# PytorchConnectomics/pytorch_connectomics

Measured on AMD Instinct MI355X. Metric: voxels/s (train + sliding-window infer), MedNeXt-S 112^3 bf16, higher is better.
Workload: dtype bf16; 1 GPU; Lucchi++ sliding-window inference (configs[1]): MedNeXt-S k3, 165x1024x768 volume, roi 112^3, overlap 0.5, bump blending, sw_batch_size 8, random-init weights; step = one whole-volume EagerSlidingWindowEngine call (TTA off); value = window-voxels/s; sw_batch_size=8, window_pipeline_streams=3

## Files before the change

### include/pytc_hip.h

```cpp
#ifndef PYTC_HIP_H
#define PYTC_HIP_H

#include <stdint.h>

#ifdef __cplusplus
extern "C" {
#endif

#define PYTC_ABI_VERSION 10

#define PYTC_OK 0
#define PYTC_ERR_INVALID 1
#define PYTC_ERR_HIP 2
#define PYTC_ERR_UNSUPPORTED 3

#define PYTC_F32 0
#define PYTC_BF16 1

#define PYTC_VIEW_FLIP_Z 1
#define PYTC_VIEW_FLIP_Y 2
#define PYTC_VIEW_FLIP_X 4
#define PYTC_VIEW_SWAP_YX 8
#define PYTC_VIEW_SWAP_ZY 16
#define PYTC_VIEW_SWAP_ZX 32

#define PYTC_PAD_CONSTANT 0
#define PYTC_PAD_REFLECT 1
#define PYTC_PAD_REPLICATE 2
#define PYTC_PAD_CIRCULAR 3

#define PYTC_BLEND_PRODUCT 0
#define PYTC_BLEND_MIN 1

#define PYTC_ACT_NONE 0
#define PYTC_ACT_SIGMOID 1
#define PYTC_ACT_TANH 2
#define PYTC_ACT_GELU 3

#define PYTC_RES_NONE 0
#define PYTC_RES_ADD 1
#define PYTC_RES_UPSAMPLE 2
#define PYTC_RES_GELU_BWD 3
#define PYTC_RES_NORM_BWD 4

int pytc_abi_version(void);
const char* pytc_last_error(void);
int pytc_device_info(int device, int* cu_count, int* lds_bytes_per_cu, char* arch, int arch_len);
int pytc_set_tuning(const char* key, int value);


int pytc_gather_windows(const float* vol, int C, int Z, int Y, int X, const int32_t* starts, int B,
                        int rz, int ry, int rx, int view, int pad_mode, float cval, void* out,
                        int out_dtype, void* stream);

int pytc_blend_accumulate(const void* pred, int pred_dtype, int B, const int32_t* starts, int rz,
                          int ry, int rx, int C, int view, const float* wz, const float* wy,
                          const float* wx, int combine, float floor_w, const int32_t* border ,
                          float* value, float* weight, int Z, int Y, int X, void* stream);

int pytc_blend_accumulate_mapped(const void* pred, int pred_dtype, int B, const int32_t* starts, int rz, int ry,
                                 int rx, int C, int view, const float* wz, const float* wy, const float* wx,
                                 int combine, float floor_w, const int32_t* border, const int32_t* chan_src,
// ... 105 lines not shown

typedef struct {
  const void* t;
  const float* ab;
  const void* w2_packed;
  const float* b2;
  const void* w3_packed;
  const float* b3;
  const void* res;
  const void* res_low;
  const float* res_bias;
  void* y;
  int N;
  int64_t rows_per_sample;
  int C_in, C_hid, C_out;
  int res_mode;
  int Di, Hi, Wi;
  int w3_format;
  int per_sample;
} pytc_mlp_args;
#define PYTC_W3_BF16 0
#define PYTC_W3_F16 1

int pytc_pw_gemm_supported(int C_in, int C_out);
int pytc_pw_gemm_fwd(const void* x, const void* w, const float* bias, const float* ab, void* y, int N, int64_t rows_per_sample,
                     int C_in, int C_out, int in_f16, int gelu_out, const void* res, const void* res_low, const float* res_bias,
                     int res_mode, int Di, int Hi, int Wi, void* stream);
int pytc_pw_mlp_supported(int C_in, int C_hid, int C_out);
int pytc_pw_pack_weight_paired(const float* w, int C_out, int C_in, int transposed, void* packed_bf16,
                               void* stream);
int pytc_pack_multi(const int64_t* table_dev, int n_items, int64_t total_elems, void* stream);
int pytc_pw_pack_weight_paired_f16(const float* w, int C_out, int C_in, int transposed, void* packed_f16,
                                   void* stream);
int pytc_pw_mlp_fwd(const pytc_mlp_args* a, void* stream);

int pytc_pw_mlp_lds_supported(int C_in, int C_hid, int C_out);
int pytc_pw_mlp_lds_fwd(const pytc_mlp_args* a, void* stream);
int pytc_pw_mlp_dma_applies(const pytc_mlp_args* a, int ignore_res_mode);
int pytc_pw_mlp_proj_supported(int C_in, int C_hid, int C_out, int C_proj);
int pytc_pw_mlp_proj_fwd(const pytc_mlp_args* a, const void* proj_w, const float* proj_b, void* z, int store_y, void* stream);
int pytc_pw_mlp_chunk_supported(int C_in, int C_hid, int C_out);
int pytc_pw_mlp_chunk_fwd(const pytc_mlp_args* a, void* stream);
int pytc_groupnorm_fold_mlp(const float* stats, int slots, float count, const float* gamma, const float* beta, float eps,
                            const float* w2, const float* b2, void* w2n, float* b2n, float* ab_out, int N, int C, int C_hid,
                            void* stream);
int pytc_pw_mlp_train_fwd(const pytc_mlp_args* a, void* hidden_pre, void* stream);
int pytc_pw_mlp_train_fwd_nostore(const pytc_mlp_args* a, void* stream);
int pytc_pw_mlp_bwd(const pytc_mlp_args* a, const void* hidden_pre, void* d_hidden, void* stream);
int pytc_pw_mlp_up_supported(int C_in, int C_hid, int C_out);
int pytc_pw_mlp_up_fwd(const pytc_mlp_args* a, const float* taps, const float* dw_bias, void* stream);
int pytc_pw_mlp_head_supported(int C_in, int C_hid, int C_out);
int pytc_pw_mlp_stemres_fwd(const pytc_mlp_args* a, const float* stem_x, const float* stem_w, const float* stem_b,
                            void* stream);
int pytc_stem_dwconv3d_stat_slots(int D, int H, int W);
int pytc_stem_dwconv3d_supported(int C_in, int C, int K);
int pytc_stem_dwconv3d_mfma_image_bytes(void);
int pytc_stem_dwconv3d_pack_mfma(const float* wx, const float* wb, const float* cst, void* image, void* stream);
int pytc_stem_dwconv3d_fwd(const float* x, const float* wx, const float* wb, const float* cst, const void* mfma_image, void* y,
                           float* stats, int N, int D, int H, int W, int C, void* stream);
int pytc_pw_mlp_head_fwd(const pytc_mlp_args* a, const void* head_w, const float* head_b, float* head_y, int n_head,
                         int store_y, void* stream);


#define PYTC_ACT_RELU 5
#define PYTC_ACT_LEAKY 6
#define PYTC_ACT_ELU 7

typedef struct {
  const void* x;
  const void* w_packed;
  const float* bias;
  const float* ab;
  const void* res;
  void* y;
  int N, D, H, W, C_in, C_out;
  int kd, kh, kw;
  int act_in;
  float act_param;
  int res_mode;
  int dtype;
} pytc_conv3d_args;

int64_t pytc_conv3d_packed_elems(int C_out, int C_in, int kd, int kh, int kw, int dtype);
int pytc_conv3d_pack_weight(const float* w, int C_out, int C_in, int kd, int kh, int kw, void* packed, int dtype,
                            void* stream);
int pytc_conv3d_fwd(const pytc_conv3d_args* a, void* stream);

int pytc_channel_stats_slots(int64_t rows);
int pytc_channel_stats(const void* x, float* stats, int N, int64_t rows, int C, int dtype, void* stream);
int pytc_norm_finalize_groups(const float* stats, int slots, float count, const float* gamma, const float* beta,
                              float eps, int groups, float* ab, int N, int C, void* stream);
int pytc_affine_act(const void* x, void* y, const float* ab, int N, int64_t rows, int C, int act, float prm,
                    int dtype, void* stream);
int pytc_maxpool3d_fwd(const void* x, void* y, int N, int D, int H, int W, int C, int fz, int fy, int fx, int dtype,
                       void* stream);
int pytc_dwconvT3d_generic_fwd(const void* x, void* y, const float* w, int N, int D, int H, int W, int C,
                               const int32_t* kernel, const int32_t* stride, const int32_t* pad, int dtype,
                               void* stream);


int pytc_groupnorm_finalize_mr(const float* stats, int slots, float count, const float* gamma, const float* beta,
                               float eps, float* ab, float* mean_rstd, int N, int C, void* stream);
int pytc_gelu(const void* x, const void* dy, void* out, int64_t n, int dtype, void* stream);
int pytc_add_inplace(void* y, const void* x, int64_t n, int dtype, void* stream);
int pytc_pw_wgrad_slots(int64_t rows_total);
int pytc_pw_wgrad(const void* x, const float* ab, const void* dy, float* dW, float* db, float* workspace, int N,
// ... 217 lines not shown
```

### pytorch_connectomics_amd/_native.py

```python
from __future__ import annotations

import ctypes as C
import os
from pathlib import Path

LIB_PATH = Path(__file__).resolve().parent / "lib" / "libpytc_hip.so"
ABI_VERSION = 10

F32, BF16 = 0, 1
OK = 0

VIEW_FLIP_Z, VIEW_FLIP_Y, VIEW_FLIP_X, VIEW_SWAP_YX, VIEW_SWAP_ZY, VIEW_SWAP_ZX = 1, 2, 4, 8, 16, 32
VIEW_SWAPS = {VIEW_SWAP_YX: (1, 2), VIEW_SWAP_ZY: (0, 1), VIEW_SWAP_ZX: (0, 2)}
PAD_MODES = {"constant": 0, "reflect": 1, "replicate": 2, "circular": 3}
BLEND_PRODUCT, BLEND_MIN = 0, 1
ACT_NONE, ACT_SIGMOID, ACT_TANH, ACT_GELU, ACT_SOFTMAX, ACT_RELU, ACT_LEAKY, ACT_ELU = 0, 1, 2, 3, 4, 5, 6, 7
RES_NONE, RES_ADD, RES_UPSAMPLE, RES_GELU_BWD, RES_NORM_BWD = 0, 1, 2, 3, 4


class PwArgs(C.Structure):
    _fields_ = [
        ("x", C.c_void_p), ("w_packed", C.c_void_p), ("bias", C.c_void_p), ("ab", C.c_void_p),
        ("res", C.c_void_p), ("y", C.c_void_p),
        ("N", C.c_int), ("rows_per_sample", C.c_int64),
        ("C_in", C.c_int), ("C_out", C.c_int),
        ("in_dtype", C.c_int), ("out_dtype", C.c_int), ("w_dtype", C.c_int),
        ("act", C.c_int), ("res_mode", C.c_int), ("gather", C.c_int),
        ("Di", C.c_int), ("Hi", C.c_int), ("Wi", C.c_int),
        ("res_low", C.c_void_p), ("res_bias", C.c_void_p), ("pre_act", C.c_int), ("w_paired", C.c_int),
    ]


class MlpArgs(C.Structure):
    _fields_ = [
        ("t", C.c_void_p), ("ab", C.c_void_p), ("w2_packed", C.c_void_p), ("b2", C.c_void_p),
        ("w3_packed", C.c_void_p), ("b3", C.c_void_p), ("res", C.c_void_p), ("res_low", C.c_void_p),
        ("res_bias", C.c_void_p), ("y", C.c_void_p),
        ("N", C.c_int), ("rows_per_sample", C.c_int64),
        ("C_in", C.c_int), ("C_hid", C.c_int), ("C_out", C.c_int), ("res_mode", C.c_int),
        ("Di", C.c_int), ("Hi", C.c_int), ("Wi", C.c_int), ("w3_format", C.c_int), ("per_sample", C.c_int),
    ]


W3_BF16, W3_F16 = 0, 1
NORM_NONE, NORM_ZSCORE, NORM_MINMAX, NORM_DIVIDE = 0, 1, 2, 3
RAW_DTYPES = {"uint8": 0, "int8": 1, "uint16": 2, "int16": 3, "uint32": 4, "int32": 5, "float32": 6, "float64": 7}


class ReduceItem(C.Structure):
    _fields_ = [("part", C.c_void_p), ("out", C.c_void_p), ("n", C.c_int64), ("slots", C.c_int32), ("out_t", C.c_int32)]


class Conv3dArgs(C.Structure):
    _fields_ = [
        ("x", C.c_void_p), ("w_packed", C.c_void_p), ("bias", C.c_void_p), ("ab", C.c_void_p), ("res", C.c_void_p),
        ("y", C.c_void_p),
        ("N", C.c_int), ("D", C.c_int), ("H", C.c_int), ("W", C.c_int), ("C_in", C.c_int), ("C_out", C.c_int),
        ("kd", C.c_int), ("kh", C.c_int), ("kw", C.c_int),
        ("act_in", C.c_int), ("act_param", C.c_float), ("res_mode", C.c_int), ("dtype", C.c_int),
    ]
# ... 139 lines not shown
                                      C.c_int, C.c_void_p]),
    "pytc_convT3d_phase_plan": (C.c_int, [C.c_int, C.c_int, C.c_int, C.c_void_p]),
    "pytc_convT3d_phase_supported": (C.c_int, [C.c_int, C.c_int, C.c_int]),
    "pytc_convT3d_phase_fwd": (C.c_int, [C.POINTER(Conv3dArgs), C.POINTER(C.c_int32), C.c_void_p]),
    "pytc_conv3d_wgrad_strided_ws_elems": (C.c_int64, [C.c_int, C.POINTER(C.c_int32), C.c_int, C.c_int, C.POINTER(C.c_int32)]),
    "pytc_conv3d_wgrad_strided": (C.c_int, [C.c_void_p, C.c_void_p, C.c_void_p, C.c_void_p, C.c_int, C.POINTER(C.c_int32),
                                            C.POINTER(C.c_int32), C.c_int, C.c_int, C.POINTER(C.c_int32), C.POINTER(C.c_int32),
                                            C.POINTER(C.c_int32), C.c_int, C.c_void_p]),
    "pytc_conv3d_pack_plan": (C.c_int, [C.c_int] * 7 + [C.c_void_p]),
    "pytc_conv3d_pack_multi": (C.c_int, [C.c_void_p, C.c_int, C.c_int64, C.c_void_p]),
    "pytc_conv3d_launch_plan": (C.c_int, [C.c_int] * 13 + [C.c_void_p]),
    "pytc_conv3d_pack_weight_dgrad": (C.c_int, [C.c_void_p, C.c_int, C.c_int, C.c_int, C.c_int, C.c_int, C.c_void_p, C.c_int, C.c_void_p]),
    "pytc_norm_bwd_means": (C.c_int, [C.c_void_p, C.c_void_p, C.c_void_p, C.c_void_p, C.c_void_p, C.c_int, C.c_int, C.c_int,
                                      C.c_float, C.c_void_p]),
    "pytc_norm_bwd_means_cpg": (C.c_int, [C.c_void_p, C.c_void_p, C.c_void_p, C.c_void_p, C.c_void_p, C.c_int, C.c_int, C.c_int,
                                          C.c_int, C.c_float, C.c_void_p]),
    "pytc_norm_finalize_groups_cpg": (C.c_int, [C.c_void_p, C.c_int, C.c_float, C.c_void_p, C.c_void_p, C.c_float, C.c_int, C.c_int,
                                                C.c_void_p, C.c_void_p, C.c_int, C.c_int, C.c_void_p]),
    "pytc_bn_train_finalize": (C.c_int, [C.c_void_p, C.c_int, C.c_float, C.c_void_p, C.c_void_p, C.c_float, C.c_float, C.c_void_p,
                                         C.c_void_p, C.c_void_p, C.c_void_p, C.c_void_p, C.c_int, C.c_int, C.c_void_p]),
    "pytc_bn_train_finalize_cpad": (C.c_int, [C.c_void_p, C.c_int, C.c_float, C.c_void_p, C.c_void_p, C.c_float, C.c_float, C.c_void_p,
                                              C.c_void_p, C.c_void_p, C.c_void_p, C.c_void_p, C.c_int, C.c_int, C.c_int, C.c_void_p]),
    "pytc_bn_update_running": (C.c_int, [C.c_void_p, C.c_void_p, C.c_void_p, C.c_int, C.c_float, C.c_float, C.c_float, C.c_void_p]),
    "pytc_layernorm_rows": (C.c_int, [C.c_void_p, C.c_void_p, C.c_void_p, C.c_void_p, C.c_int64, C.c_int, C.c_float, C.c_int, C.c_void_p]),
    "pytc_layernorm_rows_bwd_slots": (C.c_int, [C.c_int64, C.c_int, C.c_int]),
    "pytc_layernorm_rows_bwd": (C.c_int, [C.c_void_p, C.c_void_p, C.c_void_p, C.c_void_p, C.c_void_p, C.c_int64, C.c_int, C.c_float,
                                          C.c_int, C.c_void_p]),
    "pytc_grn_bwd_apply": (C.c_int, [C.c_void_p, C.c_void_p, C.c_void_p, C.c_void_p, C.c_void_p, C.c_int, C.c_int64, C.c_int, C.c_int,
                                     C.c_void_p]),
    "pytc_bce_dice_ws_elems": (C.c_int64, [C.c_int, C.c_int, C.c_int64]),
    "pytc_bce_dice_fwd": (C.c_int, [C.c_void_p, C.c_void_p, C.c_void_p, C.c_int, C.c_int, C.c_int64, C.POINTER(C.c_int64),
                                    C.POINTER(C.c_int64), C.POINTER(C.c_int64), C.c_float, C.c_float, C.c_float, C.c_float,
                                    C.c_float, C.c_void_p, C.c_void_p, C.c_void_p, C.c_void_p]),
    "pytc_bce_dice_bwd": (C.c_int, [C.c_void_p, C.c_void_p, C.c_void_p, C.c_void_p, C.c_void_p, C.c_void_p, C.c_void_p,
                                    C.c_int, C.c_int, C.c_int64, C.POINTER(C.c_int64), C.POINTER(C.c_int64),
                                    C.POINTER(C.c_int64), C.POINTER(C.c_int64), C.c_float, C.c_float, C.c_float, C.c_float,
                                    C.c_float, C.c_void_p]),
    "pytc_opt_chunk_elems": (C.c_int, []),
    "pytc_grad_norm_multi": (C.c_int, [C.c_void_p, C.c_void_p, C.c_int, C.c_float, C.c_void_p, C.c_void_p, C.c_void_p]),
    "pytc_adamw_multi": (C.c_int, [C.c_void_p, C.c_void_p, C.c_int, C.POINTER(C.c_float), C.c_int, C.c_void_p, C.c_void_p]),
    "pytc_pw_mlp_supported": (C.c_int, [C.c_int, C.c_int, C.c_int]),
    "pytc_pw_pack_weight_paired": (C.c_int, [C.c_void_p, C.c_int, C.c_int, C.c_int, C.c_void_p, C.c_void_p]),
    "pytc_pack_multi": (C.c_int, [C.c_void_p, C.c_int, C.c_int64, C.c_void_p]),
    "pytc_pw_pack_weight_paired_f16": (C.c_int, [C.c_void_p, C.c_int, C.c_int, C.c_int, C.c_void_p, C.c_void_p]),
    "pytc_pw_mlp_fwd": (C.c_int, [C.POINTER(MlpArgs), C.c_void_p]),
    "pytc_pw_mlp_lds_supported": (C.c_int, [C.c_int, C.c_int, C.c_int]),
    "pytc_pw_mlp_lds_fwd": (C.c_int, [C.POINTER(MlpArgs), C.c_void_p]),
    "pytc_pw_mlp_dma_applies": (C.c_int, [C.POINTER(MlpArgs), C.c_int]),
    "pytc_pw_mlp_proj_supported": (C.c_int, [C.c_int, C.c_int, C.c_int, C.c_int]),
    "pytc_pw_mlp_proj_fwd": (C.c_int, [C.POINTER(MlpArgs), C.c_void_p, C.c_void_p, C.c_void_p, C.c_int, C.c_void_p]),
    "pytc_pw_mlp_chunk_supported": (C.c_int, [C.c_int, C.c_int, C.c_int]),
    "pytc_pw_mlp_chunk_fwd": (C.c_int, [C.POINTER(MlpArgs), C.c_void_p]),
    "pytc_pw_mlp_stemres_fwd": (C.c_int, [C.POINTER(MlpArgs), C.c_void_p, C.c_void_p, C.c_void_p, C.c_void_p]),
    "pytc_stem_dwconv3d_stat_slots": (C.c_int, [C.c_int, C.c_int, C.c_int]),
    "pytc_stem_dwconv3d_supported": (C.c_int, [C.c_int, C.c_int, C.c_int]),
    "pytc_convT3d_thin_supported": (C.c_int, [C.c_int, C.c_int]),
    "pytc_convT3d_thin_fwd": (C.c_int, [C.c_void_p, C.c_void_p, C.c_void_p, C.c_void_p, C.c_int, C.POINTER(C.c_int32), C.c_int, C.c_int,
                                        C.c_int, C.c_void_p]),
    "pytc_stem_dwconv3d_mfma_image_bytes": (C.c_int, []),
    "pytc_stem_dwconv3d_pack_mfma": (C.c_int, [C.c_void_p, C.c_void_p, C.c_void_p, C.c_void_p, C.c_void_p]),
    "pytc_stem_dwconv3d_fwd": (C.c_int, [C.c_void_p, C.c_void_p, C.c_void_p, C.c_void_p, C.c_void_p, C.c_void_p, C.c_void_p,
                                         C.c_int, C.c_int, C.c_int, C.c_int, C.c_int, C.c_void_p]),
    "pytc_pw_mlp_train_fwd": (C.c_int, [C.POINTER(MlpArgs), C.c_void_p, C.c_void_p]),
    "pytc_pw_mlp_train_fwd_nostore": (C.c_int, [C.POINTER(MlpArgs), C.c_void_p]),
    "pytc_pw_mlp_bwd": (C.c_int, [C.POINTER(MlpArgs), C.c_void_p, C.c_void_p, C.c_void_p]),
    "pytc_pw_mlp_up_supported": (C.c_int, [C.c_int, C.c_int, C.c_int]),
    "pytc_pw_mlp_up_fwd": (C.c_int, [C.POINTER(MlpArgs), C.c_void_p, C.c_void_p, C.c_void_p]),
    "pytc_pw_mlp_head_supported": (C.c_int, [C.c_int, C.c_int, C.c_int]),
    "pytc_pw_mlp_head_fwd": (C.c_int, [C.POINTER(MlpArgs), C.c_void_p, C.c_void_p, C.c_void_p, C.c_int, C.c_int, C.c_void_p]),
    "pytc_upcat_deconv2_fwd": (C.c_int, [C.c_void_p, C.c_void_p, C.c_void_p, C.c_void_p, C.c_void_p] + [C.c_int] * 11 + [C.c_void_p]),
    "pytc_upcat_deconv2_bwd_data": (C.c_int, [C.c_void_p, C.c_void_p, C.c_void_p, C.c_void_p] + [C.c_int] * 11 + [C.c_void_p]),
    "pytc_upcat_deconv2_wgrad_ws_elems": (C.c_int64, [C.c_int] * 4),
    "pytc_upcat_deconv2_wgrad": (C.c_int, [C.c_void_p] * 5 + [C.c_int] * 11 + [C.c_void_p]),
    "pytc_linear_fwd": (C.c_int, [C.c_void_p] * 4 + [C.c_int] + [C.c_void_p] * 2 + [C.c_int] * 5 + [C.c_void_p]),
    "pytc_linear_bwd_data": (C.c_int, [C.c_void_p] * 4 + [C.c_int] * 4 + [C.c_void_p]),
    "pytc_linear_wgrad": (C.c_int, [C.c_void_p] * 5 + [C.c_int] * 6 + [C.c_void_p]),
    "pytc_layernorm_wide": (C.c_int, [C.c_void_p] * 4 + [C.c_int64, C.c_int, C.c_float, C.c_int, C.c_void_p]),
    "pytc_layernorm_wide_bwd_slots": (C.c_int, [C.c_int64]),
    "pytc_layernorm_wide_bwd": (C.c_int, [C.c_void_p] * 7 + [C.c_int64, C.c_int, C.c_float, C.c_int, C.c_void_p]),
    "pytc_patch_gather16": (C.c_int, [C.c_void_p] * 2 + [C.c_int] * 7 + [C.c_void_p]),
    "pytc_attention_supported": (C.c_int, [C.c_int]),
    "pytc_attention_fwd": (C.c_int, [C.c_void_p] * 3 + [C.c_int] * 4 + [C.c_float, C.c_int, C.c_void_p]),
    "pytc_attention_bwd": (C.c_int, [C.c_void_p] * 6 + [C.c_int] * 4 + [C.c_float, C.c_int, C.c_void_p]),
    "pytc_deconv2_upfirst_fwd": (C.c_int, [C.c_void_p] * 5 + [C.c_int] * 8 + [C.c_void_p]),
    "pytc_deconv2_upfirst_bwd_data": (C.c_int, [C.c_void_p] * 4 + [C.c_int] * 8 + [C.c_void_p]),
    "pytc_deconv2_upfirst_wgrad": (C.c_int, [C.c_void_p] * 5 + [C.c_int] * 8 + [C.c_void_p]),
    "pytc_window_attention_supported": (C.c_int, [C.c_int]),
    "pytc_window_attention_bias_groups": (C.c_int, [C.c_int] * 3),
    "pytc_window_attention_fwd": (C.c_int, [C.c_void_p] * 2 + [C.POINTER(C.c_int32)] + [C.c_void_p] * 2 + [C.c_int] * 4
                                  + [C.c_float, C.c_int, C.c_void_p]),
    "pytc_window_attention_bwd": (C.c_int, [C.c_void_p] * 2 + [C.POINTER(C.c_int32)] + [C.c_void_p] * 7 + [C.c_int] * 4
                                  + [C.c_float, C.c_int, C.c_void_p]),
    "pytc_window_partition": (C.c_int, [C.c_void_p] * 3 + [C.POINTER(C.c_int32)] + [C.c_int] * 4 + [C.c_void_p]),
    "pytc_space_to_depth2": (C.c_int, [C.c_void_p] * 2 + [C.c_int] * 8 + [C.c_void_p]),
    "pytc_layernorm_any": (C.c_int, [C.c_void_p] * 4 + [C.c_int64, C.c_int, C.c_float, C.c_int, C.c_void_p]),
    "pytc_layernorm_any_bwd_slots": (C.c_int, [C.c_int64]),
    "pytc_layernorm_any_bwd": (C.c_int, [C.c_void_p] * 8 + [C.c_int64, C.c_int, C.c_float, C.c_int, C.c_void_p]),
    "pytc_cldice_tiles": (C.c_int, [C.c_int64]),
    "pytc_cldice_erode": (C.c_int, [C.c_void_p] * 2 + [C.c_int] * 5 + [C.c_void_p]),
    "pytc_cldice_skeleton": (C.c_int, [C.c_void_p] * 7 + [C.c_int] * 6 + [C.c_void_p]),
    "pytc_cldice_chain_bwd": (C.c_int, [C.c_void_p] * 7 + [C.c_int] * 6 + [C.c_void_p]),
    "pytc_cldice_sweep_bwd": (C.c_int, [C.c_void_p] * 9 + [C.c_int] * 7 + [C.c_void_p]),
    "pytc_scnp_tiles": (C.c_int, [C.c_int64]),
    "pytc_scnp_forward": (C.c_int, [C.c_void_p] * 7 + [C.c_int] * 9 + [C.c_void_p]),
    "pytc_scnp_backward": (C.c_int, [C.c_void_p] * 7 + [C.c_int] * 9 + [C.c_void_p]),
    "pytc_softmax_loss_tiles": (C.c_int, [C.c_int64]),
# ... 55 lines not shown
```

### pytorch_connectomics_amd/csrc/pw_mlp_kernels.hip

```cpp
#include <cmath>
#include "pw_common.h"

namespace pytc {

struct MlpParams {
  const bf16_t* t;
  const float* ab;
  const bf16x8_t* w2;
  const float* b2;
  const bf16x8_t* w3;
  const float* b3;
  EpiParams e;
  long rps;
  int C_in, C_hid, C_out, HC;
  int w3_f16;
  long w2_stride;
  const bf16x8_t* head_w;
  const float* head_b;
  float* head_y;
  int n_head, store_y;
  bf16_t* proj_y;
  const float* stem_x;
  const float* stem_w;
  const float* stem_b;
  bf16_t* hp;
  int round_h;
  const bf16_t* hp_in;
};

constexpr int mlp_waves_per_simd(int ks, int mo, int nt) {
  if (ks >= 8 && nt == 1) return 1;
  const int regs = ks * nt * 4 + mo * nt * 4 + 2 * nt * 4;
  return regs <= 64 ? 4 : (regs <= 112 ? 3 : (regs <= 200 ? 2 : 1));
}

template <int KS_IN, int MO, int NT, int GELU_MODE, bool HEAD = false, bool STEMRES = false, bool STOREH = false, bool BWD = false>
__global__ void __launch_bounds__(256, mlp_waves_per_simd(KS_IN, MO, NT))
pw_mlp_kernel(MlpParams p) {
  constexpr int CIN = KS_IN * 32, COUT = MO * 16;
  static_assert(MO % 2 == 0, "C_out must be a multiple of 32");
  static_assert(!STEMRES || (MO == 2 && (MO / 2) * NT <= 4), "the stem-recomputing residual covers C_out = 32");
  static_assert(!HEAD || MO == 2, "the fused head covers C_out = 32");
  static_assert(GELU_MODE == 1 || GELU_MODE == 3, "sigmoid-form or packed-fp16 GELU");
  constexpr bool PREFETCH_RES = (MO / 2) * NT <= 4;
  const int wave = threadIdx.x >> 6, lane = threadIdx.x & 63;
  const int n = blockIdx.y;
  constexpr bool WARM = KS_IN * MO >= 32;
  constexpr int WPER = KS_IN * MO >= 512 ? 6 : 2;
  WarmRegs<WPER> warm;
  const bool folded = p.ab == nullptr;
  const bf16x8_t* w2 = p.w2 + (folded ? (long)n * p.w2_stride : 0L);
  const float* b2 = p.b2 + (folded ? (long)n * p.C_hid : 0L);
  if (WARM) {
    warm_l2(w2, (long)p.C_hid * CIN * 2, warm, 0);
    warm_l2(p.w3, (long)COUT * p.C_hid * 2, warm, WPER);
  }
  const long row0 = ((long)blockIdx.x * 4 + wave) * (NT * 16);
  if (row0 >= p.rps) {
    if (WARM) asm volatile("s_waitcnt vmcnt(0)" : : : "memory");
    return;
  }
  const int r = lane & 15, kb = lane >> 4;

  long orow[NT];
#pragma unroll
  for (int nt = 0; nt < NT; ++nt) orow[nt] = row0 + nt * 16 + r;

  bf16x8_t bact[KS_IN][NT];
  const bf16_t* tn = p.t + (long)n * p.rps * CIN;
  if (folded) {
#pragma unroll
    for (int ks = 0; ks < KS_IN; ++ks)
#pragma unroll
      for (int nt = 0; nt < NT; ++nt) {
        const long rr = orow[nt] < p.rps ? orow[nt] : p.rps - 1;
        bact[ks][nt] = ld_stream(reinterpret_cast<const bf16x8_t*>(tn + rr * CIN + ks * 32 + kb * 8), p.e.nt);
      }
  }
  const float* an = p.ab + (long)n * 2 * CIN;
#pragma unroll
  for (int ks = 0; ks < KS_IN; ++ks) {
    if (folded) break;
    const int k0 = ks * 32 + kb * 8;
    float av[8], bv[8];
    VecIO<float, 4>::load(an + k0, reinterpret_cast<float(&)[4]>(av[0]));
    VecIO<float, 4>::load(an + k0 + 4, reinterpret_cast<float(&)[4]>(av[4]));
    VecIO<float, 4>::load(an + CIN + k0, reinterpret_cast<float(&)[4]>(bv[0]));
    VecIO<float, 4>::load(an + CIN + k0 + 4, reinterpret_cast<float(&)[4]>(bv[4]));
#pragma unroll
    for (int nt = 0; nt < NT; ++nt) {
      const long rr = orow[nt] < p.rps ? orow[nt] : p.rps - 1;
      float v[8];
      VecIO<bf16_t, 8>::load(tn + rr * CIN + k0, v);
#pragma unroll
      for (int j = 0; j < 8; ++j) v[j] = fmaf(v[j], av[j], bv[j]);
      bact[ks][nt] = Mma<bf16_t>::from_floats(v);
    }
  }

  if (WARM) warm_l2_done(warm);

  uint4 rpre[PREFETCH_RES ? MO / 2 : 1][PREFETCH_RES ? NT : 1];
  const bool use_pre = PREFETCH_RES && p.e.res_mode != PYTC_RES_NONE;
  if constexpr (STEMRES) {
    const float* sx = p.stem_x + (long)n * p.rps;
    float sw[8], sb[8];
    VecIO<float, 4>::load(p.stem_w + kb * 8, reinterpret_cast<float(&)[4]>(sw[0]));
    VecIO<float, 4>::load(p.stem_w + kb * 8 + 4, reinterpret_cast<float(&)[4]>(sw[4]));
    VecIO<float, 4>::load(p.stem_b + kb * 8, reinterpret_cast<float(&)[4]>(sb[0]));
    VecIO<float, 4>::load(p.stem_b + kb * 8 + 4, reinterpret_cast<float(&)[4]>(sb[4]));
#pragma unroll
    for (int nt = 0; nt < NT; ++nt) {
      const float xv = sx[orow[nt] < p.rps ? orow[nt] : p.rps - 1];
      float rv[8];
#pragma unroll
      for (int j = 0; j < 8; ++j) rv[j] = fmaf(sw[j], xv, sb[j]);
      rpre[0][nt] = __builtin_bit_cast(uint4, Mma<bf16_t>::from_floats(rv));
    }
  } else if (use_pre) {
    const bf16_t* resn = reinterpret_cast<const bf16_t*>(p.e.res) + (long)n * p.rps * COUT;
#pragma unroll
    for (int pr = 0; pr < (PREFETCH_RES ? MO / 2 : 1); ++pr)
#pragma unroll
      for (int nt = 0; nt < (PREFETCH_RES ? NT : 1); ++nt) {
        const long rr = orow[nt] < p.rps ? orow[nt] : p.rps - 1;
        rpre[pr][nt] = ld_stream(reinterpret_cast<const uint4*>(resn + rr * COUT + pr * 32 + kb * 8), p.e.nt);
      }
  }

  f32x4_t acc2[MO][NT];
#pragma unroll
  for (int pr = 0; pr < MO / 2; ++pr) {
    float b[8];
    VecIO<float, 4>::load(p.b3 + pr * 32 + kb * 8, reinterpret_cast<float(&)[4]>(b[0]));
    VecIO<float, 4>::load(p.b3 + pr * 32 + kb * 8 + 4, reinterpret_cast<float(&)[4]>(b[4]));
#pragma unroll
    for (int nt = 0; nt < NT; ++nt) {
      acc2[2 * pr][nt] = f32x4_t{b[0], b[1], b[2], b[3]};
      acc2[2 * pr + 1][nt] = f32x4_t{b[4], b[5], b[6], b[7]};
    }
  }

  for (int hc = 0; hc < p.HC; ++hc) {
    float b2v[8];
    VecIO<float, 4>::load(b2 + hc * 32 + kb * 8, reinterpret_cast<float(&)[4]>(b2v[0]));
    VecIO<float, 4>::load(b2 + hc * 32 + kb * 8 + 4, reinterpret_cast<float(&)[4]>(b2v[4]));
    f32x4_t acc1[2][NT];
#pragma unroll
    for (int nt = 0; nt < NT; ++nt) {
      acc1[0][nt] = f32x4_t{b2v[0], b2v[1], b2v[2], b2v[3]};
      acc1[1][nt] = f32x4_t{b2v[4], b2v[5], b2v[6], b2v[7]};
    }
#pragma unroll
    for (int mt = 0; mt < 2; ++mt) {
#pragma unroll
      for (int ks = 0; ks < KS_IN; ++ks) {
        const bf16x8_t a = w2[((long)(hc * 2 + mt) * KS_IN + ks) * 64 + lane];
#pragma unroll
        for (int nt = 0; nt < NT; ++nt) acc1[mt][nt] = Mma<bf16_t>::mma(a, bact[ks][nt], acc1[mt][nt]);
      }
    }
    bf16x8_t bh[NT];
    h8_t bhh[GELU_MODE == 3 ? NT : 1];
#pragma unroll
    for (int nt = 0; nt < NT; ++nt) {
      float g[8];
// ... 83 lines not shown
  }
  int upos[NT][3];
  const bool ups = p.e.res_mode == PYTC_RES_UPSAMPLE;
  if (ups) {
    const unsigned ur = (unsigned)row0, gw = (unsigned)p.e.Go_w, gh = (unsigned)p.e.Go_h;
    const unsigned t0 = ur / gw;
    const int bx = (int)(ur - t0 * gw);
    const int bz = (int)(t0 / gh);
    const int by = (int)(t0 - (unsigned)bz * gh);
#pragma unroll
    for (int nt = 0; nt < NT; ++nt) {
      int px = bx + nt * 16 + r, py = by, pz = bz;
      while (px >= p.e.Go_w) { px -= p.e.Go_w; ++py; }
      while (py >= p.e.Go_h) { py -= p.e.Go_h; ++pz; }
      upos[nt][0] = pz; upos[nt][1] = py; upos[nt][2] = px;
    }
  }
#pragma unroll
  for (int pr = 0; pr < MO / 2; ++pr) {
#pragma unroll
    for (int nt = 0; nt < NT; ++nt) {
      if (orow[nt] >= p.rps) continue;
      float v[8];
#pragma unroll
      for (int j = 0; j < 4; ++j) {
        v[j] = acc2[2 * pr][nt][j];
        v[4 + j] = acc2[2 * pr + 1][nt][j];
      }
      if (use_pre) {
        float pre[8];
        VecIO<bf16_t, 8>::load(reinterpret_cast<const bf16_t*>(&rpre[PREFETCH_RES ? pr : 0][PREFETCH_RES ? nt : 0]), pre);
        finish_and_store<bf16_t, 8, false, COUT>(v, p.e, n, orow[nt], pr * 32 + kb * 8, pre, ups ? upos[nt] : nullptr);
      } else {
        finish_and_store<bf16_t, 8, false, COUT>(v, p.e, n, orow[nt], pr * 32 + kb * 8, nullptr, ups ? upos[nt] : nullptr);
      }
    }
  }
}


__device__ __forceinline__ void glds16(const void* gsrc, unsigned lds_dst) {
  unsigned keep;
  asm volatile("s_mov_b32 %0, m0\n\ts_mov_b32 m0, %2\n\ts_nop 0\n\tglobal_load_lds_dwordx4 %1, off\n\ts_mov_b32 m0, %0"
               : "=&s"(keep) : "v"(gsrc), "s"(lds_dst) : "memory");
}
__device__ __forceinline__ void glds4(const void* gsrc, unsigned lds_dst) {
  unsigned keep;
  asm volatile("s_mov_b32 %0, m0\n\ts_mov_b32 m0, %2\n\ts_nop 0\n\tglobal_load_lds_dword %1, off\n\ts_mov_b32 m0, %0"
               : "=&s"(keep) : "v"(gsrc), "s"(lds_dst) : "memory");
}

template <int HCT, int KIND>
__global__ void __launch_bounds__(256, 3)
pw_mlp_dma_kernel(MlpParams p, int waves_per_sample) {
  constexpr int NT = 4, CIN = 32, COUT = 32;
  constexpr bool STEM = KIND == 1, HEAD = KIND == 2, PROJ = KIND == 3;
  __shared__ __attribute__((aligned(16))) uint4 land[4][2][NT * 64];
  __shared__ __attribute__((aligned(16))) uint4 w2s[HCT * 2 * 64], w3s[2 * HCT * 64];
  __shared__ __attribute__((aligned(16))) float b2s[HCT * 32], b3s[32];
  __shared__ __attribute__((aligned(16))) float auxa[STEM ? 32 : (HEAD ? 256 : (PROJ ? 512 : 4))], auxb[(STEM || PROJ) ? 32 : (HEAD ? 16 : 4)];
  const int wave = threadIdx.x >> 6, lane = threadIdx.x & 63;
  const int n = blockIdx.y;
  const int r = lane & 15, kb = lane >> 4;
  const long tiles = (p.rps + NT * 16 - 1) / (NT * 16);
  const bool with_res = STEM || p.e.res_mode == PYTC_RES_ADD;
  const bf16_t* tn = p.t + (long)n * p.rps * CIN;
  const bf16_t* resn = (!STEM && with_res) ? reinterpret_cast<const bf16_t*>(p.e.res) + (long)n * p.rps * COUT : nullptr;
  const float* sx = STEM ? p.stem_x + (long)n * p.rps : nullptr;
  bf16_t* yn = reinterpret_cast<bf16_t*>(p.e.y) + (long)n * p.rps * COUT;
  float* hy = HEAD ? p.head_y + (long)n * p.rps * p.n_head : nullptr;
  bf16_t* zn = PROJ ? p.proj_y + (long)n * p.rps * 32 : nullptr;
  {
    const uint4* w2 = reinterpret_cast<const uint4*>(p.w2 + (long)n * p.w2_stride);
    const uint4* w3 = reinterpret_cast<const uint4*>(p.w3);
    for (int i = threadIdx.x; i < HCT * 2 * 64; i += 256) { w2s[i] = w2[i]; w3s[i] = w3[i]; }
    if (threadIdx.x < HCT * 32) b2s[threadIdx.x] = p.b2[(long)n * p.C_hid + threadIdx.x];
    if (threadIdx.x < 32) b3s[threadIdx.x] = p.b3[threadIdx.x];
    if constexpr (STEM) {
      if (threadIdx.x < 32) { auxa[threadIdx.x] = p.stem_w[threadIdx.x]; auxb[threadIdx.x] = p.stem_b[threadIdx.x]; }
    }
    if constexpr (HEAD) {
      reinterpret_cast<float*>(auxa)[threadIdx.x] = reinterpret_cast<const float*>(p.head_w)[threadIdx.x];
      if (threadIdx.x < 16) auxb[threadIdx.x] = (p.head_b && (int)threadIdx.x < p.n_head) ? p.head_b[threadIdx.x] : 0.f;
    }
    if constexpr (PROJ) {
      auxa[threadIdx.x] = reinterpret_cast<const float*>(p.head_w)[threadIdx.x];
      auxa[threadIdx.x + 256] = reinterpret_cast<const float*>(p.head_w)[threadIdx.x + 256];
      if (threadIdx.x < 32) auxb[threadIdx.x] = p.head_b ? p.head_b[threadIdx.x] : 0.f;
    }
  }
  __syncthreads();
  asm volatile("s_waitcnt vmcnt(0)" ::: "memory");

  const unsigned lbase = __builtin_amdgcn_readfirstlane((unsigned)(size_t)(__attribute__((address_space(3))) void*)&land[wave][0][0]);
  auto request = [&](long tile) {
#pragma unroll
    for (int nt = 0; nt < NT; ++nt) {
      long row = tile * (NT * 16) + nt * 16 + r;
      row = row < p.rps ? row : p.rps - 1;
      glds16(tn + row * CIN + kb * 8, lbase + (unsigned)(nt * 64) * 16);
      if constexpr (STEM) glds4(sx + row, lbase + (unsigned)(NT * 64) * 16 + (unsigned)(nt * 64) * 4);
      else if (with_res) glds16(resn + row * COUT + kb * 8, lbase + (unsigned)((NT + nt) * 64) * 16);
    }
  };
  bf16x8_t out[NT];
  f32x4_t hout[HEAD ? NT : 1];
  bf16x8_t zout[PROJ ? NT : 1];
  auto store = [&](long tile) {
#pragma unroll
    for (int nt = 0; nt < NT; ++nt) {
      const long row = tile * (NT * 16) + nt * 16 + r;
      if (row >= p.rps) continue;
      if (!(HEAD || PROJ) || p.store_y) *reinterpret_cast<bf16x8_t*>(yn + row * COUT + kb * 8) = out[nt];
      if constexpr (PROJ) *reinterpret_cast<bf16x8_t*>(zn + row * 32 + kb * 8) = zout[nt];
      if constexpr (HEAD) {
#pragma unroll
        for (int i = 0; i < 4; ++i)
          if (kb * 4 + i < p.n_head) hy[row * p.n_head + kb * 4 + i] = hout[nt][i];
      }
    }
  };
  const long gw = (long)blockIdx.x * 4 + wave;
  long tile = gw;
  if (tile >= tiles) return;
  request(tile);
  long out_tile = -1;
  for (; tile < tiles; tile += waves_per_sample) {
    asm volatile("s_waitcnt vmcnt(0)" ::: "memory");
    __builtin_amdgcn_wave_barrier();
    if (out_tile >= 0) store(out_tile);
    bf16x8_t bact[NT];
    uint4 rpre[STEM ? 1 : NT];
    float xin[STEM ? NT : 1];
#pragma unroll
    for (int nt = 0; nt < NT; ++nt) {
      bact[nt] = __builtin_bit_cast(bf16x8_t, land[wave][0][nt * 64 + lane]);
      if constexpr (STEM) xin[nt] = reinterpret_cast<const float*>(&land[wave][1][0])[nt * 64 + lane];
      else if (with_res) rpre[nt] = land[wave][1][nt * 64 + lane];
    }
    asm volatile("s_waitcnt lgkmcnt(0)" ::: "memory");
    __builtin_amdgcn_wave_barrier();
    if (tile + waves_per_sample < tiles) request(tile + waves_per_sample);
    f32x4_t acc2[2][NT];
    {
      const f32x4_t lo = *reinterpret_cast<const f32x4_t*>(&b3s[kb * 8]), hi = *reinterpret_cast<const f32x4_t*>(&b3s[kb * 8 + 4]);
#pragma unroll
      for (int nt = 0; nt < NT; ++nt) { acc2[0][nt] = lo; acc2[1][nt] = hi; }
    }
#pragma unroll
    for (int hc = 0; hc < HCT; ++hc) {
      f32x4_t acc1[2][NT];
      {
        const f32x4_t lo = *reinterpret_cast<const f32x4_t*>(&b2s[hc * 32 + kb * 8]), hi = *reinterpret_cast<const f32x4_t*>(&b2s[hc * 32 + kb * 8 + 4]);
#pragma unroll
        for (int nt = 0; nt < NT; ++nt) { acc1[0][nt] = lo; acc1[1][nt] = hi; }
// ... 22 lines not shown
    float sw[STEM ? 8 : 1], sb[STEM ? 8 : 1];
    if constexpr (STEM) {
#pragma unroll
      for (int j = 0; j < 8; ++j) { sw[j] = auxa[kb * 8 + j]; sb[j] = auxb[kb * 8 + j]; }
    }
#pragma unroll
    for (int nt = 0; nt < NT; ++nt) {
      float v[8];
#pragma unroll
      for (int j = 0; j < 4; ++j) { v[j] = acc2[0][nt][j]; v[4 + j] = acc2[1][nt][j]; }
      if constexpr (STEM) {
        float rv[8], pre[8];
#pragma unroll
        for (int j = 0; j < 8; ++j) rv[j] = fmaf(sw[j], xin[nt], sb[j]);
        const bf16x8_t rb = Mma<bf16_t>::from_floats(rv);
        VecIO<bf16_t, 8>::load(reinterpret_cast<const bf16_t*>(&rb), pre);
#pragma unroll
        for (int j = 0; j < 8; ++j) v[j] += pre[j];
      } else if (with_res) {
        float pre[8];
        VecIO<bf16_t, 8>::load(reinterpret_cast<const bf16_t*>(&rpre[nt]), pre);
#pragma unroll
        for (int j = 0; j < 8; ++j) v[j] += pre[j];
      }
      out[nt] = Mma<bf16_t>::from_floats(v);
      if constexpr (HEAD) {
        const bf16x8_t ah = __builtin_bit_cast(bf16x8_t, reinterpret_cast<const uint4*>(auxa)[lane]);
        const f32x4_t hb = *reinterpret_cast<const f32x4_t*>(&auxb[kb * 4]);
        const f32x4_t h = Mma<bf16_t>::mma(ah, out[nt], f32x4_t{0.f, 0.f, 0.f, 0.f});
#pragma unroll
        for (int i = 0; i < 4; ++i) hout[nt][i] = h[i] + hb[i];
      }
      if constexpr (PROJ) {
        f32x4_t z0 = *reinterpret_cast<const f32x4_t*>(&auxb[kb * 8]), z1 = *reinterpret_cast<const f32x4_t*>(&auxb[kb * 8 + 4]);
        z0 = Mma<bf16_t>::mma(__builtin_bit_cast(bf16x8_t, reinterpret_cast<const uint4*>(auxa)[lane]), out[nt], z0);
        z1 = Mma<bf16_t>::mma(__builtin_bit_cast(bf16x8_t, reinterpret_cast<const uint4*>(auxa)[64 + lane]), out[nt], z1);
        float zv[8];
#pragma unroll
        for (int j = 0; j < 4; ++j) { zv[j] = z0[j]; zv[4 + j] = z1[j]; }
        zout[nt] = Mma<bf16_t>::from_floats(zv);
      }
    }
    out_tile = tile;
  }
  store(out_tile);
}

static bool mlp_dma_applies(const pytc_mlp_args* a, const MlpParams& p) {
  return a->per_sample && p.w3_f16 && a->C_in == 32 && a->C_out == 32 && (p.HC == 2 || p.HC == 3 || p.HC == 4) &&
         (a->res_mode == PYTC_RES_NONE || a->res_mode == PYTC_RES_ADD) && tuning_get(K_mlp_dma) != 0 &&
         (long)a->N * a->rows_per_sample >= (long)tuning_get(K_mlp_dma_rows);
}
template <int KIND>
static void mlp_dma_launch(const pytc_mlp_args* a, const MlpParams& p, hipStream_t s) {
  const long tiles = (a->rows_per_sample + 63) / 64;
  long wgs = (3072 + a->N - 1) / a->N;
  const long most = (tiles / 2 + 3) / 4;
  if (wgs > most) wgs = most < 1 ? 1 : most;
  if (const int forced = tuning_get(K_mlp_dma_wgs); forced > 0) wgs = forced;
  dim3 grid((unsigned)wgs, (unsigned)a->N), block(256);
  const int wps = (int)(wgs * 4);
  if (p.HC == 2) hipLaunchKernelGGL((pw_mlp_dma_kernel<2, KIND>), grid, block, 0, s, p, wps);
  else if (p.HC == 3) hipLaunchKernelGGL((pw_mlp_dma_kernel<3, KIND>), grid, block, 0, s, p, wps);
  else hipLaunchKernelGGL((pw_mlp_dma_kernel<4, KIND>), grid, block, 0, s, p, wps);
}

template <typename OUT>
__global__ void __launch_bounds__(256)
pw_pack_paired_kernel(const float* __restrict__ w, int C_out, int C_in, int transposed,
                      OUT* __restrict__ packed, int KG, long total) {
  long i = (long)blockIdx.x * blockDim.x + threadIdx.x;
  if (i >= total) return;
  int j = (int)(i % 8);
  long t = i / 8;
  int lane = (int)(t % 64);
  t /= 64;
  int kg = (int)(t % KG);
  int T = (int)(t / KG);
  int o = paired_row(T, lane & 15);
  int k = kg * 32 + (lane >> 4) * 8 + j;
  float v = 0.f;
  if (o < C_out && k < C_in) v = transposed ? w[(long)k * C_out + o] : w[(long)o * C_in + k];
  if constexpr (sizeof(OUT) == 2 && !__is_same(OUT, bf16_t)) packed[i] = (OUT)v;
  else packed[i] = from_f32<bf16_t>(v);
}

__global__ void __launch_bounds__(256)
pack_multi_kernel(const long* __restrict__ table, int n_items, long total) {
  const long i = (long)blockIdx.x * blockDim.x + threadIdx.x;
  __shared__ int s_lo;
  if (threadIdx.x == 0) {
    const long i0 = (long)blockIdx.x * blockDim.x;
    int lo = 0, hi = n_items - 1;
    while (lo < hi) {
      const int mid = (lo + hi + 1) >> 1;
      if (table[mid * 8 + 6] <= i0) lo = mid; else hi = mid - 1;
    }
    s_lo = lo;
  }
  __syncthreads();
  if (i >= total) return;
  int lo = s_lo;
  while (lo + 1 < n_items && table[(lo + 1) * 8 + 6] <= i) ++lo;
  const long* it = table + lo * 8;
  const float* w = reinterpret_cast<const float*>(it[0]);
  const int kind = (int)it[2], C_out = (int)it[3], C_in = (int)it[4], aux = (int)it[5];
  const long e = i - it[6];
  if (kind >= 6) {
    const int o = (int)(e / C_in), k = (int)(e % C_in);
    reinterpret_cast<bf16_t*>(it[1])[e] = from_f32<bf16_t>(kind == 7 ? w[(long)k * C_out + o] : w[e]);
    return;
  }
  if (kind >= 4) {
    const int K3 = aux, C = C_out;
    const int k = (int)(e / C), c = (int)(e % C);
    reinterpret_cast<float*>(it[1])[e] = w[(long)c * K3 + (kind == 5 ? K3 - 1 - k : k)];
    return;
// ... 225 lines not shown
  PYTC_LAUNCH_CHECK("pw_pack_weight_paired_f16");
  return PYTC_OK;
}

extern "C" int pytc_pack_multi(const int64_t* table_dev, int n_items, int64_t total_elems, void* stream) {
  PYTC_REQUIRE(table_dev && n_items >= 1 && total_elems >= 1, "pack_multi: bad arguments");
  hipLaunchKernelGGL(pack_multi_kernel, dim3(ceil_div(total_elems, 256)), dim3(256), 0, (hipStream_t)stream,
                     reinterpret_cast<const long*>(table_dev), n_items, (long)total_elems);
  PYTC_LAUNCH_CHECK("pack_multi");
  return PYTC_OK;
}

extern "C" int pytc_pw_mlp_head_fwd(const pytc_mlp_args* a, const void* head_w, const float* head_b, float* head_y,
                                    int n_head, int store_y, void* stream) {
  PYTC_REQUIRE(a && a->t && (a->ab || a->per_sample) && a->w2_packed && a->w3_packed && a->b2 && a->b3 && head_w && head_y, "pw_mlp_head: null pointer");
  PYTC_REQUIRE(!(a->ab && a->per_sample), "pw_mlp_head: per-sample (norm-folded) expand operands come without an affine");
  PYTC_REQUIRE(!store_y || a->y, "pw_mlp_head: store_y without an output buffer");
  PYTC_REQUIRE(a->N >= 1 && a->rows_per_sample >= 1 && n_head >= 1 && n_head <= 16, "pw_mlp_head: bad shape");
  if (!pytc_pw_mlp_head_supported(a->C_in, a->C_hid, a->C_out)) {
    set_error("pw_mlp_head: no fused kernel for C_in=%d C_hid=%d C_out=%d", a->C_in, a->C_hid, a->C_out);
    return PYTC_ERR_UNSUPPORTED;
  }
  PYTC_REQUIRE(a->res_mode == PYTC_RES_NONE || (a->res_mode == PYTC_RES_ADD && a->res), "pw_mlp_head: residual add or none");
  MlpParams p;
  p.t = (const bf16_t*)a->t; p.ab = a->ab; p.w2 = (const bf16x8_t*)a->w2_packed; p.b2 = a->b2;
  p.w3 = (const bf16x8_t*)a->w3_packed; p.b3 = a->b3;
  p.rps = a->rows_per_sample; p.C_in = a->C_in; p.C_hid = a->C_hid; p.C_out = a->C_out; p.HC = a->C_hid / 32;
  p.w2_stride = (long)(a->C_hid / 16) * (a->C_in / 32) * 64;
  p.e.res = a->res; p.e.res_low = nullptr; p.e.res_bias = nullptr; p.e.y = a->y;
  p.e.rps_out = a->rows_per_sample; p.e.C_out = a->C_out; p.e.res_mode = a->res_mode;
  p.e.nt = 0;
  p.e.Go_d = p.e.Go_h = p.e.Go_w = p.e.Gl_d = p.e.Gl_h = p.e.Gl_w = 0;
  p.head_w = (const bf16x8_t*)head_w; p.head_b = head_b; p.head_y = head_y; p.n_head = n_head; p.store_y = store_y;
  p.w3_f16 = a->w3_format == PYTC_W3_F16 ? 1 : 0;
  dim3 grid((unsigned)((p.rps + 4L * 4 * 16 - 1) / (4L * 4 * 16)), (unsigned)a->N), block(256);
  hipStream_t s = (hipStream_t)stream;
  if (mlp_dma_applies(a, p)) {
    mlp_dma_launch<2>(a, p, s);
    PYTC_LAUNCH_CHECK("pw_mlp_head_dma");
    return PYTC_OK;
  }
  if (p.w3_f16) {
    if (a->C_in == 32) hipLaunchKernelGGL((pw_mlp_kernel<1, 2, 4, 3, true>), grid, block, 0, s, p);
    else hipLaunchKernelGGL((pw_mlp_kernel<2, 2, 4, 3, true>), grid, block, 0, s, p);
  } else if (a->C_in == 32) {
    hipLaunchKernelGGL((pw_mlp_kernel<1, 2, 4, 1, true>), grid, block, 0, s, p);
  } else {
    hipLaunchKernelGGL((pw_mlp_kernel<2, 2, 4, 1, true>), grid, block, 0, s, p);
  }
  PYTC_LAUNCH_CHECK("pw_mlp_head");
  return PYTC_OK;
}

extern "C" int pytc_pw_mlp_stemres_fwd(const pytc_mlp_args* a, const float* stem_x, const float* stem_w, const float* stem_b,
                                       void* stream) {
  PYTC_REQUIRE(a && a->t && (a->ab || a->per_sample) && a->w2_packed && a->w3_packed && a->b2 && a->b3 && a->y && stem_x && stem_w && stem_b,
               "pw_mlp_stemres: null pointer");
  PYTC_REQUIRE(!(a->ab && a->per_sample), "pw_mlp_stemres: per-sample (norm-folded) expand operands come without an affine");
  PYTC_REQUIRE(a->N >= 1 && a->rows_per_sample >= 1, "pw_mlp_stemres: bad shape");
  if (!(a->C_in == 32 && a->C_out == 32 && a->C_hid % 32 == 0 && a->C_hid >= 32)) {
    set_error("pw_mlp_stemres: no fused kernel for C_in=%d C_hid=%d C_out=%d", a->C_in, a->C_hid, a->C_out);
    return PYTC_ERR_UNSUPPORTED;
  }
  MlpParams p{};
  p.t = (const bf16_t*)a->t; p.ab = a->ab; p.w2 = (const bf16x8_t*)a->w2_packed; p.b2 = a->b2;
  p.w3 = (const bf16x8_t*)a->w3_packed; p.b3 = a->b3;
  p.rps = a->rows_per_sample; p.C_in = a->C_in; p.C_hid = a->C_hid; p.C_out = a->C_out; p.HC = a->C_hid / 32;
  p.w2_stride = (long)(a->C_hid / 16) * (a->C_in / 32) * 64;
  p.e.res = a->y;
  p.e.y = a->y;
  p.e.rps_out = a->rows_per_sample; p.e.C_out = a->C_out; p.e.res_mode = PYTC_RES_ADD;
  p.e.nt = 0;
  p.stem_x = stem_x; p.stem_w = stem_w; p.stem_b = stem_b;
  p.w3_f16 = a->w3_format == PYTC_W3_F16 ? 1 : 0;
  dim3 grid((unsigned)((p.rps + 4L * 4 * 16 - 1) / (4L * 4 * 16)), (unsigned)a->N), block(256);
  hipStream_t s = (hipStream_t)stream;
  pytc_mlp_args shape = *a;
  shape.res_mode = PYTC_RES_NONE;
  if (mlp_dma_applies(&shape, p)) {
    mlp_dma_launch<1>(a, p, s);
    PYTC_LAUNCH_CHECK("pw_mlp_stemres_dma");
    return PYTC_OK;
  }
  if (p.w3_f16) hipLaunchKernelGGL((pw_mlp_kernel<1, 2, 4, 3, false, true>), grid, block, 0, s, p);
  else hipLaunchKernelGGL((pw_mlp_kernel<1, 2, 4, 1, false, true>), grid, block, 0, s, p);
  PYTC_LAUNCH_CHECK("pw_mlp_stemres");
  return PYTC_OK;
}

extern "C" int pytc_pw_mlp_dma_applies(const pytc_mlp_args* a, int ignore_res_mode) {
  if (!a) return 0;
  MlpParams p{};
  p.HC = a->C_hid / 32;
  p.w3_f16 = a->w3_format == PYTC_W3_F16 ? 1 : 0;
  pytc_mlp_args shape = *a;
  if (ignore_res_mode) shape.res_mode = PYTC_RES_NONE;
  return mlp_dma_applies(&shape, p) ? 1 : 0;
}

extern "C" int pytc_pw_mlp_proj_supported(int C_in, int C_hid, int C_out, int C_proj) {
  return (C_in == 32 && C_out == 32 && C_proj == 32 && (C_hid == 64 || C_hid == 96 || C_hid == 128)) ? 1 : 0;
}
extern "C" int pytc_pw_mlp_proj_fwd(const pytc_mlp_args* a, const void* proj_w, const float* proj_b, void* z, int store_y, void* stream) {
  PYTC_REQUIRE(a && a->t && a->w2_packed && a->w3_packed && a->b2 && a->b3 && proj_w && z, "pw_mlp_proj: null pointer");
  PYTC_REQUIRE(a->per_sample && !a->ab, "pw_mlp_proj: takes the per-sample (norm-folded) expand operands");
  PYTC_REQUIRE(a->w3_format == PYTC_W3_F16, "pw_mlp_proj: the mixer's projection image must be fp16 (pytc_pw_pack_weight_paired_f16)");
  PYTC_REQUIRE(!store_y || a->y, "pw_mlp_proj: store_y without an output buffer");
  PYTC_REQUIRE(a->N >= 1 && a->rows_per_sample >= 1, "pw_mlp_proj: bad shape");
  if (!pytc_pw_mlp_proj_supported(a->C_in, a->C_hid, a->C_out, 32)) {
    set_error("pw_mlp_proj: no fused kernel for C_in=%d C_hid=%d C_out=%d", a->C_in, a->C_hid, a->C_out);
    return PYTC_ERR_UNSUPPORTED;
  }
  PYTC_REQUIRE(a->res_mode == PYTC_RES_NONE || (a->res_mode == PYTC_RES_ADD && a->res), "pw_mlp_proj: residual add or none");
  MlpParams p{};
  p.t = (const bf16_t*)a->t; p.ab = nullptr; p.w2 = (const bf16x8_t*)a->w2_packed; p.b2 = a->b2;
  p.w3 = (const bf16x8_t*)a->w3_packed; p.b3 = a->b3;
  p.rps = a->rows_per_sample; p.C_in = a->C_in; p.C_hid = a->C_hid; p.C_out = a->C_out; p.HC = a->C_hid / 32;
  p.w2_stride = (long)(a->C_hid / 16) * (a->C_in / 32) * 64;
  p.e.res = a->res; p.e.y = a->y; p.e.rps_out = a->rows_per_sample; p.e.C_out = a->C_out; p.e.res_mode = a->res_mode;
  p.head_w = (const bf16x8_t*)proj_w; p.head_b = proj_b; p.proj_y = (bf16_t*)z; p.store_y = store_y;
  p.w3_f16 = 1;
  mlp_dma_launch<3>(a, p, (hipStream_t)stream);
  PYTC_LAUNCH_CHECK("pw_mlp_proj");
  return PYTC_OK;
}

static int mlp_fwd_impl(const pytc_mlp_args* a, void* hp, void* stream, const void* hp_in = nullptr, bool round_h = false);

extern "C" int pytc_pw_mlp_bwd(const pytc_mlp_args* a, const void* hidden_pre, void* d_hidden, void* stream) {
  PYTC_REQUIRE(hidden_pre && d_hidden, "pw_mlp_bwd: null hidden buffers");
  PYTC_REQUIRE(a && a->res_mode == PYTC_RES_NONE, "pw_mlp_bwd: no residual in the backward mixer");
  return mlp_fwd_impl(a, d_hidden, stream, hidden_pre);
}

extern "C" int pytc_pw_mlp_train_fwd(const pytc_mlp_args* a, void* hidden_pre, void* stream) {
  PYTC_REQUIRE(hidden_pre, "pw_mlp_train: null hidden buffer");
  return mlp_fwd_impl(a, hidden_pre, stream);
}

extern "C" int pytc_pw_mlp_train_fwd_nostore(const pytc_mlp_args* a, void* stream) {
// ... 51 lines not shown
```

### pytorch_connectomics_amd/csrc/pytc_common.h

```cpp
#pragma once
#include <hip/hip_runtime.h>
#include <stdint.h>
#include <stdio.h>
#include <string.h>

#include "../../include/pytc_hip.h"

namespace pytc {

typedef __bf16 bf16_t;
typedef __bf16 bf16x2_t __attribute__((ext_vector_type(2)));
typedef __bf16 bf16x4_t __attribute__((ext_vector_type(4)));
typedef __bf16 bf16x8_t __attribute__((ext_vector_type(8)));
typedef float f32x2_t __attribute__((ext_vector_type(2)));
typedef float f32x4_t __attribute__((ext_vector_type(4)));
typedef float f32x8_t __attribute__((ext_vector_type(8)));
typedef float f32x16_t __attribute__((ext_vector_type(16)));
typedef short s16x8_t __attribute__((ext_vector_type(8)));

constexpr int WAVE = 64;

void set_error(const char* fmt, ...);
int hip_fail(hipError_t e, const char* what);
bool ensure_dynamic_lds(const void* kernel, size_t bytes, const char* what);
bool take_launch_failure();

#define PYTC_REQUIRE(cond, ...)                     \
  do {                                              \
    if (!(cond)) {                                  \
      pytc::set_error(__VA_ARGS__);                 \
      return PYTC_ERR_INVALID;                      \
    }                                               \
  } while (0)

#define PYTC_LAUNCH_CHECK(name)                                  \
  do {                                                           \
    if (pytc::take_launch_failure()) return PYTC_ERR_HIP;        \
    hipError_t e_ = hipGetLastError();                           \
    if (e_ != hipSuccess) return pytc::hip_fail(e_, name);       \
  } while (0)

#define PYTC_KNOBS(X)                                                                                                             \
  X(channel_act_flat, 1, "channel activation of contiguous NDHWC tensors as a flat 16-byte stream; 0 = the per-voxel kernel")      \
  X(conv_wgrad_mfma, 1, "dense-conv weight gradient on the matrix cores (bf16); 0 = the VALU kernel")                              \
  X(dw_wgrad_march, 1, "depthwise K = 3 / stride 1 weight gradient as a z-march; 0 = the vector / generic kernels")                \
  X(dw_wgrad_vec, 1, "depthwise K = 3 weight gradient with 16-byte channel vectors; 0 = the generic kernel")                       \
  X(dwconvT_tile, 1, "transposed depthwise conv at C = 64 / 128 (bf16) as one tile of input cells per workgroup; 0 = cell kernel") \
  X(dwconv_march_h16, 1, "VALU z-march depthwise conv: packed-f16 in-plane partial sums; 0 = fp32 taps")                           \
  X(dwconv_mfma, 1, "bf16 stride-1 K = 3 depthwise forward (and the fused block) on the matrix cores; 0 = the VALU z-march")       \
  X(dwconv_mfma_variant, 0, "matrix-core depthwise conv: bit 0 = hi + lo weight halves, bit 1 = two planes in flight, not three")  \
  X(dwconv_s2_march, 1, "stride-2 K = 3 depthwise conv at C = 32 / 64 (bf16) as a z-march over an LDS ring; 0 = gather kernel")    \
  X(elementwise_vec, 1, "16-byte vector forms of the norm-apply / elementwise training kernels; 0 = the scalar kernels")           \
  X(mixer_bwd_rc_slot_div, 1, "recomputing mixer backward: divide the slot count (fewer, longer slots)")                           \
  X(mlp_chunk_variant, 0, "chunked-hidden mixer (pw_mlp_chunk_kernels.hip): tile shape of the launch")                             \
  X(mlp_dma, 1, "level-0 mixer with DMA-prefetched row tiles (pw_mlp_dma_kernel); 0 = one tile per wave")                          \
  X(mlp_dma_rows, 1 << 20, "fewest rows of a launch that takes the DMA mixer")                                                     \
  X(mlp_dma_wgs, 0, "DMA mixer: workgroups per sample; 0 = chosen from the row count")                                             \
  X(mlp_lds_variant, 0, "LDS-resident mixer (pw_mlp_lds_kernels.hip): tile shape of the launch")                                   \
  X(norm_bwd_from_wgrad_flat, 1, "GroupNorm-backward epilogue of the expand weight gradient as one flat kernel; 0 = chunked")      \
  X(pw_gemm_rows, 0, "LDS-tiled 1x1 GEMM: 64 / 128 forces the rows per workgroup; 0 = by problem size")                            \
  X(pw_thin, 1, "plain 1x1 convs with one input / few output channels on the thin kernels; 0 = the generic kernel")                \
  X(wgrad_dgrad_fused, 1, "projecting conv's weight gradient and the GELU-backward data gradient in one kernel; 0 = two launches")  \
  X(wgrad_small_split, 1, "matrix-core 1x1 weight gradient: more, shorter row slots when the launch would leave CUs idle")         \
  X(wgrad_valu, 0, "1: 1x1 weight gradient on the VALU kernel instead of the matrix cores")                                        \
  X(wgrad_whole_rounds, 1, "matrix-core 1x1 weight gradient: round the slot count down to whole rounds of resident workgroups")

enum Knob {
#define PYTC_KNOB_ENUM(name, dflt, doc) K_##name,
  PYTC_KNOBS(PYTC_KNOB_ENUM)
#undef PYTC_KNOB_ENUM
  K_COUNT
};
int tuning_get(Knob k);

template <typename T, int VEC>
struct VecIO;

template <int VEC>
struct VecIO<float, VEC> {
  typedef float vec_t __attribute__((ext_vector_type(VEC)));
  static __device__ __forceinline__ void load(const float* p, float (&v)[VEC]) {
    vec_t t = *reinterpret_cast<const vec_t*>(p);
#pragma unroll
    for (int i = 0; i < VEC; ++i) v[i] = t[i];
  }
  static __device__ __forceinline__ void store(float* p, const float (&v)[VEC]) {
    vec_t t;
#pragma unroll
    for (int i = 0; i < VEC; ++i) t[i] = v[i];
    *reinterpret_cast<vec_t*>(p) = t;
  }
};
template <>
struct VecIO<float, 1> {
  static __device__ __forceinline__ void load(const float* p, float (&v)[1]) { v[0] = *p; }
  static __device__ __forceinline__ void store(float* p, const float (&v)[1]) { *p = v[0]; }
};

template <int VEC>
struct VecIO<bf16_t, VEC> {
  typedef __bf16 vec_t __attribute__((ext_vector_type(VEC)));
  typedef float fvec_t __attribute__((ext_vector_type(VEC)));
  static __device__ __forceinline__ void load(const bf16_t* p, float (&v)[VEC]) {
    vec_t t = *reinterpret_cast<const vec_t*>(p);
    fvec_t f = __builtin_convertvector(t, fvec_t);
#pragma unroll
    for (int i = 0; i < VEC; ++i) v[i] = f[i];
  }
  static __device__ __forceinline__ void store(bf16_t* p, const float (&v)[VEC]) {
    fvec_t f;
#pragma unroll
    for (int i = 0; i < VEC; ++i) f[i] = v[i];
    *reinterpret_cast<vec_t*>(p) = __builtin_convertvector(f, vec_t);
  }
// ... 126 lines not shown
```

### pytorch_connectomics_amd/csrc/stem_dwconv_kernels.hip

```cpp
#include "pytc_common.h"

namespace pytc {

constexpr int SD_C = 32;

struct StemDw { int D, H, W, GX; long groups; };

constexpr int SD_IT = 4;
template <int SD_VX>
__global__ void __launch_bounds__(256)
stem_dwconv_k3_kernel(const float* __restrict__ x, const float* __restrict__ wx, const float* __restrict__ wb,
                      const float* __restrict__ cst, bf16_t* __restrict__ y, float* __restrict__ stats, StemDw g, int slots) {
  __shared__ __attribute__((aligned(16))) float lw[2 * 27 * SD_C + SD_C];
  __shared__ float red[16][256 + 4];
  for (int i = threadIdx.x; i < 27 * SD_C; i += 256) { lw[i] = wx[i]; lw[27 * SD_C + i] = wb[i]; }
  if (threadIdx.x < SD_C) lw[54 * SD_C + threadIdx.x] = cst[threadIdx.x];
  __syncthreads();
  const float* lwx = lw;
  const float* lwb = lw + 27 * SD_C;
  const float* lc = lw + 54 * SD_C;

  const int n = blockIdx.y;
  const int cg = threadIdx.x & 3, c0 = cg * 8;
  const long rps = (long)g.D * g.H * g.W;
  const float* xn = x + (long)n * rps;
  bf16_t* yn = y + (long)n * rps * SD_C;
  float s1[8], s2[8];
#pragma unroll
  for (int j = 0; j < 8; ++j) { s1[j] = 0.f; s2[j] = 0.f; }

  for (int it = 0; it < SD_IT; ++it) {
    asm volatile("" ::: "memory");
    const long G = ((long)blockIdx.x * SD_IT + it) * 64 + (threadIdx.x >> 2);
    const bool live = G < g.groups;
    const long Gc = live ? G : g.groups - 1;
    const int gx = (int)(Gc % g.GX);
    const long tq = Gc / g.GX;
    const int vy = (int)(tq % g.H), vz = (int)(tq / g.H);
    const int x0 = gx * SD_VX;
    float acc[SD_VX][8];
    {
      const float4 k0 = *reinterpret_cast<const float4*>(lc + c0), k1 = *reinterpret_cast<const float4*>(lc + c0 + 4);
#pragma unroll
      for (int v = 0; v < SD_VX; ++v) {
        acc[v][0] = k0.x; acc[v][1] = k0.y; acc[v][2] = k0.z; acc[v][3] = k0.w;
        acc[v][4] = k1.x; acc[v][5] = k1.y; acc[v][6] = k1.z; acc[v][7] = k1.w;
      }
    }
    const bool left_in = x0 > 0, right_in = x0 + SD_VX < g.W;
#pragma unroll
    for (int r = 0; r < 9; ++r) {
      const int dz = r / 3 - 1, dy = r % 3 - 1;
      const int z = vz + dz, yy = vy + dy;
      const bool row_in = z >= 0 && z < g.D && yy >= 0 && yy < g.H;
      const int zc = z < 0 ? 0 : (z >= g.D ? g.D - 1 : z), yc = yy < 0 ? 0 : (yy >= g.H ? g.H - 1 : yy);
      const float* row = xn + ((long)zc * g.H + yc) * g.W + x0;
      const float lft = row[left_in ? -1 : 0], rgt = row[right_in ? SD_VX : SD_VX - 1];
      float in[SD_VX + 2];
      in[0] = (row_in && left_in) ? lft : 0.f;
#pragma unroll
      for (int q = 0; q < SD_VX / 4; ++q) {
        const float4 mid = *reinterpret_cast<const float4*>(row + q * 4);
        in[1 + q * 4] = row_in ? mid.x : 0.f; in[2 + q * 4] = row_in ? mid.y : 0.f;
        in[3 + q * 4] = row_in ? mid.z : 0.f; in[4 + q * 4] = row_in ? mid.w : 0.f;
      }
      in[SD_VX + 1] = (row_in && right_in) ? rgt : 0.f;
#pragma unroll
      for (int dx = 0; dx < 3; ++dx) {
        const int t = r * 3 + dx;
        const float4 w0 = *reinterpret_cast<const float4*>(lwx + t * SD_C + c0);
        const float4 w1 = *reinterpret_cast<const float4*>(lwx + t * SD_C + c0 + 4);
#pragma unroll
        for (int v = 0; v < SD_VX; ++v) {
          const float xv = in[v + dx];
          acc[v][0] = fmaf(w0.x, xv, acc[v][0]); acc[v][1] = fmaf(w0.y, xv, acc[v][1]);
          acc[v][2] = fmaf(w0.z, xv, acc[v][2]); acc[v][3] = fmaf(w0.w, xv, acc[v][3]);
          acc[v][4] = fmaf(w1.x, xv, acc[v][4]); acc[v][5] = fmaf(w1.y, xv, acc[v][5]);
          acc[v][6] = fmaf(w1.z, xv, acc[v][6]); acc[v][7] = fmaf(w1.w, xv, acc[v][7]);
        }
        const bool edge_l = dx == 0 && !left_in, edge_r = dx == 2 && !right_in;
        if (!row_in || edge_l || edge_r) {
          const float4 b0 = *reinterpret_cast<const float4*>(lwb + t * SD_C + c0);
          const float4 b1 = *reinterpret_cast<const float4*>(lwb + t * SD_C + c0 + 4);
#pragma unroll
          for (int v = 0; v < SD_VX; ++v) {
            const bool out = !row_in || (edge_l && v == 0) || (edge_r && v == SD_VX - 1);
            if (out) {
              acc[v][0] -= b0.x; acc[v][1] -= b0.y; acc[v][2] -= b0.z; acc[v][3] -= b0.w;
              acc[v][4] -= b1.x; acc[v][5] -= b1.y; acc[v][6] -= b1.z; acc[v][7] -= b1.w;
            }
          }
        }
      }
    }
    if (live) {
      const long vbase = ((long)vz * g.H + vy) * g.W + x0;
#pragma unroll
      for (int v = 0; v < SD_VX; ++v) {
        f32x8_t f;
#pragma unroll
        for (int j = 0; j < 8; ++j) f[j] = acc[v][j];
        const bf16x8_t o = __builtin_convertvector(f, bf16x8_t);
        *reinterpret_cast<bf16x8_t*>(yn + (vbase + v) * SD_C + c0) = o;
        const f32x8_t q = __builtin_convertvector(o, f32x8_t);
#pragma unroll
        for (int j = 0; j < 8; ++j) { s1[j] += q[j]; s2[j] = fmaf(q[j], q[j], s2[j]); }
      }
    }
  }

#pragma unroll
  for (int j = 0; j < 8; ++j) { red[j][threadIdx.x] = s1[j]; red[8 + j][threadIdx.x] = s2[j]; }
  __syncthreads();
  if (threadIdx.x < 2 * SD_C) {
    const int which = threadIdx.x / SD_C, c = threadIdx.x % SD_C;
    const float* col = red[which * 8 + (c & 7)];
    float a = 0.f;
    for (int l = 0; l < 64; ++l) a += col[l * 4 + (c >> 3)];
    stats[(((long)n * slots + blockIdx.x) * 2 + which) * SD_C + c] = a;
  }
}

constexpr int SM_XT = 16, SM_YT = 8, SM_ZT = 8;
constexpr int SM_RS = 20;
constexpr int SM_EY = SM_YT + 2, SM_EZ = SM_ZT + 2, SM_ROWS = SM_EY * SM_EZ, SM_HALO = SM_ROWS * SM_RS;
constexpr int SM_IMG_FRAG = 4 * 64;
constexpr int SM_IMG_BYTES = SM_IMG_FRAG * 16 + 2 * SD_C * 4;

struct StemMf { int D, H, W, bx, by, bz, zr; };

__global__ void __launch_bounds__(256)
stem_pack_mfma_kernel(const float* __restrict__ wx, const float* __restrict__ wb, const float* __restrict__ cst,
                      h8_t* __restrict__ frag, float* __restrict__ kc) {
  const int tid = threadIdx.x;
  const int mat = tid >> 7, q = (tid >> 6) & 1, lane = tid & 63;
  const int grp = lane >> 4, m = lane & 15;
  const int ch = 8 * (m >> 2) + (m & 3) + 4 * q;
  const float* w = mat ? wb : wx;
  h8_t v;
#pragma unroll
  for (int j = 0; j < 8; ++j) {
    const int k = 8 * grp + j;
    v[j] = (_Float16)(k < 27 ? w[k * SD_C + ch] : 0.f);
  }
  frag[tid] = v;
  if (tid < SD_C) {
    float sb = 0.f;
    for (int k = 0; k < 27; ++k) sb += wb[k * SD_C + tid];
    kc[tid] = cst[tid];
    kc[SD_C + tid] = cst[tid] - sb;
  }
}

template <bool STORE_PERMUTE>
__global__ void __launch_bounds__(256, 4)
stem_dwconv_k3_mfma_kernel(const float* __restrict__ x, const h8_t* __restrict__ frag, const float* __restrict__ kc,
                           bf16_t* __restrict__ y, float* __restrict__ stats, StemMf g, int slots) {
  __shared__ __attribute__((aligned(16))) _Float16 hbuf[2 * SM_HALO];
  _Float16* const hx = hbuf;
  _Float16* const hin = hbuf + SM_HALO;
  __shared__ float red[4][2][SD_C];
  const int tid = threadIdx.x;
  const int lane = tid & 63, wave = tid >> 6;
  const int grp = lane >> 4, nn = lane & 15;
  const int c0 = 8 * grp;
  const h8_t ax0 = frag[lane], ax1 = frag[64 + lane], ab0 = frag[128 + lane], ab1 = frag[192 + lane];
  const f32x4_t ki0 = *reinterpret_cast<const f32x4_t*>(kc + c0), ki1 = *reinterpret_cast<const f32x4_t*>(kc + c0 + 4);
  const f32x4_t kb0 = *reinterpret_cast<const f32x4_t*>(kc + SD_C + c0), kb1 = *reinterpret_cast<const f32x4_t*>(kc + SD_C + c0 + 4);

  const int n = blockIdx.y;
  int b = blockIdx.x;
  const int bxi = b % g.bx; b /= g.bx;
  const int byi = b % g.by;
  const int bzi = b / g.by;
  const int x0 = bxi * SM_XT, y0 = byi * SM_YT;
  const int zbeg = bzi * g.zr, zend = min(zbeg + g.zr, g.D);
  const bool left_in = x0 > 0, right_in = x0 + SM_XT < g.W;
  const bool xy_border = !left_in || !right_in || y0 == 0 || y0 + SM_YT >= g.H;
  const long rps = (long)g.D * g.H * g.W;
  const float* xn = x + (long)n * rps;
  bf16_t* yn = y + (long)n * rps * SD_C;

  typedef const __attribute__((address_space(3))) _Float16* lds_h_ptr;
  lds_h_ptr tp[8];
#pragma unroll
  for (int j = 0; j < 8; ++j) {
    const int k = 8 * grp + j;
    tp[j] = (lds_h_ptr)hbuf + (wave * SM_RS + 1 + nn + (k < 27 ? ((k / 9) * SM_EY + (k / 3) % 3) * SM_RS + k % 3 : 0));
  }
  const int st_src = ((lane & 3) << 4) | (lane >> 2);
  const int st_vox = lane >> 2, st_piece = lane & 3;
  float s1[8], s2[8];
#pragma unroll
  for (int j = 0; j < 8; ++j) { s1[j] = 0.f; s2[j] = 0.f; }

  constexpr int N_INT = SM_ROWS * 4, N_EDGE = SM_ROWS * 2;
  float4 pre_v[2];
  float pre_e;
  auto stage_issue = [&](int z0) {
#pragma unroll
    for (int u = 0; u < 2; ++u) {
      const int it = min(tid + 256 * u, N_INT - 1);
      const int r = it >> 2, p = it & 3;
      const int gy = y0 - 1 + r % SM_EY, gz = z0 - 1 + r / SM_EY;
      const int cy = min(max(gy, 0), g.H - 1), cz = min(max(gz, 0), g.D - 1);
      pre_v[u] = *reinterpret_cast<const float4*>(xn + ((long)cz * g.H + cy) * g.W + x0 + 4 * p);
    }
    {
      const int it = min(tid, N_EDGE - 1);
      const int r = it >> 1, right = it & 1;
      const int gy = y0 - 1 + r % SM_EY, gz = z0 - 1 + r / SM_EY;
      const int cy = min(max(gy, 0), g.H - 1), cz = min(max(gz, 0), g.D - 1);
      pre_e = xn[((long)cz * g.H + cy) * g.W + x0 + (right ? (right_in ? SM_XT : SM_XT - 1) : (left_in ? -1 : 0))];
    }
  };
  auto stage_commit = [&](int z0, bool border) {
#pragma unroll
    for (int u = 0; u < 2; ++u) {
      const int it = tid + 256 * u;
      if (it < N_INT) {
        const int r = it >> 2, p = it & 3;
        const int gy = y0 - 1 + r % SM_EY, gz = z0 - 1 + r / SM_EY;
        const bool row_in = gy >= 0 && gy < g.H && gz >= 0 && gz < g.D;
        const float4 v = pre_v[u];
        h2_t* dst = reinterpret_cast<h2_t*>(&hx[r * SM_RS + 2 + 4 * p]);
        dst[0] = h2_t{(_Float16)(row_in ? v.x : 0.f), (_Float16)(row_in ? v.y : 0.f)};
        dst[1] = h2_t{(_Float16)(row_in ? v.z : 0.f), (_Float16)(row_in ? v.w : 0.f)};
        if (border) {
          const _Float16 one = (_Float16)(row_in ? 1.f : 0.f);
          h2_t* di = reinterpret_cast<h2_t*>(&hin[r * SM_RS + 2 + 4 * p]);
          di[0] = h2_t{one, one}; di[1] = h2_t{one, one};
        }
      }
    }
    if (tid < N_EDGE) {
      const int r = tid >> 1, right = tid & 1;
      const int gy = y0 - 1 + r % SM_EY, gz = z0 - 1 + r / SM_EY;
      const bool in = gy >= 0 && gy < g.H && gz >= 0 && gz < g.D && (right ? right_in : left_in);
      const int dsti = r * SM_RS + (right ? 2 + SM_XT : 1);
      hx[dsti] = (_Float16)(in ? pre_e : 0.f);
      if (border) hin[dsti] = (_Float16)(in ? 1.f : 0.f);
    }
  };

  stage_issue(zbeg);
  for (int z0 = zbeg; z0 < zend; z0 += SM_ZT) {
    const bool border = xy_border || z0 == 0 || z0 + SM_ZT >= g.D;
    __syncthreads();
    stage_commit(z0, border);
    __syncthreads();
    if (z0 + SM_ZT < zend) stage_issue(z0 + SM_ZT);
    const f32x4_t k0 = border ? kb0 : ki0, k1 = border ? kb1 : ki1;
    bf16_t* ytile = yn + (((long)z0 * g.H + y0 + wave) * g.W + x0) * SD_C + (STORE_PERMUTE ? st_vox * SD_C + st_piece * 8 : nn * SD_C + c0);
#pragma unroll 1
    for (int tz = 0; tz < SM_ZT; ++tz) {
#pragma unroll
      for (int h = 0; h < 2; ++h) {
        const int toff = 4 * h * SM_RS;
        h8_t bq;
#pragma unroll
        for (int j = 0; j < 8; ++j) bq[j] = tp[j][toff];
        f32x4_t a0 = __builtin_amdgcn_mfma_f32_16x16x32_f16(ax0, bq, k0, 0, 0, 0);
        f32x4_t a1 = __builtin_amdgcn_mfma_f32_16x16x32_f16(ax1, bq, k1, 0, 0, 0);
        if (border) {
          h8_t bi;
#pragma unroll
// ... 36 lines not shown
  __syncthreads();
  if (tid < 2 * SD_C) {
    const int which = tid / SD_C, c = tid % SD_C;
    stats[(((long)n * slots + blockIdx.x) * 2 + which) * SD_C + c] =
        ((red[0][which][c] + red[1][which][c]) + red[2][which][c]) + red[3][which][c];
  }
}

}

using namespace pytc;

static int sd_vx(int) { return 4; }

static int sd_it() { return SD_IT; }

static bool sd_mfma(int D, int H, int W) {
  return W % SM_XT == 0 && H % SM_YT == 0 && D % SM_ZT == 0;
}

static void sd_geom(pytc::StemMf& m, int D, int H, int W) {
  m.D = D; m.H = H; m.W = W;
  m.bx = W / SM_XT;
  m.by = (H + SM_YT - 1) / SM_YT;
  m.zr = SM_ZT;
  for (int zr = 32; zr > SM_ZT; zr >>= 1)
    if ((long)m.bx * m.by * ((D + zr - 1) / zr) >= 256) { m.zr = zr; break; }
  m.bz = (D + m.zr - 1) / m.zr;
}

extern "C" int pytc_stem_dwconv3d_stat_slots(int D, int H, int W) {
  if (sd_mfma(D, H, W)) {
    StemMf m;
    sd_geom(m, D, H, W);
    return m.bx * m.by * m.bz;
  }
  const long groups = (long)D * H * (W / sd_vx(W));
  const long gpb = 64L * sd_it();
  return (int)((groups + gpb - 1) / gpb);
}

extern "C" int pytc_stem_dwconv3d_supported(int C_in, int C, int K) { return (C_in == 1 && C == SD_C && K == 3) ? 1 : 0; }

extern "C" int pytc_stem_dwconv3d_mfma_image_bytes(void) { return SM_IMG_BYTES; }

extern "C" int pytc_stem_dwconv3d_pack_mfma(const float* wx, const float* wb, const float* cst, void* image, void* stream) {
  PYTC_REQUIRE(wx && wb && cst && image, "stem_dwconv3d_pack_mfma: null pointer");
  hipLaunchKernelGGL(stem_pack_mfma_kernel, dim3(1), dim3(256), 0, (hipStream_t)stream, wx, wb, cst, (h8_t*)image,
                     (float*)((char*)image + SM_IMG_FRAG * 16));
  PYTC_LAUNCH_CHECK("stem_dwconv3d_pack_mfma");
  return PYTC_OK;
}

extern "C" int pytc_stem_dwconv3d_fwd(const float* x, const float* wx, const float* wb, const float* cst, const void* mfma_image,
                                      void* y, float* stats, int N, int D, int H, int W, int C, void* stream) {
  PYTC_REQUIRE(x && wx && wb && cst && y && stats, "stem_dwconv3d: null pointer");
  PYTC_REQUIRE(N >= 1 && D >= 1 && H >= 1 && W >= 4 && C == SD_C, "stem_dwconv3d: C must be 32");
  PYTC_REQUIRE(W % 4 == 0, "stem_dwconv3d: W must be a multiple of 4");
  const int slots = pytc_stem_dwconv3d_stat_slots(D, H, W);
  if (sd_mfma(D, H, W)) {
    PYTC_REQUIRE(mfma_image, "stem_dwconv3d: the f16-MFMA form needs the image of pytc_stem_dwconv3d_pack_mfma");
    StemMf m;
    sd_geom(m, D, H, W);
    const float* kc = (const float*)((const char*)mfma_image + SM_IMG_FRAG * 16);
    hipLaunchKernelGGL(stem_dwconv_k3_mfma_kernel<true>, dim3(slots, N), dim3(256), 0, (hipStream_t)stream, x,
                       (const h8_t*)mfma_image, kc, (bf16_t*)y, stats, m, slots);
    PYTC_LAUNCH_CHECK("stem_dwconv3d_mfma");
    return PYTC_OK;
  }
  const int vx = sd_vx(W);
  StemDw g{D, H, W, W / vx, (long)D * H * (W / vx)};
  hipLaunchKernelGGL(stem_dwconv_k3_kernel<4>, dim3(slots, N), dim3(256), 0, (hipStream_t)stream, x, wx, wb, cst, (bf16_t*)y,
                     stats, g, slots);
  PYTC_LAUNCH_CHECK("stem_dwconv3d");
  return PYTC_OK;
}
```

### pytorch_connectomics_amd/csrc/window_kernels.hip

```cpp
#include "pytc_common.h"

#pragma clang fp contract(off)

namespace pytc {

__device__ __forceinline__ float mul_rn(float a, float b) { return a * b; }
__device__ __forceinline__ float add_rn(float a, float b) { return a + b; }
__device__ __forceinline__ float sub_rn(float a, float b) { return a - b; }

struct StartList {
  int s[64 * 3];
};

__device__ __forceinline__ int pad_index(int g, int lo, int hi, int mode, bool& inside) {
  inside = true;
  if (g >= lo && g < hi) return g;
  const int n = hi - lo, j = g - lo;
  if (n <= 0) { inside = false; return 0; }
  switch (mode) {
    case PYTC_PAD_REFLECT: {
      if (n == 1) return lo;
      int p = 2 * (n - 1);
      int m = j % p;
      if (m < 0) m += p;
      return lo + (m < n ? m : p - m);
    }
    case PYTC_PAD_REPLICATE:
      return j < 0 ? lo : hi - 1;
    case PYTC_PAD_CIRCULAR: {
      int m = j % n;
      return lo + (m < 0 ? m + n : m);
    }
    default:
      inside = false;
      return 0;
  }
}

__device__ __forceinline__ void view_src(int view, int rz, int ry, int rx, int z, int y, int x,
                                         int& wz, int& wy, int& wx) {
  int fz = (view & PYTC_VIEW_FLIP_Z) ? rz - 1 - z : z;
  int fy = (view & PYTC_VIEW_FLIP_Y) ? ry - 1 - y : y;
  int fx = (view & PYTC_VIEW_FLIP_X) ? rx - 1 - x : x;
  if (view & PYTC_VIEW_SWAP_YX) {
    wz = fz; wy = fx; wx = fy;
  } else if (view & PYTC_VIEW_SWAP_ZY) {
    wz = fy; wy = fz; wx = fx;
  } else if (view & PYTC_VIEW_SWAP_ZX) {
    wz = fx; wy = fy; wx = fz;
  } else {
    wz = fz; wy = fy; wx = fx;
  }
}

static inline bool view_ok(int view, int rz, int ry, int rx) {
  const int swaps = view & (PYTC_VIEW_SWAP_YX | PYTC_VIEW_SWAP_ZY | PYTC_VIEW_SWAP_ZX);
  if (view & ~63) return false;
  if (swaps == 0) return true;
  if (swaps == PYTC_VIEW_SWAP_YX) return ry == rx;
  if (swaps == PYTC_VIEW_SWAP_ZY) return rz == ry;
  if (swaps == PYTC_VIEW_SWAP_ZX) return rz == rx;
  return false;
}

template <typename TO>
// ... 219 lines not shown
  }
}

__global__ void __launch_bounds__(256)
channel_activation_flat_kernel(float4* __restrict__ value, long n4, int C, int c0, int c1, int act, float scale) {
  long i = (long)blockIdx.x * blockDim.x + threadIdx.x;
  const long stride = (long)gridDim.x * blockDim.x;
  for (; i < n4; i += stride) {
    float4 q = value[i];
    float v[4] = {q.x, q.y, q.z, q.w};
    int c = (int)((i * 4) % C);
#pragma unroll
    for (int j = 0; j < 4; ++j) {
      if (c >= c0 && c < c1) {
        float t = v[j] * scale;
        if (act == PYTC_ACT_SIGMOID) t = 1.0f / (1.0f + expf(-t));
        else if (act == PYTC_ACT_TANH) t = tanhf(t);
        v[j] = t;
      }
      if (++c == C) c = 0;
    }
    value[i] = float4{v[0], v[1], v[2], v[3]};
  }
}

}

using namespace pytc;

extern "C" int pytc_channel_activation(float* value, int C, int64_t nvox, int channels_last, int c0, int c1, int act,
                                       float scale, void* stream) {
  PYTC_REQUIRE(value && C >= 1 && nvox > 0 && c0 >= 0 && c1 <= C && c0 < c1, "channel_activation: bad arguments");
  PYTC_REQUIRE(act == PYTC_ACT_NONE || act == PYTC_ACT_SIGMOID || act == PYTC_ACT_TANH || act == 4,
               "channel_activation: bad activation %d", act);
  if (channels_last && act != 4 && ((long)nvox * C) % 4 == 0 && ((uintptr_t)value & 15) == 0 && tuning_get(K_channel_act_flat)) {
    const long n4 = (long)nvox * C / 4;
    const long want = (n4 + 255) / 256;
    hipLaunchKernelGGL(channel_activation_flat_kernel, dim3((unsigned)(want < 65536 ? want : 65536)), dim3(256), 0, (hipStream_t)stream,
                       reinterpret_cast<float4*>(value), n4, C, c0, c1, act, scale);
    PYTC_LAUNCH_CHECK("channel_activation");
    return PYTC_OK;
  }
  int blocks = (int)((nvox + 255) / 256 < 8192 ? (nvox + 255) / 256 : 8192);
  hipLaunchKernelGGL(channel_activation_kernel, dim3(blocks), dim3(256), 0, (hipStream_t)stream, value, (long)nvox,
                     channels_last ? 1L : (long)nvox, channels_last ? (long)C : 1L, c0, c1, act, scale);
  PYTC_LAUNCH_CHECK("channel_activation");
  return PYTC_OK;
}

extern "C" int pytc_gather_windows(const float* vol, int C, int Z, int Y, int X, const int32_t* starts,
                                   int B, int rz, int ry, int rx, int view, int pad_mode, float cval,
                                   void* out, int out_dtype, void* stream) {
  PYTC_REQUIRE(vol && out && starts, "gather_windows: null pointer");
  PYTC_REQUIRE(B >= 1 && B <= 64, "gather_windows: B=%d must be in [1,64]", B);
  PYTC_REQUIRE(C >= 1 && rz > 0 && ry > 0 && rx > 0 && Z > 0 && Y > 0 && X > 0, "gather_windows: bad shape");
  PYTC_REQUIRE(view_ok(view, rz, ry, rx), "gather_windows: at most one SWAP bit, and the exchanged window axes must have equal length");
  PYTC_REQUIRE(pad_mode >= 0 && pad_mode <= 3, "gather_windows: bad pad_mode %d", pad_mode);
  StartList st;
  memcpy(st.s, starts, sizeof(int) * 3 * B);
  long per_win = (long)rz * ry * rx;
  dim3 grid(ceil_div(per_win, 256), 1, B), block(256);
  hipStream_t s = (hipStream_t)stream;
  if (out_dtype == PYTC_F32)
    hipLaunchKernelGGL(gather_windows_kernel<float>, grid, block, 0, s, vol, C, Z, Y, X, st, rz, ry, rx, view,
                       pad_mode, cval, 0, 0, 0, (float*)out);
  else if (out_dtype == PYTC_BF16)
    hipLaunchKernelGGL(gather_windows_kernel<bf16_t>, grid, block, 0, s, vol, C, Z, Y, X, st, rz, ry, rx, view,
                       pad_mode, cval, 0, 0, 0, (bf16_t*)out);
  else
    PYTC_REQUIRE(false, "gather_windows: bad out_dtype %d", out_dtype);
  PYTC_LAUNCH_CHECK("gather_windows");
  return PYTC_OK;
}

extern "C" int pytc_blend_accumulate(const void* pred, int pred_dtype, int B, const int32_t* starts, int rz,
                                     int ry, int rx, int C, int view, const float* wz, const float* wy,
                                     const float* wx, int combine, float floor_w, const int32_t* border,
                                     float* value, float* weight, int Z, int Y, int X, void* stream) {
  PYTC_REQUIRE(pred && starts && wz && wy && wx && value, "blend_accumulate: null pointer");
  PYTC_REQUIRE(B >= 1 && C >= 1, "blend_accumulate: bad B/C");
  PYTC_REQUIRE(view_ok(view, rz, ry, rx), "blend_accumulate: at most one SWAP bit, and the exchanged window axes must have equal length");
  PYTC_REQUIRE(combine == PYTC_BLEND_PRODUCT || combine == PYTC_BLEND_MIN, "blend_accumulate: bad combine");
  long per_win = (long)rz * ry * rx;
  dim3 grid(ceil_div(per_win, 256)), block(256);
  hipStream_t s = (hipStream_t)stream;
  const int bz = border ? border[0] : 0, by = border ? border[1] : 0, bx = border ? border[2] : 0;
  PYTC_REQUIRE(bz >= 0 && by >= 0 && bx >= 0 && 2 * bz < rz && 2 * by < ry && 2 * bx < rx,
               "blend_accumulate: border mask too large for the window");
  for (int b = 0; b < B; ++b) {
    int sz = starts[3 * b], sy = starts[3 * b + 1], sx = starts[3 * b + 2];
    if (pred_dtype == PYTC_F32)
      hipLaunchKernelGGL(blend_accumulate_kernel<float>, grid, block, 0, s,
                         (const float*)pred + (long)b * per_win * C, sz, sy, sx, rz, ry, rx, C, view, wz, wy, wx,
                         combine, floor_w, bz, by, bx, value, weight, Z, Y, X);
    else if (pred_dtype == PYTC_BF16)
      hipLaunchKernelGGL(blend_accumulate_kernel<bf16_t>, grid, block, 0, s,
                         (const bf16_t*)pred + (long)b * per_win * C, sz, sy, sx, rz, ry, rx, C, view, wz, wy, wx,
                         combine, floor_w, bz, by, bx, value, weight, Z, Y, X);
    else
      PYTC_REQUIRE(false, "blend_accumulate: bad pred_dtype %d", pred_dtype);
  }
  PYTC_LAUNCH_CHECK("blend_accumulate");
  return PYTC_OK;
}

extern "C" int pytc_blend_accumulate_mapped(const void* pred, int pred_dtype, int B, const int32_t* starts, int rz, int ry,
                                            int rx, int C, int view, const float* wz, const float* wy, const float* wx,
                                            int combine, float floor_w, const int32_t* border, const int32_t* chan_src,
                                            const int32_t* chan_shift, float* value, float* weight, int Z, int Y, int X,
                                            void* stream) {
  PYTC_REQUIRE(pred && starts && wz && wy && wx && value && chan_src && chan_shift, "blend_accumulate_mapped: null pointer");
  PYTC_REQUIRE(B >= 1 && C >= 1 && C <= MAX_MAP, "blend_accumulate_mapped: C=%d must be in [1,%d]", C, MAX_MAP);
  PYTC_REQUIRE(view_ok(view, rz, ry, rx), "blend_accumulate_mapped: at most one SWAP bit, and the exchanged window axes must have equal length");
  PYTC_REQUIRE(combine == PYTC_BLEND_PRODUCT || combine == PYTC_BLEND_MIN, "blend_accumulate_mapped: bad combine");
  ChanMap m;
  for (int d = 0; d < C; ++d) {
    PYTC_REQUIRE(chan_src[d] >= 0 && chan_src[d] < C, "blend_accumulate_mapped: bad source channel %d", chan_src[d]);
    m.src[d] = chan_src[d]; m.sz[d] = chan_shift[3 * d]; m.sy[d] = chan_shift[3 * d + 1]; m.sx[d] = chan_shift[3 * d + 2];
  }
  const long per_win = (long)rz * ry * rx;
  dim3 grid(ceil_div(per_win, 256)), block(256);
  hipStream_t s = (hipStream_t)stream;
  const int bz = border ? border[0] : 0, by = border ? border[1] : 0, bx = border ? border[2] : 0;
  PYTC_REQUIRE(bz >= 0 && by >= 0 && bx >= 0 && 2 * bz < rz && 2 * by < ry && 2 * bx < rx,
               "blend_accumulate_mapped: border mask too large for the window");
// ... 127 lines not shown
```

### pytorch_connectomics_amd/hip_ops.py

```python
from __future__ import annotations

import ctypes as C
from typing import Optional, Sequence

import torch

from . import _native as nat

_DT = {torch.float32: nat.F32, torch.bfloat16: nat.BF16}


def dtype_code(dt: torch.dtype) -> int:
    try:
        return _DT[dt]
    except KeyError:
        raise TypeError(f"pytorch_connectomics_amd kernels support float32/bfloat16, got {dt}") from None


def require_device(device, what: str = "this inference path") -> None:
    if torch.device(device).type != "cuda":
        raise RuntimeError(f"{what} (pytorch_connectomics_amd) needs a CUDA(HIP) device: there is no CPU path")


def _on_device(t: torch.Tensor, name: str) -> torch.Tensor:
    if not isinstance(t, torch.Tensor) or not t.is_cuda:
        raise RuntimeError(f"{name} must be a CUDA(HIP) tensor: pytorch_connectomics_amd has no CPU path")
    return t


def _dev(t: torch.Tensor, name: str) -> torch.Tensor:
    _on_device(t, name)
    if not t.is_contiguous():
        raise RuntimeError(f"{name} must be contiguous")
    return t


def _p(t: Optional[torch.Tensor]):
    return C.c_void_p(t.data_ptr()) if t is not None else None


_raw_stream = getattr(torch._C, "_cuda_getCurrentRawStream", None)
_raw_device = getattr(torch._C, "_cuda_getDevice", None)


def _stream():
    if _raw_stream is not None and _raw_device is not None:
        return C.c_void_p(_raw_stream(_raw_device()))
    return C.c_void_p(torch.cuda.current_stream().cuda_stream)


class _Profiler:
    def __init__(self):
        self.enabled = False
        self.records = []

    def summary(self):
# ... 49 lines not shown
    nat.check(st, name)


def _nbytes(*ts) -> int:
    return sum(t.numel() * t.element_size() for t in ts if t is not None)


def _starts_array(starts: Sequence[Sequence[int]], windows: Optional[int] = None):
    if windows is not None and len(starts) != int(windows):
        raise ValueError(f"{int(windows)} window predictions for {len(starts)} window positions: the network must keep the batch size")
    flat = [int(v) for s in starts for v in s]
    return (C.c_int32 * len(flat))(*flat)


def _f32_operand(t, name: str, *, shape=None, numel: Optional[int] = None) -> None:
    if not isinstance(t, torch.Tensor) or not t.is_cuda or t.dtype != torch.float32 or not t.is_contiguous():
        raise ValueError(f"{name} must be a contiguous float32 CUDA(HIP) tensor")
    if shape is not None and tuple(t.shape) != tuple(shape):
        raise ValueError(f"{name} must have shape {tuple(shape)}, got {tuple(t.shape)}")
    if numel is not None and t.numel() != numel:
        raise ValueError(f"{name} must have {numel} elements, got {t.numel()}")


def _window_operands(name: str, roi, weight, wshape, wz, wy, wx) -> None:
    for t, n, ax in ((wz, roi[0], "wz"), (wy, roi[1], "wy"), (wx, roi[2], "wx")):
        _f32_operand(t, f"{name}: {ax}", shape=(int(n),))
    if weight is not None:
        _f32_operand(weight, f"{name}: weight", shape=wshape)


def gather_windows(vol: torch.Tensor, starts, roi, *, view: int = 0, pad_mode: str = "constant",
                   cval: float = 0.0, out_dtype: torch.dtype = torch.float32,
                   out: Optional[torch.Tensor] = None) -> torch.Tensor:
    _dev(vol, "vol")
    if vol.dtype != torch.float32 or vol.dim() != 4:
        raise ValueError("vol must be float32 with shape (C, Z, Y, X)")
    Cc, Z, Y, X = vol.shape
    B = len(starts)
    rz, ry, rx = (int(v) for v in roi)
    if out is None:
        out = torch.empty((B, rz, ry, rx, Cc), dtype=out_dtype, device=vol.device)
    elif (not isinstance(out, torch.Tensor) or not out.is_cuda or not out.is_contiguous() or out.dtype not in _DT
          or tuple(out.shape) != (B, rz, ry, rx, Cc)):
        raise ValueError(f"gather_windows: out must be a contiguous float32 / bfloat16 CUDA(HIP) tensor of shape {(B, rz, ry, rx, Cc)}")
    st = _starts_array(starts)
    for b0 in range(0, B, 64):
        nb = min(64, B - b0)
        sub = (C.c_int32 * (3 * nb)).from_buffer(st, 4 * 3 * b0)
        o = out[b0:b0 + nb]
        _run("gather_windows", 2 * _nbytes(o) if o.dtype == torch.float32 else 3 * _nbytes(o),
             nat.lib().pytc_gather_windows, _p(vol), Cc, Z, Y, X, sub, nb, rz, ry, rx, int(view),
             nat.PAD_MODES[pad_mode], float(cval), _p(o), dtype_code(out.dtype), _stream())
    return out


def blend_accumulate(pred: torch.Tensor, starts, value: torch.Tensor, weight: Optional[torch.Tensor],
                     wz: torch.Tensor, wy: torch.Tensor, wx: torch.Tensor, *, view: int = 0,
                     combine: int = nat.BLEND_PRODUCT, floor_w: float = 1e-5, border=None) -> None:
    _dev(pred, "pred"); _dev(value, "value")
    B, rz, ry, rx, Cc = pred.shape
    if value.dtype != torch.float32 or value.shape[0] != Cc:
        raise ValueError("value accumulator must be float32 (C, Z, Y, X) with C matching pred")
    _, Z, Y, X = value.shape
    _window_operands("blend_accumulate", (rz, ry, rx), weight, (Z, Y, X), wz, wy, wx)
    st = _starts_array(starts, B)
    bd = (C.c_int32 * 3)(*[int(v) for v in border]) if border else None
    win = B * rz * ry * rx
    _run("blend_accumulate", _nbytes(pred) + win * 4 * (2 * Cc + (2 if weight is not None else 0)),
         nat.lib().pytc_blend_accumulate, _p(pred), dtype_code(pred.dtype), B, st, rz, ry, rx, Cc, int(view),
         _p(wz), _p(wy), _p(wx), int(combine), float(floor_w), bd, _p(value), _p(weight), Z, Y, X, _stream())


def blend_accumulate_mapped(pred: torch.Tensor, starts, value: torch.Tensor, weight: Optional[torch.Tensor],
                            wz: torch.Tensor, wy: torch.Tensor, wx: torch.Tensor, chan_src, chan_shift, *, view: int = 0,
                            combine: int = nat.BLEND_PRODUCT, floor_w: float = 1e-5, border=None) -> None:
    _dev(pred, "pred"); _dev(value, "value")
    B, rz, ry, rx, Cc = pred.shape
    if value.dtype != torch.float32 or value.shape[0] != Cc:
        raise ValueError("value accumulator must be float32 (C, Z, Y, X) with C matching pred")
    if len(chan_src) != Cc or len(chan_shift) != Cc:
        raise ValueError("channel map must describe every output channel")
    _, Z, Y, X = value.shape
    _window_operands("blend_accumulate_mapped", (rz, ry, rx), weight, (Z, Y, X), wz, wy, wx)
    st = _starts_array(starts, B)
    bd = (C.c_int32 * 3)(*[int(v) for v in border]) if border else None
    cs = (C.c_int32 * Cc)(*[int(v) for v in chan_src])
    sh = (C.c_int32 * (3 * Cc))(*[int(v) for s3 in chan_shift for v in s3])
    win = B * rz * ry * rx
    _run("blend_accumulate_mapped", _nbytes(pred) + win * 4 * (2 * Cc + (2 if weight is not None else 0)),
         nat.lib().pytc_blend_accumulate_mapped, _p(pred), dtype_code(pred.dtype), B, st, rz, ry, rx, Cc, int(view),
         _p(wz), _p(wy), _p(wx), int(combine), float(floor_w), bd, cs, sh, _p(value), _p(weight), Z, Y, X, _stream())


def blend_weight_shifted(starts, roi, weight: torch.Tensor, wz, wy, wx, shift, *, combine: int = nat.BLEND_PRODUCT,
                         floor_w: float = 1e-5, border=None) -> None:
    _on_device(weight, "weight")
    if weight.dim() != 3 or len(roi) != 3 or len(shift) != 3:
        raise ValueError("blend_weight_shifted: weight must be (Z, Y, X), roi and shift three integers")
    Z, Y, X = weight.shape
    _window_operands("blend_weight_shifted", roi, weight, (Z, Y, X), wz, wy, wx)
    st = _starts_array(starts)
    B = len(starts)
    bd = (C.c_int32 * 3)(*[int(v) for v in border]) if border else None
    sh = (C.c_int32 * 3)(*[int(v) for v in shift])
    _run("blend_weight_shifted", B * int(roi[0]) * int(roi[1]) * int(roi[2]) * 8, nat.lib().pytc_blend_weight_shifted, B, st,
         int(roi[0]), int(roi[1]), int(roi[2]), _p(wz), _p(wy), _p(wx), int(combine), float(floor_w), bd, sh, _p(weight),
# ... 481 lines not shown
         c_out, int(x.dtype == torch.float16), int(gelu), _p(res), _p(res_low), _p(res_bias), int(res_mode), *(int(v) for v in grid),
         _stream(), flops=2 * N * rows_per_sample * c_in * c_out, symbol="pw_gemm_lds_kernel")
    return y


def pw_mlp_up_supported(c_in: int, c_hid: int, c_out: int) -> bool:
    return bool(nat.lib().pytc_pw_mlp_up_supported(int(c_in), int(c_hid), int(c_out)))


def pw_mlp_up(x_low: torch.Tensor, taps: torch.Tensor, dw_bias: Optional[torch.Tensor], ab: torch.Tensor, w2p: torch.Tensor,
              b2: torch.Tensor, w3p: torch.Tensor, b3: torch.Tensor, skip: torch.Tensor, *, c_hid: int, c_out: int,
              res_low: Optional[torch.Tensor] = None, res_bias: Optional[torch.Tensor] = None) -> torch.Tensor:
    _dev(x_low, "x_low"); _dev(skip, "skip"); _dev(taps, "taps")
    if x_low.dtype != torch.bfloat16 or skip.dtype != torch.bfloat16:
        raise TypeError("pw_mlp_up runs on bfloat16 activations")
    N, D, H, W, c_in = x_low.shape
    if tuple(skip.shape) != (N, 2 * D, 2 * H, 2 * W, c_out):
        raise ValueError(f"pw_mlp_up: skip shape {tuple(skip.shape)} does not match the up-sampled grid")
    y = torch.empty((N, 2 * D, 2 * H, 2 * W, c_out), dtype=torch.bfloat16, device=x_low.device)
    a = nat.MlpArgs()
    a.t, a.ab, a.w2_packed, a.b2, a.w3_packed, a.b3 = (x_low.data_ptr(), ab.data_ptr(), w2p.data_ptr(), b2.data_ptr(),
                                                       w3p.data_ptr(), b3.data_ptr())
    if w3p.dtype != torch.bfloat16:
        raise TypeError("pw_mlp_up takes the bf16 image of the projection weights")
    a.res = skip.data_ptr()
    if dw_bias is None:
        dw_bias = torch.zeros((c_in,), dtype=torch.float32, device=x_low.device)
    if res_bias is None:
        res_bias = torch.zeros((c_out,), dtype=torch.float32, device=x_low.device)
    a.res_low = res_low.data_ptr() if res_low is not None else None
    a.res_bias = res_bias.data_ptr()
    a.y = y.data_ptr()
    a.N, a.rows_per_sample, a.C_in, a.C_hid, a.C_out, a.res_mode = N, 8 * D * H * W, c_in, c_hid, c_out, nat.RES_UPSAMPLE
    a.Di, a.Hi, a.Wi = D, H, W
    nb = _nbytes(x_low, skip, y) + (_nbytes(res_low) if res_low is not None else 0)
    _run(f"pw_mlp_up_fwd[{c_in}->{c_hid}->{c_out}]", nb, nat.lib().pytc_pw_mlp_up_fwd, C.byref(a), _p(taps), _p(dw_bias),
         _stream())
    return y


def stem_dwconv3d_supported(c_in: int, c: int, K: int) -> bool:
    return bool(nat.lib().pytc_stem_dwconv3d_supported(int(c_in), int(c), int(K)))


def stem_dwconv3d_pack(stem_w: torch.Tensor, stem_b: torch.Tensor, w_taps: torch.Tensor, bias: Optional[torch.Tensor]):
    wx = (w_taps * stem_w.view(1, -1)).contiguous()
    wb = (w_taps * stem_b.view(1, -1)).contiguous()
    cst = (wb.sum(0) + (bias if bias is not None else 0.0)).contiguous()
    image = torch.empty((nat.lib().pytc_stem_dwconv3d_mfma_image_bytes(),), dtype=torch.uint8, device=wx.device)
    _run("stem_dwconv3d_pack_mfma", 0, nat.lib().pytc_stem_dwconv3d_pack_mfma, _p(wx), _p(wb), _p(cst), _p(image), _stream())
    return wx, wb, cst, image


def stem_dwconv3d(x: torch.Tensor, packed):
    wx, wb, cst, image = packed
    _dev(x, "x"); _dev(wx, "wx")
    if x.dtype != torch.float32 or x.shape[-1] != 1:
        raise TypeError("stem_dwconv3d takes the 1-channel fp32 network input")
    N, D, H, W, _ = x.shape
    Cc = wx.shape[1]
    y = torch.empty((N, D, H, W, Cc), dtype=torch.bfloat16, device=x.device)
    slots = nat.lib().pytc_stem_dwconv3d_stat_slots(D, H, W)
    st = torch.empty((N, slots, 2, Cc), dtype=torch.float32, device=x.device)
    _run(f"stem_dwconv3d_fwd[C{Cc}_k3]", _nbytes(x, y), nat.lib().pytc_stem_dwconv3d_fwd, _p(x), _p(wx), _p(wb), _p(cst),
         _p(image), _p(y), _p(st), N, D, H, W, Cc, _stream())
    return y, st


def pw_mlp_stemres(t: torch.Tensor, ab: torch.Tensor, w2p: torch.Tensor, b2: torch.Tensor, w3p: torch.Tensor, b3: torch.Tensor,
                   x0: torch.Tensor, stem_w: torch.Tensor, stem_b: torch.Tensor, *, N: int, rows_per_sample: int, c_in: int,
                   c_hid: int, c_out: int, y: Optional[torch.Tensor] = None) -> torch.Tensor:
    _dev(t, "t"); _dev(x0, "x0")
    if t.dtype != torch.bfloat16 or x0.dtype != torch.float32:
        raise TypeError("pw_mlp_stemres: bf16 activations and the fp32 network input")
    if y is None:
        y = torch.empty((N, rows_per_sample, c_out), dtype=torch.bfloat16, device=t.device)
    else:
        _check_out(y, N * rows_per_sample * c_out, torch.bfloat16, "pw_mlp_stemres")
    a = nat.MlpArgs()
    a.t, a.ab, a.w2_packed, a.b2, a.w3_packed, a.b3 = (t.data_ptr(), None if ab is None else ab.data_ptr(), w2p.data_ptr(),
                                                       b2.data_ptr(), w3p.data_ptr(), b3.data_ptr())
    a.per_sample = _folded_operands(ab, w2p, b2, N, c_in, c_hid)
    a.w3_format = _w3_format(w3p)
    a.res = a.res_low = a.res_bias = None
    a.y = y.data_ptr()
    a.N, a.rows_per_sample, a.C_in, a.C_hid, a.C_out, a.res_mode = N, rows_per_sample, c_in, c_hid, c_out, nat.RES_ADD
    a.Di = a.Hi = a.Wi = 0
    nb = N * rows_per_sample * (2 * (c_in + c_out) + 4)
    _run(f"pw_mlp_fwd[{c_in}->{c_hid}->{c_out}]", nb, nat.lib().pytc_pw_mlp_stemres_fwd, C.byref(a), _p(x0), _p(stem_w),
         _p(stem_b), _stream(), symbol=_mlp_symbol(a, f"pw_mlp_kernel<{c_in // 32}, {c_out // 16}>+stemres", 1))
    return y


_MLP_BWD_CONSTS: dict = {}


def pw_mlp_bwd(dy: torch.Tensor, hidden_pre: torch.Tensor, w3t_p: torch.Tensor, w2t_p: torch.Tensor, *, N: int,
               rows_per_sample: int, c_in: int, c_hid: int, c_out: int):
    _dev(dy, "dy"); _dev(hidden_pre, "hidden_pre")
    if dy.dtype != torch.bfloat16:
        raise TypeError("pw_mlp_bwd runs on bfloat16 activations")
    dev = dy.device
    dx = torch.empty((N, rows_per_sample, c_in), dtype=torch.bfloat16, device=dev)
    dh = torch.empty((N, rows_per_sample, c_hid), dtype=torch.bfloat16, device=dev)
    key = (dev, N, c_in, c_hid, c_out)
    consts = _MLP_BWD_CONSTS.get(key)
    if consts is None:
        consts = (torch.cat([torch.ones((N, 1, c_out), device=dev), torch.zeros((N, 1, c_out), device=dev)], 1).contiguous(),
                  torch.zeros((c_hid,), device=dev), torch.zeros((c_in,), device=dev))
        _MLP_BWD_CONSTS[key] = consts
    ident, zh, zi = consts
    a = nat.MlpArgs()
    a.t, a.ab, a.w2_packed, a.b2, a.w3_packed, a.b3 = (dy.data_ptr(), ident.data_ptr(), w3t_p.data_ptr(), zh.data_ptr(),
                                                       w2t_p.data_ptr(), zi.data_ptr())
    a.w3_format = nat.W3_BF16
    a.res = a.res_low = a.res_bias = None
    a.y = dx.data_ptr()
    a.N, a.rows_per_sample, a.C_in, a.C_hid, a.C_out, a.res_mode = N, rows_per_sample, c_out, c_hid, c_in, nat.RES_NONE
    a.Di = a.Hi = a.Wi = 0
    nb = N * rows_per_sample * 2 * (c_out + 2 * c_hid + c_in)
    _run(f"pw_mlp_bwd[{c_out}->{c_hid}->{c_in}]", nb, nat.lib().pytc_pw_mlp_bwd, C.byref(a), _p(hidden_pre), _p(dh), _stream())
    return dx, dh


def pw_mlp_proj_supported(c_in: int, c_hid: int, c_out: int, c_proj: int) -> bool:
    return bool(nat.lib().pytc_pw_mlp_proj_supported(int(c_in), int(c_hid), int(c_out), int(c_proj)))


def pw_mlp_proj(t: torch.Tensor, w2n: torch.Tensor, b2n: torch.Tensor, w3p: torch.Tensor, b3: torch.Tensor, proj_w: torch.Tensor,
                proj_b: Optional[torch.Tensor], *, N: int, rows_per_sample: int, c_in: int, c_hid: int, c_out: int,
                res: Optional[torch.Tensor] = None, store_y: bool = False):
    _dev(t, "t"); _dev(proj_w, "proj_w")
    if t.dtype != torch.bfloat16 or proj_w.dtype != torch.bfloat16 or proj_w.numel() != 32 * 32:
        raise TypeError("pw_mlp_proj runs on bfloat16 activations and the paired bf16 image of a 32 x 32 projection")
    y = torch.empty((N, rows_per_sample, c_out), dtype=torch.bfloat16, device=t.device) if store_y else None
    z = torch.empty((N, rows_per_sample, 32), dtype=torch.bfloat16, device=t.device)
    a = nat.MlpArgs()
    a.t, a.ab, a.w2_packed, a.b2, a.w3_packed, a.b3 = t.data_ptr(), None, w2n.data_ptr(), b2n.data_ptr(), w3p.data_ptr(), b3.data_ptr()
    a.per_sample = _folded_operands(None, w2n, b2n, N, c_in, c_hid)
    a.w3_format = _w3_format(w3p)
    a.res = res.data_ptr() if res is not None else None
    a.res_low = a.res_bias = None
    a.y = y.data_ptr() if y is not None else None
# ... 1563 lines not shown
```

### pytorch_connectomics_amd/inference/window.py

```python
from __future__ import annotations

import logging
import os
from collections.abc import Mapping
from typing import Callable, Optional, Sequence, Tuple, Union

import torch

from .. import _native as nat
from .. import hip_ops as ops

logger = logging.getLogger(__name__)

_DISTANCE_TRANSFORM_BLEND_MODES = {"distance", "distance_transform", "distance-transform",
                                   "distance_transform_cdt", "banis", "banis_distance"}


def _cfg_value(obj, key: str, default=None):
    if obj is None:
        return default
    if isinstance(obj, Mapping):
        return obj.get(key, default)
    return getattr(obj, key, default)

# ... 347 lines not shown
        image_size = tuple(max(int(image_size[i]), self.roi_size[i]) for i in range(len(self.roi_size)))
        interval = compute_scan_interval(image_size, self.roi_size, overlap=self.overlap)
        return image_size, dense_patch_slices(image_size, self.roi_size, interval, return_slice=False)

    def _run_network(self, network, batch_cl: torch.Tensor) -> torch.Tensor:
        fwd_cl = getattr(network, "forward_cl", None)
        if fwd_cl is not None:
            y = fwd_cl(batch_cl)
        else:
            x = batch_cl.permute(0, 4, 1, 2, 3)
            if batch_cl.shape[-1] != 1:
                x = x.contiguous()
            y = network(x)
            if not isinstance(y, torch.Tensor):
                raise ValueError("EagerSlidingWindowEngine: `network` must return a torch.Tensor; "
                                 f"got {type(y).__name__}.")
            if tuple(y.shape[2:]) != self.roi_size:
                raise ValueError(f"network must preserve the ROI shape {self.roi_size}, got {tuple(y.shape[2:])}")
            y = y.permute(0, 2, 3, 4, 1).contiguous()
        if y.dtype not in (torch.float32, torch.bfloat16):
            y = y.float()
        return y.contiguous()

    def _check_inputs(self, inputs: torch.Tensor):
        nd = len(self.roi_size)
        if nd != 3:
            raise NotImplementedError("the MI355X engine handles 3-D ROIs (use roi (1,H,W) for 2-D data)")
        if inputs.dim() < nd + 2:
            raise ValueError("EagerSlidingWindowEngine: inputs must have shape (B, C, *spatial); "
                             f"got shape {tuple(inputs.shape)} for roi_size {self.roi_size}.")
        if inputs.shape[0] != 1:
            raise ValueError(f"EagerSlidingWindowEngine currently expects batch size 1; got batch {inputs.shape[0]}.")
        dev = torch.device(self.sw_device) if self.sw_device else inputs.device
        if dev.type != "cuda":
            raise RuntimeError("EagerSlidingWindowEngine (pytorch_connectomics_amd) needs a CUDA(HIP) device: "
                               "there is no CPU path")
        return dev

    @torch.no_grad()
    def accumulate(self, vol: torch.Tensor, network, *, view: int = 0, value: Optional[torch.Tensor] = None,
                   weight: Optional[torch.Tensor] = None, add_weight: bool = True, starts=None, chan_map=None):
        dev = vol.device
        orig = tuple(int(v) for v in vol.shape[1:])
        image_size, all_starts = self.plan(orig)
        if starts is None:
            starts = all_starts
        (wz, wy, wx), combine = self._axis_vectors(dev)
        roi = self.roi_size
        for bit, (a0, a1) in nat.VIEW_SWAPS.items():
            if (view & bit) and roi[a0] != roi[a1]:
                raise ValueError(f"a TTA view rotated in the plane of spatial axes ({a0}, {a1}) needs a window of equal size along them, "
                                 f"got roi {tuple(roi)}" + (" (a yx-rotated TTA view needs a window that is square in (y, x))" if bit == nat.VIEW_SWAP_YX else ""))

        def run(batch_starts):
            x = ops.gather_windows(vol, batch_starts, roi, view=view, pad_mode="constant", cval=self.cval)
            return self._run_network(network, x)

        on_gpu = dev.type == "cuda"
        before = torch.cuda.memory_allocated(dev) if on_gpu else 0
        peak_before = torch.cuda.max_memory_allocated(dev) if on_gpu else 0
        probe = run(starts[:1])
        peak = torch.cuda.max_memory_allocated(dev) if on_gpu else 0
        self._probe_bytes = max(0, peak - before) if peak > peak_before else 0
        c_out = int(probe.shape[-1])
        if value is None:
            value = torch.zeros((c_out,) + image_size, dtype=torch.float32, device=dev)
        if weight is None:
            weight = torch.zeros(image_size, dtype=torch.float32, device=dev)
            add_weight = True
        wacc = weight if add_weight else None

        def blend(pred, batch_starts):
            if chan_map is None:
                ops.blend_accumulate(pred, batch_starts, value, wacc, wz, wy, wx, view=view, combine=combine, floor_w=1e-5)
            else:
                ops.blend_accumulate_mapped(pred, batch_starts, value, wacc, wz, wy, wx, chan_map[0], chan_map[1],
                                            view=view, combine=combine, floor_w=1e-5)

        blend(probe, starts[:1])
        rest = starts[1:]
        chunks = [rest[b0:b0 + self.sw_batch_size] for b0 in range(0, len(rest), self.sw_batch_size)]
        lanes = self._lanes(dev, len(chunks), network)
        if not lanes:
            for chunk in chunks:
                blend(run(chunk), chunk)
        else:
            main = torch.cuda.current_stream(dev)
            for s in lanes:
                s.wait_stream(main)
            order_ev = None
            try:
                for i, chunk in enumerate(chunks):
                    s = lanes[i % len(lanes)]
                    with torch.cuda.stream(s):
                        pred = run(chunk)
                        if order_ev is not None:
                            s.wait_event(order_ev)
                        blend(pred, chunk)
                        order_ev = torch.cuda.Event()
                        order_ev.record(s)
                    del pred
            finally:
                for s in lanes:
                    main.wait_stream(s)
        self.last_stats = {"windows": len(starts), "roi": roi, "image_size": image_size, "streams": max(1, len(lanes))}
        return value, weight

# ... 59 lines not shown
```

### pytorch_connectomics_amd/models/architectures/mednext.py

```python
from __future__ import annotations

import os
from typing import Dict, List, Optional, Sequence, Union

import torch
import torch.nn as nn

from ... import _native as nat
from ... import hip_ops as ops

SMALL_ROWS_TWO_GEMMS = int(os.environ.get("PYTC_MIXER_TWO_GEMM_ROWS", "0"))

L0_SUBBATCH = int(os.environ.get("PYTC_L0_SUBBATCH", "0"))


def _conv_nd(dim: str):
    if dim == "3d":
        return nn.Conv3d, nn.ConvTranspose3d
    if dim == "2d":
        return nn.Conv2d, nn.ConvTranspose2d
    raise ValueError(f"dim must be '2d' or '3d', got {dim!r}")


class _ChannelLayerNorm(nn.Module):
# ... 281 lines not shown
            h = ops.pw_conv(t, self._pw_paired(m.conv2), self._vec(m.conv2, "bias", m.conv2.bias), N=N, rows_per_sample=rows,
                            c_in=C, c_out=c_hid, out_dtype=dt, ab=ab, w_paired=True)
            w3, b3 = self._pw_paired(m.conv3), self._vec(m.conv3, "bias", m.conv3.bias)
            G = dict(pre_act=nat.ACT_GELU, w_paired=True)
        else:
            h = ops.pw_conv(t, self._pw(m.conv2, dt), self._vec(m.conv2, "bias", m.conv2.bias), N=N,
                            rows_per_sample=rows, c_in=C, c_out=c_hid, out_dtype=dt, ab=ab, act=nat.ACT_GELU)
            if m.grn:
                h = self._grn(m, h, N, (Do, Ho, Wo), c_hid, kind)
            w3, b3 = self._pw(m.conv3, dt), self._vec(m.conv3, "bias", m.conv3.bias)
        if kind == "block":
            y = ops.pw_conv(h, w3, b3, N=N, rows_per_sample=rows, c_in=c_hid, c_out=c_out, out_dtype=dt,
                            res=x if m.do_res else None, res_mode=nat.RES_ADD if m.do_res else nat.RES_NONE, **G)
        elif kind == "down":
            res = None
            if m.resample_do_res:
                res = ops.pw_conv(x, self._pw(m.res_conv, dt), self._vec(m.res_conv, "bias", m.res_conv.bias),
                                  N=N, rows_per_sample=rows, c_in=C, c_out=c_out, out_dtype=dt, gather=2,
                                  grid=(D, H, W))
            y = ops.pw_conv(h, w3, b3, N=N, rows_per_sample=rows, c_in=c_hid, c_out=c_out, out_dtype=dt,
                            res=res, res_mode=nat.RES_ADD if res is not None else nat.RES_NONE, **G)
        else:
            if skip is None:
                skip = torch.zeros((N, Do, Ho, Wo, c_out), dtype=dt, device=x.device)
            res_low = res_bias = None
            if m.resample_do_res:
                res_bias = self._vec(m.res_conv, "bias", m.res_conv.bias)
                res_low = ops.pw_conv(x, self._pw(m.res_conv, dt, transposed=True), res_bias, N=N,
                                      rows_per_sample=D * H * W, c_in=C, c_out=c_out, out_dtype=dt)
            y = ops.pw_conv(h, w3, b3, N=N, rows_per_sample=rows, c_in=c_hid, c_out=c_out, out_dtype=dt,
                            res=skip, res_mode=nat.RES_UPSAMPLE, grid=(Do, Ho, Wo), res_low=res_low,
                            res_bias=res_bias, **G)
        return y.view(N, Do, Ho, Wo, c_out)


def _block_dwmix(self, m, x, taps, b1, c_hid, c_out, head=None, out=None):
    N, D, H, W, C = x.shape
    _, st = ops.dwconv3d(x, taps, b1, K=3, store=False)
    w2n, b2n = ops.groupnorm_fold_mlp(st, float(D * H * W), self._vec(m.norm, "weight", m.norm.weight), self._vec(m.norm, "bias", m.norm.bias),
                                      m.norm.eps, self._w2_matrix(m.conv2), self._vec(m.conv2, "bias", m.conv2.bias))
    w3, b3 = self._pw_paired(m.conv3, project=True), self._vec(m.conv3, "bias", m.conv3.bias)
    if head is not None:
        _, logits = ops.dwmix(x, taps, b1, w2n, b2n, w3, b3, c_hid=c_hid, c_out=c_out, residual=bool(m.do_res),
                              head_w=self._head_w(head), head_b=self._vec(head, "bias", head.bias), store_y=False)
        return None, logits
    if out is not None and tuple(out.shape) != (N, D, H, W, c_out):
        raise ValueError(f"block output buffer {tuple(out.shape)} != {(N, D, H, W, c_out)}")
    return ops.dwmix(x, taps, b1, w2n, b2n, w3, b3, c_hid=c_hid, c_out=c_out, residual=bool(m.do_res), y=out)


HipBlockOps._block_dwmix = None


def _stem_block_fused(self, stem: nn.Module, m, x_cl: torch.Tensor, out: Optional[torch.Tensor] = None) -> Optional[torch.Tensor]:
    N, D, H, W, cin = x_cl.shape
    C = stem.weight.shape[0]
    K = m.conv1.weight.shape[-1]
    if (cin != 1 or x_cl.dtype != torch.float32 or stem.bias is None or m.kind != "block" or not m.do_res or m.grn
            or not isinstance(m.norm, nn.GroupNorm) or m.dim != "3d" or m.conv2.bias is None or m.conv3.bias is None
            or m.conv1.weight.shape[0] != C or W % 4 != 0 or not ops.stem_dwconv3d_supported(cin, C, K)):
        return None
    c_hid, c_out = m.conv2.weight.shape[0], m.conv3.weight.shape[0]
    if c_out != C or not ops.pw_mlp_supported(C, c_hid, c_out):
        return None
    sw = self.cache.get(("stemw", id(stem)), [stem.weight], lambda: stem.weight.detach().float().reshape(-1).bfloat16().float().contiguous())
    sb = self._vec(stem, "bias", stem.bias)
    taps, _ = self._taps(m.conv1)
    packed = self.cache.get(("stemdw", id(stem), id(m.conv1)), [stem.weight, stem.bias, m.conv1.weight, m.conv1.bias],
                            lambda: ops.stem_dwconv3d_pack(sw, sb, taps, self._vec(m.conv1, "bias", m.conv1.bias)))
    t, st = ops.stem_dwconv3d(x_cl, packed)
    rows = D * H * W
    ab, w2x, b2x = self._fold(m, st, float(rows), C, c_hid)
    y = ops.pw_mlp_stemres(t, ab, w2x, b2x,
                           self._pw_paired(m.conv3, project=True), self._vec(m.conv3, "bias", m.conv3.bias), x_cl.reshape(N, rows), sw, sb,
                           N=N, rows_per_sample=rows, c_in=C, c_hid=c_hid, c_out=c_out,
                           y=None if out is None else out.view(N, rows, c_out))
    return y.view(N, D, H, W, c_out)


HipBlockOps._stem_block_fused = None


def _block_fused(self, m, x, t, ab, skip, ishape, oshape, c_hid, c_out, out=None, w2=None, b2=None):
    N, D, H, W, C = ishape
    Do, Ho, Wo = oshape
    rows = Do * Ho * Wo
    dt = torch.bfloat16
    if w2 is None:
        w2, b2 = self._pw_paired(m.conv2), self._vec(m.conv2, "bias", m.conv2.bias)
    w3, b3 = self._pw_paired(m.conv3, project=True), self._vec(m.conv3, "bias", m.conv3.bias)
    kw = dict(N=N, rows_per_sample=rows, c_in=C, c_hid=c_hid, c_out=c_out)
    if (self.lds_mixer_rows and N * rows >= self.lds_mixer_rows and w3.dtype == torch.float16
            and ops.pw_mlp_lds_supported(C, c_hid, c_out)):
        kw["lds"] = True
    chunk_ok = (self.chunk_mixer_rows and N * rows >= self.chunk_mixer_rows and w3.dtype == torch.float16
                and ops.pw_mlp_chunk_supported(C, c_hid, c_out))
    if chunk_ok and (c_hid >= self.chunk_mixer_hid or (C, c_out) == (128, 64)):
        kw.pop("lds", None)
        kw["chunked"] = True
    if out is not None:
        if tuple(out.shape) != (N, Do, Ho, Wo, c_out):
            raise ValueError(f"block output buffer {tuple(out.shape)} != {(N, Do, Ho, Wo, c_out)}")
        kw["y"] = out.view(N, rows, c_out)
    if m.kind == "block":
        y = ops.pw_mlp(t, ab, w2, b2, w3, b3, res=x if m.do_res else None,
                       res_mode=nat.RES_ADD if m.do_res else nat.RES_NONE, **kw)
    elif m.kind == "down":
        res = None
        if m.resample_do_res:
            paired = ops.pw_conv_paired_supported(c_in=C, c_out=c_out, in_dtype=dt, out_dtype=dt, gather=2)
            wres = self._pw_paired(m.res_conv) if paired else self._pw(m.res_conv, dt)
            res = ops.pw_conv(x, wres, self._vec(m.res_conv, "bias", m.res_conv.bias), N=N, rows_per_sample=rows,
                              c_in=C, c_out=c_out, out_dtype=dt, gather=2, grid=(D, H, W), w_paired=paired)
        y = ops.pw_mlp(t, ab, w2, b2, w3, b3, res=res, res_mode=nat.RES_ADD if res is not None else nat.RES_NONE, **kw)
    else:
        if skip is None:
            skip = torch.zeros((N, Do, Ho, Wo, c_out), dtype=dt, device=x.device)
        res_low = res_bias = None
        if m.resample_do_res:
            res_bias = self._vec(m.res_conv, "bias", m.res_conv.bias)
            paired = ops.pw_conv_paired_supported(c_in=C, c_out=c_out, in_dtype=dt, out_dtype=dt)
            wres = self._pw_paired(m.res_conv, transposed=True) if paired else self._pw(m.res_conv, dt, transposed=True)
            res_low = ops.pw_conv(x, wres, res_bias, N=N, rows_per_sample=D * H * W, c_in=C, c_out=c_out,
                                  out_dtype=dt, w_paired=paired)
        y = ops.pw_mlp(t, ab, w2, b2, w3, b3, res=skip, res_mode=nat.RES_UPSAMPLE, grid=(Do, Ho, Wo),
                       res_low=res_low, res_bias=res_bias, **kw)
    return y.view(N, Do, Ho, Wo, c_out)


# ... 118 lines not shown
        self.stem = conv(in_channels, n, kernel_size=1)

        def blocks(c, r, k, count):
            return nn.Sequential(*[MedNeXtBlock(c, c, r, k, do_res, norm_type, dim=dim, grn=grn)
                                   for _ in range(count)])

        for lvl in range(4):
            setattr(self, f"enc_block_{lvl}", blocks(n << lvl, exp_r[lvl], enc_kernel_size, block_counts[lvl]))
            setattr(self, f"down_{lvl}", MedNeXtDownBlock(n << lvl, n << (lvl + 1), exp_r[lvl + 1], enc_kernel_size,
                                                          do_res=do_res_up_down, norm_type=norm_type, dim=dim, grn=grn))
        self.bottleneck = blocks(n << 4, exp_r[4], dec_kernel_size, block_counts[4])
        for i, lvl in enumerate((3, 2, 1, 0)):
            setattr(self, f"up_{lvl}", MedNeXtUpBlock(n << (lvl + 1), n << lvl, exp_r[5 + i], dec_kernel_size,
                                                      do_res=do_res_up_down, norm_type=norm_type, dim=dim, grn=grn))
            setattr(self, f"dec_block_{lvl}", blocks(n << lvl, exp_r[5 + i], dec_kernel_size, block_counts[5 + i]))
        self.out_0 = OutBlock(n, n_classes, dim)
        self.dummy_tensor = nn.Parameter(torch.tensor([1.0]), requires_grad=True)
        if deep_supervision:
            for h in (1, 2, 3, 4):
                setattr(self, f"out_{h}", OutBlock(n << h, n_classes, dim))
        self.block_counts = list(block_counts)
        self.compute_dtype: Optional[torch.dtype] = None
        self._hip = HipBlockOps()
        self.fuse_head = True
        self.fuse_stem = True
        self.l0_subbatch = L0_SUBBATCH

    def _check_input(self, x: torch.Tensor):
        if not x.is_cuda:
            raise RuntimeError("MedNeXt (pytorch_connectomics_amd) runs only on an MI355X/ROCm device: "
                               "there is no CPU path. Move the model and input to 'cuda'.")
        if self.dim == "2d":
            if x.dim() not in (4, 5) or (x.dim() == 5 and x.shape[2] != 1):
                raise ValueError(f"MedNeXt dim='2d' takes (B,C,H,W) (or (B,C,1,H,W)) inputs, got {tuple(x.shape)}")
        elif x.dim() != 5:
            raise ValueError(f"MedNeXt dim='3d' takes (B,C,D,H,W) inputs, got {tuple(x.shape)}")
        spatial = x.shape[-2:] if self.dim == "2d" else x.shape[2:]
        if any(int(v) % 16 for v in spatial):
            raise ValueError(f"MedNeXt needs spatial sizes divisible by 16, got {tuple(spatial)}")

    def _lift(self, x: torch.Tensor):
        if self.dim == "2d" and x.dim() == 4:
            return x.unsqueeze(2), True
        return x, False

    @staticmethod
    def _drop(y, was_4d: bool):
        if not was_4d:
            return y
        if isinstance(y, list):
            return [v.squeeze(2) for v in y]
        return y.squeeze(2)

    def features_cl(self, x_cl: torch.Tensor, collect: Optional[List[torch.Tensor]] = None,
                    head: Optional[nn.Module] = None, proj: Optional[nn.Module] = None):
        hip = self._hip
        dt = resolve_compute_dtype(self.compute_dtype)
        spatial = x_cl.shape[2:4] if self.dim == "2d" else x_cl.shape[1:4]
        if any(int(v) % 16 for v in spatial) or (self.dim == "2d" and x_cl.shape[1] != 1):
            raise ValueError(f"MedNeXt needs spatial sizes divisible by 16, got {tuple(x_cl.shape[1:4])}"
                             + (" (dim='2d': depth must be 1)" if self.dim == "2d" else ""))
        enc0 = list(self.enc_block_0)
        N = int(x_cl.shape[0])
        sb = int(self.l0_subbatch)
        chained = 0 < sb < N and dt == torch.bfloat16 and hip.fused and self.dim == "3d"
        fuse_stem = self.fuse_stem and hip.fused and dt == torch.bfloat16 and bool(enc0)

        def level0_encoder(xs: torch.Tensor, skip_out: Optional[torch.Tensor], down_out: Optional[torch.Tensor]):
            blocks = list(enc0)
            h = None
            if fuse_stem:
                h = hip._stem_block_fused(self.stem, blocks[0], xs, skip_out if len(blocks) == 1 else None)
                if h is not None:
                    blocks = blocks[1:]
            if h is None:
                h = hip.pointwise(xs, self.stem, out_dtype=dt)
                if not blocks and skip_out is not None:
                    h = skip_out.copy_(h)
            for bi, blk in enumerate(blocks):
                h = hip.block(blk, h, out=skip_out if bi == len(blocks) - 1 else None)
            return h, hip.block(self.down_0, h, out=down_out)

        def level0_decoder(xl: torch.Tensor, sk: torch.Tensor, y_out: Optional[torch.Tensor] = None):
            h = hip.block(self.up_0, xl, skip=sk)
            blocks = list(self.dec_block_0)
            for bi, blk in enumerate(blocks):
                last = bi == len(blocks) - 1
                h = hip.block(blk, h, head=head if last else None, out=y_out if last else None, proj=proj if last else None)
            if not blocks and y_out is not None:
                h = y_out.copy_(h)
            return h

        skips = []
        if chained:
            _, D0, H0, W0, _ = x_cl.shape
            c0, c1 = self.stem.weight.shape[0], self.down_0.conv3.weight.shape[0]
            skip0 = torch.empty((N, D0, H0, W0, c0), dtype=dt, device=x_cl.device)
            x = torch.empty((N, D0 // 2, H0 // 2, W0 // 2, c1), dtype=dt, device=x_cl.device)
            for s0 in range(0, N, sb):
                level0_encoder(x_cl[s0:s0 + sb], skip0[s0:s0 + sb], x[s0:s0 + sb])
            skips.append(skip0)
        else:
            h, x = level0_encoder(x_cl, None, None)
            skips.append(h)
        for lvl in range(1, 4):
            for blk in getattr(self, f"enc_block_{lvl}"):
                x = hip.block(blk, x)
            skips.append(x)
            x = hip.block(getattr(self, f"down_{lvl}"), x)
        for blk in self.bottleneck:
            x = hip.block(blk, x)
        if collect is not None:
            collect.append(x)
        for lvl in (3, 2, 1):
            x = hip.block(getattr(self, f"up_{lvl}"), x, skip=skips[lvl])
            for blk in getattr(self, f"dec_block_{lvl}"):
                x = hip.block(blk, x)
            if collect is not None:
                collect.append(x)
        if not chained:
            return level0_decoder(x, skips[0])
        first = level0_decoder(x[0:sb], skips[0][0:sb])
        if isinstance(first, tuple):
            parts = [first[1]] + [level0_decoder(x[s0:s0 + sb], skips[0][s0:s0 + sb])[1] for s0 in range(sb, N, sb)]
            return None, torch.cat(parts, 0)
        y0 = torch.empty((N,) + tuple(first.shape[1:]), dtype=first.dtype, device=first.device)
        y0[0:sb].copy_(first)
        for s0 in range(sb, N, sb):
            level0_decoder(x[s0:s0 + sb], skips[0][s0:s0 + sb], y0[s0:s0 + sb])
        return y0

    def output_cl(self, feat_cl: torch.Tensor, head: int = 0) -> torch.Tensor:
        return self._hip.pointwise(feat_cl, getattr(self, f"out_{head}").conv_out, out_dtype=torch.float32,
                                   transposed=True)

    def forward_cl(self, x_cl: torch.Tensor):
        out = self.features_cl(x_cl, head=self.out_0.conv_out if self.fuse_head else None)
        if isinstance(out, tuple):
            return out[1]
        return self.output_cl(out)

    def forward_features(self, x: torch.Tensor) -> torch.Tensor:
        self._check_input(x)
        x, flat = self._lift(x)
        return self._drop(to_channels_first(self.features_cl(to_channels_last(x.float())).float()), flat)

    def forward_output(self, features: torch.Tensor) -> torch.Tensor:
        if not features.is_cuda:
            raise RuntimeError("forward_output needs a CUDA tensor: there is no CPU path")
        dt = resolve_compute_dtype(self.compute_dtype)
        features, flat = self._lift(features)
        return self._drop(to_channels_first(self.output_cl(to_channels_last(features).to(dt))), flat)

    def _autograd_active(self) -> bool:
        return torch.is_grad_enabled() and any(p.requires_grad for p in self.parameters())

    def forward(self, x: torch.Tensor):
        self._check_input(x)
        x, flat = self._lift(x)
        return self._drop(self._forward5(x), flat)

    def _forward5(self, x: torch.Tensor):
        if self._autograd_active():
            from ...training.autograd import mednext_train_forward
            out = mednext_train_forward(self, to_channels_last(x.float()), resolve_compute_dtype(self.compute_dtype))
            if isinstance(out, list):
                return [to_channels_first(o) for o in out]
            return to_channels_first(out)
        if not self.do_ds:
            return to_channels_first(self.forward_cl(to_channels_last(x.float())))
        feats: Optional[List[torch.Tensor]] = []
        f = self.features_cl(to_channels_last(x.float()), collect=feats)
        out = to_channels_first(self.output_cl(f))
        ds = [to_channels_first(self.output_cl(ft, h)) for ft, h in zip(feats, (4, 3, 2, 1))]
        return [out, ds[3], ds[2], ds[1], ds[0]]


def create_mednext_v1(num_input_channels: int, num_classes: int, model_id: str, kernel_size: int = 3,
                      deep_supervision: bool = False) -> MedNeXt:
    table = {
        "S": dict(exp_r=2, block_counts=[2] * 9, checkpoint_style=None),
        "B": dict(exp_r=[2, 3, 4, 4, 4, 4, 4, 3, 2], block_counts=[2] * 9, checkpoint_style=None),
        "M": dict(exp_r=[2, 3, 4, 4, 4, 4, 4, 3, 2], block_counts=[3, 4, 4, 4, 4, 4, 4, 4, 3],
                  checkpoint_style="outside_block"),
        "L": dict(exp_r=[3, 4, 8, 8, 8, 8, 8, 4, 3], block_counts=[3, 4, 8, 8, 8, 8, 8, 4, 3],
                  checkpoint_style="outside_block"),
    }
    if model_id not in table:
        raise ValueError(f"model_id must be one of S, B, M, L; got {model_id!r}")
    return MedNeXt(in_channels=num_input_channels, n_channels=32, n_classes=num_classes,
# ... 7 lines not shown
```

### pytorch_connectomics_amd/models/architectures/mednext_models.py

```python
from __future__ import annotations

import os

from dataclasses import dataclass
from typing import Any, Dict, Mapping, Optional, Union

import torch
import torch.nn as nn
import torch.nn.functional as F

from .base import ConnectomicsModel
from .mednext import (MedNeXt as MedNeXtBase, MedNeXtBlock, create_mednext_v1, to_channels_first,
                      to_channels_last)
from .registry import register_architecture

MEDNEXT_AVAILABLE = True


class MedNeXtWrapper(ConnectomicsModel):

    def __init__(self, model: nn.Module, deep_supervision: bool = False):
        super().__init__()
        self.model = model
        self.supports_deep_supervision = deep_supervision
        self.output_scales = 5 if deep_supervision else 1

    def forward(self, x: torch.Tensor) -> Union[torch.Tensor, Dict[str, torch.Tensor]]:
        outputs = self.model(x)
        if self.supports_deep_supervision and isinstance(outputs, list):
            return {"output": outputs[0], "ds_1": outputs[1], "ds_2": outputs[2], "ds_3": outputs[3],
                    "ds_4": outputs[4]}
        return outputs

    def forward_cl(self, x_cl: torch.Tensor) -> torch.Tensor:
        return self.model.forward_cl(x_cl)


def _cfg_value(cfg: Any, key: str, default: Any = None) -> Any:
    return cfg.get(key, default) if isinstance(cfg, Mapping) else getattr(cfg, key, default)


_NORM_NAME = {nn.GroupNorm: "group"}


def _infer_mednext_head_block_kwargs(model: nn.Module) -> dict:
    blocks = getattr(model, "dec_block_0", None)
    if blocks is None or len(blocks) == 0:
        raise ValueError("MedNeXt trunk must expose a non-empty dec_block_0 to build task heads.")
    ref = blocks[0]
    if not isinstance(ref, MedNeXtBlock):
        raise TypeError("Expected MedNeXt dec_block_0 to contain MedNeXtBlock instances for multi-head reuse.")
    k = ref.conv1.kernel_size
    return dict(exp_r=ref.conv2.out_channels // ref.conv2.in_channels, kernel_size=int(k[0] if isinstance(k, tuple) else k),
                do_res=ref.do_res, norm_type=_NORM_NAME.get(type(ref.norm), "layer"), dim=ref.dim, grn=ref.grn)


MERGE_NARROW_HEADS = os.environ.get("PYTC_MERGE_HEADS", "1") != "0"
FUSE_MERGED_HEAD_PROJECTION = os.environ.get("PYTC_FUSE_MERGED_HEAD", "1") != "0"


@dataclass(frozen=True)
class _HeadSpec:
    out_channels: int
    num_blocks: int = 0
    hidden_channels: Optional[int] = None

    @classmethod
    def parse(cls, entry: Any) -> "_HeadSpec":
        hidden = _cfg_value(entry, "hidden_channels", None)
        return cls(int(_cfg_value(entry, "out_channels", entry)), int(_cfg_value(entry, "num_blocks", 0)),
                   None if hidden is None else int(hidden))

    def as_dict(self, feature_channels: int) -> dict:
        return {"out_channels": self.out_channels, "num_blocks": self.num_blocks,
                "hidden_channels": self.hidden_channels or feature_channels}


class MedNeXtTaskHead(nn.Module):

    def __init__(self, in_channels: int, out_channels: int, num_blocks: int, hidden_channels: int | None = None,
                 *, exp_r: int, kernel_size: int, do_res: bool, norm_type: str, dim: str, grn: bool):
        super().__init__()
        width = in_channels if hidden_channels is None else hidden_channels
        for ok, msg in (
                (num_blocks >= 0, f"MedNeXt task head num_blocks must be >= 0, got {num_blocks}"),
                (out_channels > 0, f"MedNeXt task head out_channels must be positive, got {out_channels}"),
                (width > 0, f"MedNeXt task head hidden_channels must be positive, got {width}"),
# ... 257 lines not shown
```

Measured before the change: 1.789 billion voxels/s.

## Read sliding-window batches directly from the volume in stem kernels

Adds a window-source path: the fused stem depthwise conv and the stem-residual MLP kernels compute addresses straight into the full input volume from per-window start offsets. This replaces the gather_windows step that packed the batch into a contiguous tensor. It removes one gather kernel and its write and reread of the packed batch for in-bounds windows. In exchange it adds per-row index arithmetic in the kernels, is limited to 64 windows with x-aligned starts, and falls back to gathering for windows near the border.

```diff
diff --git a/include/pytc_hip.h b/include/pytc_hip.h
--- a/include/pytc_hip.h
+++ b/include/pytc_hip.h
@@ -7,7 +7,7 @@
 extern "C" {
 #endif
 
-#define PYTC_ABI_VERSION 10
+#define PYTC_ABI_VERSION 11
 
 #define PYTC_OK 0
 #define PYTC_ERR_INVALID 1
@@ -219,6 +219,12 @@
 int pytc_pw_mlp_head_supported(int C_in, int C_hid, int C_out);
 int pytc_pw_mlp_stemres_fwd(const pytc_mlp_args* a, const float* stem_x, const float* stem_w, const float* stem_b,
                             void* stream);
+int pytc_window_source_ok(int C, int Z, int Y, int X, const int32_t* starts, int B, int rz, int ry, int rx, int view);
+int pytc_stem_dwconv3d_win_fwd(const float* vol, int Z, int Y, int X, const int32_t* starts, const float* wx, const float* wb,
+                               const float* cst, const void* mfma_image, void* y, float* stats, int N, int D, int H, int W, int C,
+                               void* stream);
+int pytc_pw_mlp_stemres_win_fwd(const pytc_mlp_args* a, const float* vol, int Z, int Y, int X, const int32_t* starts, int D, int H,
+                                int W, const float* stem_w, const float* stem_b, void* stream);
 int pytc_stem_dwconv3d_stat_slots(int D, int H, int W);
 int pytc_stem_dwconv3d_supported(int C_in, int C, int K);
 int pytc_stem_dwconv3d_mfma_image_bytes(void);
diff --git a/pytorch_connectomics_amd/_native.py b/pytorch_connectomics_amd/_native.py
--- a/pytorch_connectomics_amd/_native.py
+++ b/pytorch_connectomics_amd/_native.py
@@ -5,7 +5,7 @@
 from pathlib import Path
 
 LIB_PATH = Path(__file__).resolve().parent / "lib" / "libpytc_hip.so"
-ABI_VERSION = 10
+ABI_VERSION = 11
 
 F32, BF16 = 0, 1
 OK = 0
@@ -251,6 +251,11 @@
     "pytc_pw_mlp_chunk_supported": (C.c_int, [C.c_int, C.c_int, C.c_int]),
     "pytc_pw_mlp_chunk_fwd": (C.c_int, [C.POINTER(MlpArgs), C.c_void_p]),
     "pytc_pw_mlp_stemres_fwd": (C.c_int, [C.POINTER(MlpArgs), C.c_void_p, C.c_void_p, C.c_void_p, C.c_void_p]),
+    "pytc_window_source_ok": (C.c_int, [C.c_int, C.c_int, C.c_int, C.c_int, C.POINTER(C.c_int32), C.c_int, C.c_int, C.c_int, C.c_int, C.c_int]),
+    "pytc_stem_dwconv3d_win_fwd": (C.c_int, [C.c_void_p, C.c_int, C.c_int, C.c_int, C.POINTER(C.c_int32), C.c_void_p, C.c_void_p, C.c_void_p,
+                                             C.c_void_p, C.c_void_p, C.c_void_p, C.c_int, C.c_int, C.c_int, C.c_int, C.c_int, C.c_void_p]),
+    "pytc_pw_mlp_stemres_win_fwd": (C.c_int, [C.POINTER(MlpArgs), C.c_void_p, C.c_int, C.c_int, C.c_int, C.POINTER(C.c_int32), C.c_int, C.c_int,
+                                              C.c_int, C.c_void_p, C.c_void_p, C.c_void_p]),
     "pytc_stem_dwconv3d_stat_slots": (C.c_int, [C.c_int, C.c_int, C.c_int]),
     "pytc_stem_dwconv3d_supported": (C.c_int, [C.c_int, C.c_int, C.c_int]),
     "pytc_convT3d_thin_supported": (C.c_int, [C.c_int, C.c_int]),
diff --git a/pytorch_connectomics_amd/csrc/pw_mlp_kernels.hip b/pytorch_connectomics_amd/csrc/pw_mlp_kernels.hip
--- a/pytorch_connectomics_amd/csrc/pw_mlp_kernels.hip
+++ b/pytorch_connectomics_amd/csrc/pw_mlp_kernels.hip
@@ -1,5 +1,6 @@
 #include <cmath>
 #include "pw_common.h"
+#include "window_source.h"
 
 namespace pytc {
 
@@ -28,6 +29,17 @@
   const bf16_t* hp_in;
 };
 
+__device__ __forceinline__ const float* win_sample(const WinSrc& ws, int n) {
+  return ws.vol + ((long)ws.st.s[3 * n] * ws.zs + (long)ws.st.s[3 * n + 1] * ws.ys + ws.st.s[3 * n + 2]);
+}
+__device__ __forceinline__ const float* win_sample(const NoWinSrc&, int) { return nullptr; }
+__device__ __forceinline__ long win_row_offset(const WinSrc& ws, unsigned row) {
+  const unsigned line = row / (unsigned)ws.ww, x = row - line * (unsigned)ws.ww;
+  const unsigned z = line / (unsigned)ws.wh, y = line - z * (unsigned)ws.wh;
+  return (long)z * ws.zs + (long)y * ws.ys + x;
+}
+__device__ __forceinline__ long win_row_offset(const NoWinSrc&, unsigned) { return 0; }
+
 constexpr int mlp_waves_per_simd(int ks, int mo, int nt) {
   if (ks >= 8 && nt == 1) return 1;
   const int regs = ks * nt * 4 + mo * nt * 4 + 2 * nt * 4;
@@ -36,7 +48,7 @@
 
 template <int KS_IN, int MO, int NT, int GELU_MODE, bool HEAD = false, bool STEMRES = false, bool STOREH = false, bool BWD = false>
 __global__ void __launch_bounds__(256, mlp_waves_per_simd(KS_IN, MO, NT))
-pw_mlp_kernel(MlpParams p) {
+pw_mlp_kernel(MlpParams p, WinArg<STEMRES> ws = WinArg<STEMRES>{}) {
   constexpr int CIN = KS_IN * 32, COUT = MO * 16;
   static_assert(MO % 2 == 0, "C_out must be a multiple of 32");
   static_assert(!STEMRES || (MO == 2 && (MO / 2) * NT <= 4), "the stem-recomputing residual covers C_out = 32");
@@ -103,7 +115,8 @@
   uint4 rpre[PREFETCH_RES ? MO / 2 : 1][PREFETCH_RES ? NT : 1];
   const bool use_pre = PREFETCH_RES && p.e.res_mode != PYTC_RES_NONE;
   if constexpr (STEMRES) {
-    const float* sx = p.stem_x + (long)n * p.rps;
+    const bool win = ws.vol != nullptr;
+    const float* sx = win ? win_sample(ws, n) : p.stem_x + (long)n * p.rps;
     float sw[8], sb[8];
     VecIO<float, 4>::load(p.stem_w + kb * 8, reinterpret_cast<float(&)[4]>(sw[0]));
     VecIO<float, 4>::load(p.stem_w + kb * 8 + 4, reinterpret_cast<float(&)[4]>(sw[4]));
@@ -111,7 +124,8 @@
     VecIO<float, 4>::load(p.stem_b + kb * 8 + 4, reinterpret_cast<float(&)[4]>(sb[4]));
 #pragma unroll
     for (int nt = 0; nt < NT; ++nt) {
-      const float xv = sx[orow[nt] < p.rps ? orow[nt] : p.rps - 1];
+      const long rr = orow[nt] < p.rps ? orow[nt] : p.rps - 1;
+      const float xv = sx[win ? win_row_offset(ws, (unsigned)rr) : rr];
       float rv[8];
 #pragma unroll
       for (int j = 0; j < 8; ++j) rv[j] = fmaf(sw[j], xv, sb[j]);
@@ -301,9 +315,9 @@
 
 template <int HCT, int KIND>
 __global__ void __launch_bounds__(256, 3)
-pw_mlp_dma_kernel(MlpParams p, int waves_per_sample) {
+pw_mlp_dma_kernel(MlpParams p, int waves_per_sample, WinArg<KIND == 4> ws) {
   constexpr int NT = 4, CIN = 32, COUT = 32;
-  constexpr bool STEM = KIND == 1, HEAD = KIND == 2, PROJ = KIND == 3;
+  constexpr bool WIN = KIND == 4, STEM = KIND == 1 || WIN, HEAD = KIND == 2, PROJ = KIND == 3;
   __shared__ __attribute__((aligned(16))) uint4 land[4][2][NT * 64];
   __shared__ __attribute__((aligned(16))) uint4 w2s[HCT * 2 * 64], w3s[2 * HCT * 64];
   __shared__ __attribute__((aligned(16))) float b2s[HCT * 32], b3s[32];
@@ -315,7 +329,7 @@
   const bool with_res = STEM || p.e.res_mode == PYTC_RES_ADD;
   const bf16_t* tn = p.t + (long)n * p.rps * CIN;
   const bf16_t* resn = (!STEM && with_res) ? reinterpret_cast<const bf16_t*>(p.e.res) + (long)n * p.rps * COUT : nullptr;
-  const float* sx = STEM ? p.stem_x + (long)n * p.rps : nullptr;
+  const float* sx = STEM ? (WIN ? win_sample(ws, n) : p.stem_x + (long)n * p.rps) : nullptr;
   bf16_t* yn = reinterpret_cast<bf16_t*>(p.e.y) + (long)n * p.rps * COUT;
   float* hy = HEAD ? p.head_y + (long)n * p.rps * p.n_head : nullptr;
   bf16_t* zn = PROJ ? p.proj_y + (long)n * p.rps * 32 : nullptr;
@@ -342,14 +356,36 @@
   asm volatile("s_waitcnt vmcnt(0)" ::: "memory");
 
   const unsigned lbase = __builtin_amdgcn_readfirstlane((unsigned)(size_t)(__attribute__((address_space(3))) void*)&land[wave][0][0]);
+  int qz = 0, qy = 0, qx = 0, dz = 0, dy = 0, dx = 0, wh = 1, ww = 1;
+  long wzs = 0, wys = 0;
+  if constexpr (WIN) {
+    wh = ws.wh; ww = ws.ww; wzs = ws.zs; wys = ws.ys;
+    const unsigned first = (unsigned)__builtin_amdgcn_readfirstlane((int)((blockIdx.x * 4 + wave) * (NT * 16)));
+    const unsigned step = (unsigned)waves_per_sample * (NT * 16);
+    const unsigned fl = first / (unsigned)ww, sl = step / (unsigned)ww;
+    qx = (int)(first - fl * (unsigned)ww); qz = (int)(fl / (unsigned)wh); qy = (int)(fl - (unsigned)qz * (unsigned)wh);
+    dx = (int)(step - sl * (unsigned)ww); dz = (int)(sl / (unsigned)wh); dy = (int)(sl - (unsigned)dz * (unsigned)wh);
+  }
   auto request = [&](long tile) {
 #pragma unroll
     for (int nt = 0; nt < NT; ++nt) {
       long row = tile * (NT * 16) + nt * 16 + r;
-      row = row < p.rps ? row : p.rps - 1;
+      const bool live = row < p.rps;
+      row = live ? row : p.rps - 1;
       glds16(tn + row * CIN + kb * 8, lbase + (unsigned)(nt * 64) * 16);
-      if constexpr (STEM) glds4(sx + row, lbase + (unsigned)(NT * 64) * 16 + (unsigned)(nt * 64) * 4);
+      if constexpr (STEM && WIN) {
+        int px = qx + nt * 16 + r, py = qy, pz = qz;
+        while (px >= ww) { px -= ww; ++py; }
+        while (py >= wh) { py -= wh; ++pz; }
+        const long off = live ? (long)pz * wzs + (long)py * wys + px : 0L;
+        glds4(sx + off, lbase + (unsigned)(NT * 64) * 16 + (unsigned)(nt * 64) * 4);
+      } else if constexpr (STEM) glds4(sx + row, lbase + (unsigned)(NT * 64) * 16 + (unsigned)(nt * 64) * 4);
       else if (with_res) glds16(resn + row * COUT + kb * 8, lbase + (unsigned)((NT + nt) * 64) * 16);
+    }
+    if constexpr (WIN) {
+      qx += dx; if (qx >= ww) { qx -= ww; ++qy; }
+      qy += dy; if (qy >= wh) { qy -= wh; ++qz; }
+      qz += dz;
     }
   };
   bf16x8_t out[NT];
@@ -478,7 +514,7 @@
          (long)a->N * a->rows_per_sample >= (long)tuning_get(K_mlp_dma_rows);
 }
 template <int KIND>
-static void mlp_dma_launch(const pytc_mlp_args* a, const MlpParams& p, hipStream_t s) {
+static void mlp_dma_launch(const pytc_mlp_args* a, const MlpParams& p, hipStream_t s, const WinArg<KIND == 4>& ws = WinArg<KIND == 4>{}) {
   const long tiles = (a->rows_per_sample + 63) / 64;
   long wgs = (3072 + a->N - 1) / a->N;
   const long most = (tiles / 2 + 3) / 4;
@@ -486,9 +522,9 @@
   if (const int forced = tuning_get(K_mlp_dma_wgs); forced > 0) wgs = forced;
   dim3 grid((unsigned)wgs, (unsigned)a->N), block(256);
   const int wps = (int)(wgs * 4);
-  if (p.HC == 2) hipLaunchKernelGGL((pw_mlp_dma_kernel<2, KIND>), grid, block, 0, s, p, wps);
-  else if (p.HC == 3) hipLaunchKernelGGL((pw_mlp_dma_kernel<3, KIND>), grid, block, 0, s, p, wps);
-  else hipLaunchKernelGGL((pw_mlp_dma_kernel<4, KIND>), grid, block, 0, s, p, wps);
+  if (p.HC == 2) hipLaunchKernelGGL((pw_mlp_dma_kernel<2, KIND>), grid, block, 0, s, p, wps, ws);
+  else if (p.HC == 3) hipLaunchKernelGGL((pw_mlp_dma_kernel<3, KIND>), grid, block, 0, s, p, wps, ws);
+  else hipLaunchKernelGGL((pw_mlp_dma_kernel<4, KIND>), grid, block, 0, s, p, wps, ws);
 }
 
 template <typename OUT>
@@ -820,9 +856,9 @@
   return PYTC_OK;
 }
 
-extern "C" int pytc_pw_mlp_stemres_fwd(const pytc_mlp_args* a, const float* stem_x, const float* stem_w, const float* stem_b,
-                                       void* stream) {
-  PYTC_REQUIRE(a && a->t && (a->ab || a->per_sample) && a->w2_packed && a->w3_packed && a->b2 && a->b3 && a->y && stem_x && stem_w && stem_b,
+static int mlp_stemres_launch(const pytc_mlp_args* a, const float* stem_x, const WinSrc* ws, const float* stem_w, const float* stem_b,
+                              void* stream) {
+  PYTC_REQUIRE(a && a->t && (a->ab || a->per_sample) && a->w2_packed && a->w3_packed && a->b2 && a->b3 && a->y && (stem_x || ws) && stem_w && stem_b,
                "pw_mlp_stemres: null pointer");
   PYTC_REQUIRE(!(a->ab && a->per_sample), "pw_mlp_stemres: per-sample (norm-folded) expand operands come without an affine");
   PYTC_REQUIRE(a->N >= 1 && a->rows_per_sample >= 1, "pw_mlp_stemres: bad shape");
@@ -846,14 +882,35 @@
   pytc_mlp_args shape = *a;
   shape.res_mode = PYTC_RES_NONE;
   if (mlp_dma_applies(&shape, p)) {
-    mlp_dma_launch<1>(a, p, s);
+    if (ws) mlp_dma_launch<4>(a, p, s, *ws);
+    else mlp_dma_launch<1>(a, p, s);
     PYTC_LAUNCH_CHECK("pw_mlp_stemres_dma");
     return PYTC_OK;
   }
-  if (p.w3_f16) hipLaunchKernelGGL((pw_mlp_kernel<1, 2, 4, 3, false, true>), grid, block, 0, s, p);
-  else hipLaunchKernelGGL((pw_mlp_kernel<1, 2, 4, 1, false, true>), grid, block, 0, s, p);
+  const WinSrc src = ws ? *ws : WinSrc{};
+  if (p.w3_f16) hipLaunchKernelGGL((pw_mlp_kernel<1, 2, 4, 3, false, true>), grid, block, 0, s, p, src);
+  else hipLaunchKernelGGL((pw_mlp_kernel<1, 2, 4, 1, false, true>), grid, block, 0, s, p, src);
   PYTC_LAUNCH_CHECK("pw_mlp_stemres");
   return PYTC_OK;
+}
+
+extern "C" int pytc_pw_mlp_stemres_fwd(const pytc_mlp_args* a, const float* stem_x, const float* stem_w, const float* stem_b,
+                                       void* stream) {
+  PYTC_REQUIRE(stem_x, "pw_mlp_stemres: null pointer");
+  return mlp_stemres_launch(a, stem_x, nullptr, stem_w, stem_b, stream);
+}
+
+extern "C" int pytc_pw_mlp_stemres_win_fwd(const pytc_mlp_args* a, const float* vol, int Z, int Y, int X, const int32_t* starts, int D,
+                                           int H, int W, const float* stem_w, const float* stem_b, void* stream) {
+  PYTC_REQUIRE(a && vol && starts, "pw_mlp_stemres_win: null pointer");
+  PYTC_REQUIRE(window_source_ok(1, 1, Z, Y, X, starts, a->N, D, H, W, 0) && ((uintptr_t)vol & 15) == 0 &&
+                   a->rows_per_sample == (int64_t)D * H * W,
+               "pw_mlp_stemres_win: window source needs <= 64 windows of rows_per_sample voxels wholly inside the volume, x starts and x "
+               "extents multiples of 4, a 16-byte aligned volume (pytc_window_source_ok)");
+  WinSrc ws{};
+  ws.vol = vol; ws.zs = (long)Y * X; ws.ys = X; ws.wh = H; ws.ww = W;
+  memcpy(ws.st.s, starts, sizeof(int) * 3 * a->N);
+  return mlp_stemres_launch(a, nullptr, &ws, stem_w, stem_b, stream);
 }
 
 extern "C" int pytc_pw_mlp_dma_applies(const pytc_mlp_args* a, int ignore_res_mode) {
diff --git a/pytorch_connectomics_amd/csrc/pytc_common.h b/pytorch_connectomics_amd/csrc/pytc_common.h
--- a/pytorch_connectomics_amd/csrc/pytc_common.h
+++ b/pytorch_connectomics_amd/csrc/pytc_common.h
@@ -60,6 +60,7 @@
   X(norm_bwd_from_wgrad_flat, 1, "GroupNorm-backward epilogue of the expand weight gradient as one flat kernel; 0 = chunked")      \
   X(pw_gemm_rows, 0, "LDS-tiled 1x1 GEMM: 64 / 128 forces the rows per workgroup; 0 = by problem size")                            \
   X(pw_thin, 1, "plain 1x1 convs with one input / few output channels on the thin kernels; 0 = the generic kernel")                \
+  X(window_direct, 1, "stem kernels read in-volume window batches from the volume itself; 0 = gather_windows + packed form")      \
   X(wgrad_dgrad_fused, 1, "projecting conv's weight gradient and the GELU-backward data gradient in one kernel; 0 = two launches")  \
   X(wgrad_small_split, 1, "matrix-core 1x1 weight gradient: more, shorter row slots when the launch would leave CUs idle")         \
   X(wgrad_valu, 0, "1: 1x1 weight gradient on the VALU kernel instead of the matrix cores")                                        \
diff --git a/pytorch_connectomics_amd/csrc/stem_dwconv_kernels.hip b/pytorch_connectomics_amd/csrc/stem_dwconv_kernels.hip
--- a/pytorch_connectomics_amd/csrc/stem_dwconv_kernels.hip
+++ b/pytorch_connectomics_amd/csrc/stem_dwconv_kernels.hip
@@ -1,16 +1,28 @@
 #include "pytc_common.h"
+#include "window_source.h"
 
 namespace pytc {
 
 constexpr int SD_C = 32;
 
+template <bool WIN>
+__device__ __forceinline__ const float* stem_sample(const float* x, int n, int D, int H, int W, const WinArg<WIN>& ws, long& zs, long& ys) {
+  if constexpr (WIN) {
+    zs = ws.zs; ys = ws.ys;
+    return ws.vol + ((long)ws.st.s[3 * n] * ws.zs + (long)ws.st.s[3 * n + 1] * ws.ys + ws.st.s[3 * n + 2]);
+  } else {
+    zs = (long)H * W; ys = W;
+    return x + (long)n * ((long)D * H * W);
+  }
+}
+
 struct StemDw { int D, H, W, GX; long groups; };
 
 constexpr int SD_IT = 4;
-template <int SD_VX>
+template <int SD_VX, bool WIN = false>
 __global__ void __launch_bounds__(256)
 stem_dwconv_k3_kernel(const float* __restrict__ x, const float* __restrict__ wx, const float* __restrict__ wb,
-                      const float* __restrict__ cst, bf16_t* __restrict__ y, float* __restrict__ stats, StemDw g, int slots) {
+                      const float* __restrict__ cst, bf16_t* __restrict__ y, float* __restrict__ stats, StemDw g, int slots, WinArg<WIN> ws) {
   __shared__ __attribute__((aligned(16))) float lw[2 * 27 * SD_C + SD_C];
   __shared__ float red[16][256 + 4];
   for (int i = threadIdx.x; i < 27 * SD_C; i += 256) { lw[i] = wx[i]; lw[27 * SD_C + i] = wb[i]; }
@@ -23,7 +35,8 @@
   const int n = blockIdx.y;
   const int cg = threadIdx.x & 3, c0 = cg * 8;
   const long rps = (long)g.D * g.H * g.W;
-  const float* xn = x + (long)n * rps;
+  long zs, ys;
+  const float* xn = stem_sample<WIN>(x, n, g.D, g.H, g.W, ws, zs, ys);
   bf16_t* yn = y + (long)n * rps * SD_C;
   float s1[8], s2[8];
 #pragma unroll
@@ -54,7 +67,7 @@
       const int z = vz + dz, yy = vy + dy;
       const bool row_in = z >= 0 && z < g.D && yy >= 0 && yy < g.H;
       const int zc = z < 0 ? 0 : (z >= g.D ? g.D - 1 : z), yc = yy < 0 ? 0 : (yy >= g.H ? g.H - 1 : yy);
-      const float* row = xn + ((long)zc * g.H + yc) * g.W + x0;
+      const float* row = WIN ? xn + (long)zc * zs + (long)yc * ys + x0 : xn + ((long)zc * g.H + yc) * g.W + x0;
       const float lft = row[left_in ? -1 : 0], rgt = row[right_in ? SD_VX : SD_VX - 1];
       float in[SD_VX + 2];
       in[0] = (row_in && left_in) ? lft : 0.f;
@@ -152,10 +165,10 @@
   }
 }
 
-template <bool STORE_PERMUTE>
+template <bool STORE_PERMUTE, bool WIN = false>
 __global__ void __launch_bounds__(256, 4)
 stem_dwconv_k3_mfma_kernel(const float* __restrict__ x, const h8_t* __restrict__ frag, const float* __restrict__ kc,
-                           bf16_t* __restrict__ y, float* __restrict__ stats, StemMf g, int slots) {
+                           bf16_t* __restrict__ y, float* __restrict__ stats, StemMf g, int slots, WinArg<WIN> ws) {
   __shared__ __attribute__((aligned(16))) _Float16 hbuf[2 * SM_HALO];
   _Float16* const hx = hbuf;
   _Float16* const hin = hbuf + SM_HALO;
@@ -178,8 +191,13 @@
   const bool left_in = x0 > 0, right_in = x0 + SM_XT < g.W;
   const bool xy_border = !left_in || !right_in || y0 == 0 || y0 + SM_YT >= g.H;
   const long rps = (long)g.D * g.H * g.W;
-  const float* xn = x + (long)n * rps;
+  long zs, ys;
+  const float* xn = stem_sample<WIN>(x, n, g.D, g.H, g.W, ws, zs, ys);
   bf16_t* yn = y + (long)n * rps * SD_C;
+  auto row_at = [&](int cz, int cy) -> const float* {
+    if constexpr (WIN) return xn + (long)cz * zs + (long)cy * ys;
+    else return xn + ((long)cz * g.H + cy) * g.W;
+  };
 
   typedef const __attribute__((address_space(3))) _Float16* lds_h_ptr;
   lds_h_ptr tp[8];
@@ -204,14 +222,14 @@
       const int r = it >> 2, p = it & 3;
       const int gy = y0 - 1 + r % SM_EY, gz = z0 - 1 + r / SM_EY;
       const int cy = min(max(gy, 0), g.H - 1), cz = min(max(gz, 0), g.D - 1);
-      pre_v[u] = *reinterpret_cast<const float4*>(xn + ((long)cz * g.H + cy) * g.W + x0 + 4 * p);
+      pre_v[u] = *reinterpret_cast<const float4*>(row_at(cz, cy) + x0 + 4 * p);
     }
     {
       const int it = min(tid, N_EDGE - 1);
       const int r = it >> 1, right = it & 1;
       const int gy = y0 - 1 + r % SM_EY, gz = z0 - 1 + r / SM_EY;
       const int cy = min(max(gy, 0), g.H - 1), cz = min(max(gz, 0), g.D - 1);
-      pre_e = xn[((long)cz * g.H + cy) * g.W + x0 + (right ? (right_in ? SM_XT : SM_XT - 1) : (left_in ? -1 : 0))];
+      pre_e = row_at(cz, cy)[x0 + (right ? (right_in ? SM_XT : SM_XT - 1) : (left_in ? -1 : 0))];
     }
   };
   auto stage_commit = [&](int z0, bool border) {
@@ -354,26 +372,56 @@
   return PYTC_OK;
 }
 
-extern "C" int pytc_stem_dwconv3d_fwd(const float* x, const float* wx, const float* wb, const float* cst, const void* mfma_image,
-                                      void* y, float* stats, int N, int D, int H, int W, int C, void* stream) {
-  PYTC_REQUIRE(x && wx && wb && cst && y && stats, "stem_dwconv3d: null pointer");
+static int stem_dwconv3d_launch(const float* x, const float* vol, int Z, int Y, int X, const int32_t* starts, const float* wx,
+                                const float* wb, const float* cst, const void* mfma_image, void* y, float* stats, int N, int D, int H,
+                                int W, int C, void* stream) {
+  PYTC_REQUIRE((x || vol) && wx && wb && cst && y && stats, "stem_dwconv3d: null pointer");
   PYTC_REQUIRE(N >= 1 && D >= 1 && H >= 1 && W >= 4 && C == SD_C, "stem_dwconv3d: C must be 32");
   PYTC_REQUIRE(W % 4 == 0, "stem_dwconv3d: W must be a multiple of 4");
+  WinSrc ws{};
+  if (vol) {
+    PYTC_REQUIRE(window_source_ok(1, 1, Z, Y, X, starts, N, D, H, W, 0) && ((uintptr_t)vol & 15) == 0,
+                 "stem_dwconv3d: window source needs <= 64 windows wholly inside the volume, x starts and x extents multiples of 4, a 16-byte "
+                 "aligned volume (pytc_window_source_ok)");
+    ws.vol = vol; ws.zs = (long)Y * X; ws.ys = X;
+    memcpy(ws.st.s, starts, sizeof(int) * 3 * N);
+  }
   const int slots = pytc_stem_dwconv3d_stat_slots(D, H, W);
   if (sd_mfma(D, H, W)) {
     PYTC_REQUIRE(mfma_image, "stem_dwconv3d: the f16-MFMA form needs the image of pytc_stem_dwconv3d_pack_mfma");
     StemMf m;
     sd_geom(m, D, H, W);
     const float* kc = (const float*)((const char*)mfma_image + SM_IMG_FRAG * 16);
-    hipLaunchKernelGGL(stem_dwconv_k3_mfma_kernel<true>, dim3(slots, N), dim3(256), 0, (hipStream_t)stream, x,
-                       (const h8_t*)mfma_image, kc, (bf16_t*)y, stats, m, slots);
+    if (vol)
+      hipLaunchKernelGGL((stem_dwconv_k3_mfma_kernel<true, true>), dim3(slots, N), dim3(256), 0, (hipStream_t)stream, x,
+                         (const h8_t*)mfma_image, kc, (bf16_t*)y, stats, m, slots, ws);
+    else
+      hipLaunchKernelGGL((stem_dwconv_k3_mfma_kernel<true, false>), dim3(slots, N), dim3(256), 0, (hipStream_t)stream, x,
+                         (const h8_t*)mfma_image, kc, (bf16_t*)y, stats, m, slots, NoWinSrc{});
     PYTC_LAUNCH_CHECK("stem_dwconv3d_mfma");
     return PYTC_OK;
   }
   const int vx = sd_vx(W);
   StemDw g{D, H, W, W / vx, (long)D * H * (W / vx)};
-  hipLaunchKernelGGL(stem_dwconv_k3_kernel<4>, dim3(slots, N), dim3(256), 0, (hipStream_t)stream, x, wx, wb, cst, (bf16_t*)y,
-                     stats, g, slots);
+  if (vol)
+    hipLaunchKernelGGL((stem_dwconv_k3_kernel<4, true>), dim3(slots, N), dim3(256), 0, (hipStream_t)stream, x, wx, wb, cst, (bf16_t*)y,
+                       stats, g, slots, ws);
+  else
+    hipLaunchKernelGGL((stem_dwconv_k3_kernel<4, false>), dim3(slots, N), dim3(256), 0, (hipStream_t)stream, x, wx, wb, cst, (bf16_t*)y,
+                       stats, g, slots, NoWinSrc{});
   PYTC_LAUNCH_CHECK("stem_dwconv3d");
   return PYTC_OK;
 }
+
+extern "C" int pytc_stem_dwconv3d_fwd(const float* x, const float* wx, const float* wb, const float* cst, const void* mfma_image,
+                                      void* y, float* stats, int N, int D, int H, int W, int C, void* stream) {
+  PYTC_REQUIRE(x, "stem_dwconv3d: null pointer");
+  return stem_dwconv3d_launch(x, nullptr, 0, 0, 0, nullptr, wx, wb, cst, mfma_image, y, stats, N, D, H, W, C, stream);
+}
+
+extern "C" int pytc_stem_dwconv3d_win_fwd(const float* vol, int Z, int Y, int X, const int32_t* starts, const float* wx, const float* wb,
+                                          const float* cst, const void* mfma_image, void* y, float* stats, int N, int D, int H, int W,
+                                          int C, void* stream) {
+  PYTC_REQUIRE(vol && starts, "stem_dwconv3d_win: null pointer");
+  return stem_dwconv3d_launch(nullptr, vol, Z, Y, X, starts, wx, wb, cst, mfma_image, y, stats, N, D, H, W, C, stream);
+}
diff --git a/pytorch_connectomics_amd/csrc/window_kernels.hip b/pytorch_connectomics_amd/csrc/window_kernels.hip
--- a/pytorch_connectomics_amd/csrc/window_kernels.hip
+++ b/pytorch_connectomics_amd/csrc/window_kernels.hip
@@ -1,4 +1,5 @@
 #include "pytc_common.h"
+#include "window_source.h"
 
 #pragma clang fp contract(off)
 
@@ -7,10 +8,6 @@
 __device__ __forceinline__ float mul_rn(float a, float b) { return a * b; }
 __device__ __forceinline__ float add_rn(float a, float b) { return a + b; }
 __device__ __forceinline__ float sub_rn(float a, float b) { return a - b; }
-
-struct StartList {
-  int s[64 * 3];
-};
 
 __device__ __forceinline__ int pad_index(int g, int lo, int hi, int mode, bool& inside) {
   inside = true;
@@ -336,7 +333,7 @@
                                    int B, int rz, int ry, int rx, int view, int pad_mode, float cval,
                                    void* out, int out_dtype, void* stream) {
   PYTC_REQUIRE(vol && out && starts, "gather_windows: null pointer");
-  PYTC_REQUIRE(B >= 1 && B <= 64, "gather_windows: B=%d must be in [1,64]", B);
+  PYTC_REQUIRE(B >= 1 && B <= WIN_BATCH_MAX, "gather_windows: B=%d must be in [1,64]", B);
   PYTC_REQUIRE(C >= 1 && rz > 0 && ry > 0 && rx > 0 && Z > 0 && Y > 0 && X > 0, "gather_windows: bad shape");
   PYTC_REQUIRE(view_ok(view, rz, ry, rx), "gather_windows: at most one SWAP bit, and the exchanged window axes must have equal length");
   PYTC_REQUIRE(pad_mode >= 0 && pad_mode <= 3, "gather_windows: bad pad_mode %d", pad_mode);
@@ -355,6 +352,10 @@
     PYTC_REQUIRE(false, "gather_windows: bad out_dtype %d", out_dtype);
   PYTC_LAUNCH_CHECK("gather_windows");
   return PYTC_OK;
+}
+
+extern "C" int pytc_window_source_ok(int C, int Z, int Y, int X, const int32_t* starts, int B, int rz, int ry, int rx, int view) {
+  return window_source_ok(tuning_get(K_window_direct), C, Z, Y, X, starts, B, rz, ry, rx, view) ? 1 : 0;
 }
 
 extern "C" int pytc_blend_accumulate(const void* pred, int pred_dtype, int B, const int32_t* starts, int rz,
diff --git a/pytorch_connectomics_amd/csrc/window_source.h b/pytorch_connectomics_amd/csrc/window_source.h
--- /dev/null
+++ b/pytorch_connectomics_amd/csrc/window_source.h
@@ -0,0 +1,38 @@
+#pragma once
+#include <stdint.h>
+
+namespace pytc {
+
+constexpr int WIN_BATCH_MAX = 64;
+
+struct StartList {
+  int s[WIN_BATCH_MAX * 3];
+};
+
+struct WinSrc {
+  const float* vol;
+  long zs;
+  int ys;
+  int wh, ww;
+  StartList st;
+};
+struct NoWinSrc {};
+template <bool WIN> struct WinArgOf { typedef NoWinSrc type; };
+template <> struct WinArgOf<true> { typedef WinSrc type; };
+template <bool WIN> using WinArg = typename WinArgOf<WIN>::type;
+
+inline bool window_source_ok(int enabled, int C, int Z, int Y, int X, const int32_t* starts, int B, int rz, int ry, int rx, int view) {
+  if (!enabled || !starts || C != 1 || view != 0) return false;
+  if (B < 1 || B > WIN_BATCH_MAX) return false;
+  if (rz < 1 || ry < 1 || rx < 4 || rx % 4 != 0 || X % 4 != 0) return false;
+  if (rz > Z || ry > Y || rx > X) return false;
+  if ((long)rz * ry * rx >= (1L << 31)) return false;
+  for (int b = 0; b < B; ++b) {
+    const int sz = starts[3 * b], sy = starts[3 * b + 1], sx = starts[3 * b + 2];
+    if (sz < 0 || sy < 0 || sx < 0 || sz > Z - rz || sy > Y - ry || sx > X - rx) return false;
+    if (sx % 4 != 0) return false;
+  }
+  return true;
+}
+
+}
diff --git a/pytorch_connectomics_amd/hip_ops.py b/pytorch_connectomics_amd/hip_ops.py
--- a/pytorch_connectomics_amd/hip_ops.py
+++ b/pytorch_connectomics_amd/hip_ops.py
@@ -1,7 +1,8 @@
 from __future__ import annotations
 
 import ctypes as C
-from typing import Optional, Sequence
+import math
+from typing import NamedTuple, Optional, Sequence
 
 import torch
 
@@ -157,6 +158,35 @@
              nat.lib().pytc_gather_windows, _p(vol), Cc, Z, Y, X, sub, nb, rz, ry, rx, int(view),
              nat.PAD_MODES[pad_mode], float(cval), _p(o), dtype_code(out.dtype), _stream())
     return out
+
+
+class WindowSource(NamedTuple):
+    vol: torch.Tensor
+    starts: Sequence[Sequence[int]]
+    roi: Sequence[int]
+
+    def gather(self) -> torch.Tensor:
+        return gather_windows(self.vol, self.starts, self.roi)
+
+    def narrow(self, b0: int, b1: int) -> "WindowSource":
+        return WindowSource(self.vol, self.starts[b0:b1], self.roi)
+
+
+def window_source_ok(vol: torch.Tensor, starts, roi, *, view: int = 0) -> bool:
+    if (not isinstance(vol, torch.Tensor) or not vol.is_cuda or vol.dtype != torch.float32 or vol.dim() != 4 or not vol.is_contiguous()
+            or vol.data_ptr() % 16 or not 1 <= len(starts) <= 64):
+        return False
+    Cc, Z, Y, X = vol.shape
+    rz, ry, rx = (int(v) for v in roi)
+    return bool(nat.lib().pytc_window_source_ok(Cc, Z, Y, X, _starts_array(starts), len(starts), rz, ry, rx, int(view)))
+
+
+def _window_source_args(ws: WindowSource, name: str):
+    _f32_operand(ws.vol, f"{name}: window source volume")
+    if ws.vol.dim() != 4 or ws.vol.shape[0] != 1 or ws.vol.data_ptr() % 16:
+        raise ValueError(f"{name}: the window source volume must be (1, Z, Y, X), 16-byte aligned")
+    _, Z, Y, X = ws.vol.shape
+    return _p(ws.vol), Z, Y, X, _starts_array(ws.starts)
 
 
 def blend_accumulate(pred: torch.Tensor, starts, value: torch.Tensor, weight: Optional[torch.Tensor],
@@ -744,26 +774,41 @@
     return wx, wb, cst, image
 
 
-def stem_dwconv3d(x: torch.Tensor, packed):
+def stem_dwconv3d(x: Optional[torch.Tensor], packed, *, window_source: Optional[WindowSource] = None):
     wx, wb, cst, image = packed
-    _dev(x, "x"); _dev(wx, "wx")
-    if x.dtype != torch.float32 or x.shape[-1] != 1:
-        raise TypeError("stem_dwconv3d takes the 1-channel fp32 network input")
-    N, D, H, W, _ = x.shape
+    _dev(wx, "wx")
     Cc = wx.shape[1]
-    y = torch.empty((N, D, H, W, Cc), dtype=torch.bfloat16, device=x.device)
+    if window_source is not None:
+        vp, Z, Y, X, starts = _window_source_args(window_source, "stem_dwconv3d")
+        N = len(window_source.starts)
+        D, H, W = (int(v) for v in window_source.roi)
+        dev, nin = window_source.vol.device, 4 * N * D * H * W
+    else:
+        _dev(x, "x")
+        if x.dtype != torch.float32 or x.shape[-1] != 1:
+            raise TypeError("stem_dwconv3d takes the 1-channel fp32 network input")
+        N, D, H, W, _ = x.shape
+        dev, nin = x.device, _nbytes(x)
+    y = torch.empty((N, D, H, W, Cc), dtype=torch.bfloat16, device=dev)
     slots = nat.lib().pytc_stem_dwconv3d_stat_slots(D, H, W)
-    st = torch.empty((N, slots, 2, Cc), dtype=torch.float32, device=x.device)
-    _run(f"stem_dwconv3d_fwd[C{Cc}_k3]", _nbytes(x, y), nat.lib().pytc_stem_dwconv3d_fwd, _p(x), _p(wx), _p(wb), _p(cst),
-         _p(image), _p(y), _p(st), N, D, H, W, Cc, _stream())
+    st = torch.empty((N, slots, 2, Cc), dtype=torch.float32, device=dev)
+    if window_source is not None:
+        _run(f"stem_dwconv3d_fwd[C{Cc}_k3]", nin + _nbytes(y), nat.lib().pytc_stem_dwconv3d_win_fwd, vp, Z, Y, X, starts, _p(wx), _p(wb),
+             _p(cst), _p(image), _p(y), _p(st), N, D, H, W, Cc, _stream())
+    else:
+        _run(f"stem_dwconv3d_fwd[C{Cc}_k3]", nin + _nbytes(y), nat.lib().pytc_stem_dwconv3d_fwd, _p(x), _p(wx), _p(wb), _p(cst),
+             _p(image), _p(y), _p(st), N, D, H, W, Cc, _stream())
     return y, st
 
 
 def pw_mlp_stemres(t: torch.Tensor, ab: torch.Tensor, w2p: torch.Tensor, b2: torch.Tensor, w3p: torch.Tensor, b3: torch.Tensor,
-                   x0: torch.Tensor, stem_w: torch.Tensor, stem_b: torch.Tensor, *, N: int, rows_per_sample: int, c_in: int,
-                   c_hid: int, c_out: int, y: Optional[torch.Tensor] = None) -> torch.Tensor:
-    _dev(t, "t"); _dev(x0, "x0")
-    if t.dtype != torch.bfloat16 or x0.dtype != torch.float32:
+                   x0: Optional[torch.Tensor], stem_w: torch.Tensor, stem_b: torch.Tensor, *, N: int, rows_per_sample: int, c_in: int,
+                   c_hid: int, c_out: int, y: Optional[torch.Tensor] = None,
+                   window_source: Optional[WindowSource] = None) -> torch.Tensor:
+    _dev(t, "t")
+    if window_source is None:
+        _dev(x0, "x0")
+    if t.dtype != torch.bfloat16 or (window_source is None and x0.dtype != torch.float32):
         raise TypeError("pw_mlp_stemres: bf16 activations and the fp32 network input")
     if y is None:
         y = torch.empty((N, rows_per_sample, c_out), dtype=torch.bfloat16, device=t.device)
@@ -779,8 +824,19 @@
     a.N, a.rows_per_sample, a.C_in, a.C_hid, a.C_out, a.res_mode = N, rows_per_sample, c_in, c_hid, c_out, nat.RES_ADD
     a.Di = a.Hi = a.Wi = 0
     nb = N * rows_per_sample * (2 * (c_in + c_out) + 4)
+    symbol = _mlp_symbol(a, f"pw_mlp_kernel<{c_in // 32}, {c_out // 16}>+stemres", 1)
+    if window_source is not None:
+        if symbol.startswith("pw_mlp_dma_kernel"):
+            symbol = symbol.replace(", 1>", ", 4>")
+        if len(window_source.starts) != N or math.prod(int(v) for v in window_source.roi) != rows_per_sample:
+            raise ValueError("pw_mlp_stemres: the window source must hold N windows of rows_per_sample voxels")
+        vp, Z, Y, X, starts = _window_source_args(window_source, "pw_mlp_stemres")
+        D, H, W = (int(v) for v in window_source.roi)
+        _run(f"pw_mlp_fwd[{c_in}->{c_hid}->{c_out}]", nb, nat.lib().pytc_pw_mlp_stemres_win_fwd, C.byref(a), vp, Z, Y, X, starts, D, H, W,
+             _p(stem_w), _p(stem_b), _stream(), symbol=symbol)
+        return y
     _run(f"pw_mlp_fwd[{c_in}->{c_hid}->{c_out}]", nb, nat.lib().pytc_pw_mlp_stemres_fwd, C.byref(a), _p(x0), _p(stem_w),
-         _p(stem_b), _stream(), symbol=_mlp_symbol(a, f"pw_mlp_kernel<{c_in // 32}, {c_out // 16}>+stemres", 1))
+         _p(stem_b), _stream(), symbol=symbol)
     return y
 
 
diff --git a/pytorch_connectomics_amd/inference/window.py b/pytorch_connectomics_amd/inference/window.py
--- a/pytorch_connectomics_amd/inference/window.py
+++ b/pytorch_connectomics_amd/inference/window.py
@@ -423,7 +423,12 @@
                 raise ValueError(f"a TTA view rotated in the plane of spatial axes ({a0}, {a1}) needs a window of equal size along them, "
                                  f"got roi {tuple(roi)}" + (" (a yx-rotated TTA view needs a window that is square in (y, x))" if bit == nat.VIEW_SWAP_YX else ""))
 
+        direct_net = bool(getattr(network, "accepts_window_source", False)) and getattr(network, "forward_cl", None) is not None
+
         def run(batch_starts):
+            if direct_net and ops.window_source_ok(vol, batch_starts, roi, view=view):
+                y = network.forward_cl(None, window_source=ops.WindowSource(vol, batch_starts, roi))
+                return (y if y.dtype in (torch.float32, torch.bfloat16) else y.float()).contiguous()
             x = ops.gather_windows(vol, batch_starts, roi, view=view, pad_mode="constant", cval=self.cval)
             return self._run_network(network, x)
 
diff --git a/pytorch_connectomics_amd/models/architectures/mednext.py b/pytorch_connectomics_amd/models/architectures/mednext.py
--- a/pytorch_connectomics_amd/models/architectures/mednext.py
+++ b/pytorch_connectomics_amd/models/architectures/mednext.py
@@ -357,11 +357,16 @@
 HipBlockOps._block_dwmix = None
 
 
-def _stem_block_fused(self, stem: nn.Module, m, x_cl: torch.Tensor, out: Optional[torch.Tensor] = None) -> Optional[torch.Tensor]:
-    N, D, H, W, cin = x_cl.shape
+def _stem_block_fused(self, stem: nn.Module, m, x_cl: Optional[torch.Tensor], out: Optional[torch.Tensor] = None,
+                      window_source=None) -> Optional[torch.Tensor]:
+    if window_source is not None:
+        N, (D, H, W), cin, in_dtype = len(window_source.starts), (int(v) for v in window_source.roi), 1, window_source.vol.dtype
+    else:
+        N, D, H, W, cin = x_cl.shape
+        in_dtype = x_cl.dtype
     C = stem.weight.shape[0]
     K = m.conv1.weight.shape[-1]
-    if (cin != 1 or x_cl.dtype != torch.float32 or stem.bias is None or m.kind != "block" or not m.do_res or m.grn
+    if (cin != 1 or in_dtype != torch.float32 or stem.bias is None or m.kind != "block" or not m.do_res or m.grn
             or not isinstance(m.norm, nn.GroupNorm) or m.dim != "3d" or m.conv2.bias is None or m.conv3.bias is None
             or m.conv1.weight.shape[0] != C or W % 4 != 0 or not ops.stem_dwconv3d_supported(cin, C, K)):
         return None
@@ -373,13 +378,14 @@
     taps, _ = self._taps(m.conv1)
     packed = self.cache.get(("stemdw", id(stem), id(m.conv1)), [stem.weight, stem.bias, m.conv1.weight, m.conv1.bias],
                             lambda: ops.stem_dwconv3d_pack(sw, sb, taps, self._vec(m.conv1, "bias", m.conv1.bias)))
-    t, st = ops.stem_dwconv3d(x_cl, packed)
+    t, st = ops.stem_dwconv3d(x_cl, packed, window_source=window_source)
     rows = D * H * W
     ab, w2x, b2x = self._fold(m, st, float(rows), C, c_hid)
     y = ops.pw_mlp_stemres(t, ab, w2x, b2x,
-                           self._pw_paired(m.conv3, project=True), self._vec(m.conv3, "bias", m.conv3.bias), x_cl.reshape(N, rows), sw, sb,
+                           self._pw_paired(m.conv3, project=True), self._vec(m.conv3, "bias", m.conv3.bias),
+                           None if window_source is not None else x_cl.reshape(N, rows), sw, sb,
                            N=N, rows_per_sample=rows, c_in=C, c_hid=c_hid, c_out=c_out,
-                           y=None if out is None else out.view(N, rows, c_out))
+                           y=None if out is None else out.view(N, rows, c_out), window_source=window_source)
     return y.view(N, D, H, W, c_out)
 
 
@@ -604,28 +610,36 @@
             return [v.squeeze(2) for v in y]
         return y.squeeze(2)
 
-    def features_cl(self, x_cl: torch.Tensor, collect: Optional[List[torch.Tensor]] = None,
-                    head: Optional[nn.Module] = None, proj: Optional[nn.Module] = None):
+    def features_cl(self, x_cl: Optional[torch.Tensor], collect: Optional[List[torch.Tensor]] = None,
+                    head: Optional[nn.Module] = None, proj: Optional[nn.Module] = None, window_source=None):
         hip = self._hip
         dt = resolve_compute_dtype(self.compute_dtype)
-        spatial = x_cl.shape[2:4] if self.dim == "2d" else x_cl.shape[1:4]
-        if any(int(v) % 16 for v in spatial) or (self.dim == "2d" and x_cl.shape[1] != 1):
-            raise ValueError(f"MedNeXt needs spatial sizes divisible by 16, got {tuple(x_cl.shape[1:4])}"
+        if window_source is not None:
+            if x_cl is not None:
+                raise ValueError("features_cl takes the packed batch or a window source, not both")
+            in_shape = (len(window_source.starts), *(int(v) for v in window_source.roi), 1)
+        else:
+            in_shape = tuple(x_cl.shape)
+        spatial = in_shape[2:4] if self.dim == "2d" else in_shape[1:4]
+        if any(int(v) % 16 for v in spatial) or (self.dim == "2d" and in_shape[1] != 1):
+            raise ValueError(f"MedNeXt needs spatial sizes divisible by 16, got {tuple(in_shape[1:4])}"
                              + (" (dim='2d': depth must be 1)" if self.dim == "2d" else ""))
         enc0 = list(self.enc_block_0)
-        N = int(x_cl.shape[0])
+        N = int(in_shape[0])
         sb = int(self.l0_subbatch)
         chained = 0 < sb < N and dt == torch.bfloat16 and hip.fused and self.dim == "3d"
         fuse_stem = self.fuse_stem and hip.fused and dt == torch.bfloat16 and bool(enc0)
 
-        def level0_encoder(xs: torch.Tensor, skip_out: Optional[torch.Tensor], down_out: Optional[torch.Tensor]):
+        def level0_encoder(xs: Optional[torch.Tensor], skip_out: Optional[torch.Tensor], down_out: Optional[torch.Tensor], ws=None):
             blocks = list(enc0)
             h = None
             if fuse_stem:
-                h = hip._stem_block_fused(self.stem, blocks[0], xs, skip_out if len(blocks) == 1 else None)
+                h = hip._stem_block_fused(self.stem, blocks[0], xs, skip_out if len(blocks) == 1 else None, window_source=ws)
                 if h is not None:
                     blocks = blocks[1:]
             if h is None:
+                if xs is None:
+                    xs = ws.gather()
                 h = hip.pointwise(xs, self.stem, out_dtype=dt)
                 if not blocks and skip_out is not None:
                     h = skip_out.copy_(h)
@@ -644,16 +658,19 @@
             return h
 
         skips = []
+        ws = window_source
         if chained:
-            _, D0, H0, W0, _ = x_cl.shape
+            _, D0, H0, W0, _ = in_shape
+            dev = ws.vol.device if ws is not None else x_cl.device
             c0, c1 = self.stem.weight.shape[0], self.down_0.conv3.weight.shape[0]
-            skip0 = torch.empty((N, D0, H0, W0, c0), dtype=dt, device=x_cl.device)
-            x = torch.empty((N, D0 // 2, H0 // 2, W0 // 2, c1), dtype=dt, device=x_cl.device)
+            skip0 = torch.empty((N, D0, H0, W0, c0), dtype=dt, device=dev)
+            x = torch.empty((N, D0 // 2, H0 // 2, W0 // 2, c1), dtype=dt, device=dev)
             for s0 in range(0, N, sb):
-                level0_encoder(x_cl[s0:s0 + sb], skip0[s0:s0 + sb], x[s0:s0 + sb])
+                level0_encoder(None if ws is not None else x_cl[s0:s0 + sb], skip0[s0:s0 + sb], x[s0:s0 + sb],
+                               None if ws is None else ws.narrow(s0, s0 + sb))
             skips.append(skip0)
         else:
-            h, x = level0_encoder(x_cl, None, None)
+            h, x = level0_encoder(x_cl, None, None, ws)
             skips.append(h)
         for lvl in range(1, 4):
             for blk in getattr(self, f"enc_block_{lvl}"):
@@ -686,8 +703,10 @@
         return self._hip.pointwise(feat_cl, getattr(self, f"out_{head}").conv_out, out_dtype=torch.float32,
                                    transposed=True)
 
-    def forward_cl(self, x_cl: torch.Tensor):
-        out = self.features_cl(x_cl, head=self.out_0.conv_out if self.fuse_head else None)
+    accepts_window_source = True
+
+    def forward_cl(self, x_cl: Optional[torch.Tensor], window_source=None):
+        out = self.features_cl(x_cl, head=self.out_0.conv_out if self.fuse_head else None, window_source=window_source)
         if isinstance(out, tuple):
             return out[1]
         return self.output_cl(out)
diff --git a/pytorch_connectomics_amd/models/architectures/mednext_models.py b/pytorch_connectomics_amd/models/architectures/mednext_models.py
--- a/pytorch_connectomics_amd/models/architectures/mednext_models.py
+++ b/pytorch_connectomics_amd/models/architectures/mednext_models.py
@@ -32,7 +32,13 @@
                     "ds_4": outputs[4]}
         return outputs
 
-    def forward_cl(self, x_cl: torch.Tensor) -> torch.Tensor:
+    @property
+    def accepts_window_source(self) -> bool:
+        return bool(getattr(self.model, "accepts_window_source", False))
+
+    def forward_cl(self, x_cl: Optional[torch.Tensor], window_source=None) -> torch.Tensor:
+        if window_source is not None:
+            return self.model.forward_cl(None, window_source=window_source)
         return self.model.forward_cl(x_cl)
 
 
```

After: 1.796 billion voxels/s (median of 6 runs). No clear change (+0.4%).
